# neeharperi/FutureDet

Measured on AMD Instinct MI355X. Metric: sweeps/sec end-to-end (300k pts, 10-sweep voxel), higher is better.
Workload: dtype f32

## Files before the change

### futuredet_amd/backbones.py

```python
import numpy as np
import torch
from torch import nn

from . import hip_ops, sparse as spconv
from .nn_utils import build_norm_layer
from .registry import BACKBONES
from .sparse import SparseConv3d, SubMConv3d


def conv3x3(in_planes, out_planes, stride=1, indice_key=None, bias=True):
    return spconv.SubMConv3d(in_planes, out_planes, kernel_size=3, stride=stride, padding=1, bias=bias,
                             indice_key=indice_key)


class SparseBasicBlock(spconv.SparseModule):
    expansion = 1

    def __init__(self, inplanes, planes, stride=1, norm_cfg=None, downsample=None, indice_key=None):
        super().__init__()
        if norm_cfg is None:
            norm_cfg = dict(type="BN1d", eps=1e-3, momentum=0.01)
        bias = norm_cfg is not None
        self.conv1 = conv3x3(inplanes, planes, stride, indice_key=indice_key, bias=bias)
        self.bn1 = build_norm_layer(norm_cfg, planes)[1]
        self.relu = nn.ReLU()
        self.conv2 = conv3x3(planes, planes, indice_key=indice_key, bias=bias)
        self.bn2 = build_norm_layer(norm_cfg, planes)[1]
        self.downsample = downsample
        self.stride = stride

    def forward(self, x):
        identity = x
        out = self.conv1(x)
        out.features = self.relu(self.bn1(out.features))
        out = self.conv2(out)
        out.features = self.bn2(out.features)
        if self.downsample is not None:
            identity = self.downsample(x)
        out.features = self.relu(out.features + identity.features)
        return out


@BACKBONES.register_module
class SpMiddleResNetFHD(nn.Module):
    def __init__(self, num_input_features=128, norm_cfg=None, name="SpMiddleResNetFHD", **kwargs):
        super().__init__()
        self.name = name
        if norm_cfg is None:
            norm_cfg = dict(type="BN1d", eps=1e-3, momentum=0.01)
        S = spconv.SparseSequential
        self.conv_input = S(SubMConv3d(num_input_features, 16, 3, bias=False, indice_key="res0"),
                            build_norm_layer(norm_cfg, 16)[1], nn.ReLU(inplace=True))
        self.conv1 = S(SparseBasicBlock(16, 16, norm_cfg=norm_cfg, indice_key="res0"),
                       SparseBasicBlock(16, 16, norm_cfg=norm_cfg, indice_key="res0"))
        self.conv2 = S(SparseConv3d(16, 32, 3, 2, padding=1, bias=False), build_norm_layer(norm_cfg, 32)[1],
                       nn.ReLU(inplace=True), SparseBasicBlock(32, 32, norm_cfg=norm_cfg, indice_key="res1"),
                       SparseBasicBlock(32, 32, norm_cfg=norm_cfg, indice_key="res1"))
        self.conv3 = S(SparseConv3d(32, 64, 3, 2, padding=1, bias=False), build_norm_layer(norm_cfg, 64)[1],
                       nn.ReLU(inplace=True), SparseBasicBlock(64, 64, norm_cfg=norm_cfg, indice_key="res2"),
                       SparseBasicBlock(64, 64, norm_cfg=norm_cfg, indice_key="res2"))
        self.conv4 = S(SparseConv3d(64, 128, 3, 2, padding=[0, 1, 1], bias=False), build_norm_layer(norm_cfg, 128)[1],
                       nn.ReLU(inplace=True), SparseBasicBlock(128, 128, norm_cfg=norm_cfg, indice_key="res3"),
                       SparseBasicBlock(128, 128, norm_cfg=norm_cfg, indice_key="res3"))
        self.extra_conv = S(SparseConv3d(128, 128, (3, 1, 1), (2, 1, 1), bias=False), build_norm_layer(norm_cfg, 128)[1],
                            nn.ReLU())
        self.compute_dtype = torch.float32
        self.dense_channels_last = True
        self.dense_dtype = None
        self.profile_hook = None

    def forward_generic(self, voxel_features, coors, batch_size, input_shape):
        sparse_shape = np.array(input_shape[::-1]) + [1, 0, 0]
        ret = spconv.SparseConvTensor(voxel_features, coors.int(), sparse_shape, batch_size)
        x = self.conv_input(ret)
        x_conv1 = self.conv1(x)
        x_conv2 = self.conv2(x_conv1)
        x_conv3 = self.conv3(x_conv2)
        x_conv4 = self.conv4(x_conv3)
        ret = self.extra_conv(x_conv4).dense()
        N, C, D, H, W = ret.shape
        ret = ret.view(N, C * D, H, W)
        return ret, {"conv1": x_conv1, "conv2": x_conv2, "conv3": x_conv3, "conv4": x_conv4}

    def _stages(self):
        return [(self.conv_input[0], self.conv_input[1], [self.conv1[0], self.conv1[1]], True),
                (self.conv2[0], self.conv2[1], [self.conv2[3], self.conv2[4]], False),
                (self.conv3[0], self.conv3[1], [self.conv3[3], self.conv3[4]], False),
                (self.conv4[0], self.conv4[1], [self.conv4[3], self.conv4[4]], False),
                (self.extra_conv[0], self.extra_conv[1], [], False)]

    def build_indexes(self, mark_fn, batch_size, input_shape, device, voxels=None, static=False, expected=None, row_caps=None):
        D, H, W = [int(v) for v in (np.array(input_shape[::-1]) + [1, 0, 0])]
        if voxels is not None:
            geoms = [self._stages()[lvl][0].geometry() for lvl in range(1, 5)]
            return hip_ops.build_pyramid(voxels[0], voxels[1], voxels[2], batch_size, (D, H, W), geoms, device, static=static,
                                         expected=expected, row_caps=row_caps)
        assert not static, "static indexes are built from the voxelizer's device output (voxels=...)"
        counts = torch.zeros((5,), dtype=torch.int32, device=device)
        idx = [hip_ops.SparseIndex(batch_size, D, H, W, device)]
        mark_fn(idx[0])
        idx[0].scan(counts[0:1])
        for lvl in range(1, 5):
            conv = self._stages()[lvl][0]
            ks, st, pd = conv.geometry()
            nxt = idx[-1].downsample(ks, st, pd)
            nxt.scan(counts[lvl:lvl + 1])
            idx.append(nxt)
        host = counts.cpu()
        for i, ix in enumerate(idx):
            ix.finalize(int(host[i]))
        return idx

    def run_fused(self, idx, feats0, dense_out=None, fork=False):
        dt = self.compute_dtype
        stages = self._stages()
        rb_cache = {}

        def rulebook(src, dst, conv):
            ks, st, pd = conv.geometry()
            key = (id(src), id(dst), tuple(ks), tuple(st), tuple(pd))
            if key not in rb_cache:
                rb_cache[key] = src.rulebook(dst, ks, st, pd)
            return rb_cache[key]

        def run(conv, bn, x, src, dst, relu, residual=None):
            wpk, bias, cin_p, cout_p = conv.packed_weight(dt, bn)
            assert x.shape[1] == cin_p, (x.shape, cin_p)
            nbr = rulebook(src, dst, conv)
            fn = lambda: hip_ops.spconv_apply(x, wpk, bias, nbr, dst.n, cout_p, residual=residual, relu=relu)
            if self.profile_hook is not None:
                s = 4 if dt == torch.float32 else 2
                K = nbr.shape[0]
                pairs = lambda: int((nbr[:, : dst.n] >= 0).sum().item())
                return self.profile_hook("spconv_%dx%d_K%d" % (cin_p, cout_p, K),
                                         dict(s=s, K=K, cin=cin_p, cout=cout_p, n_in=src.n, n_out=dst.n, pairs=pairs), fn)
            return fn()

        main, side = None, None
        if fork and feats0.is_cuda:
            main = torch.cuda.current_stream(feats0.device)
            pool = self.__dict__.setdefault("_side_streams", {})
            side = pool.get(main.cuda_stream)
            if side is None:
                side = pool[main.cuda_stream] = torch.cuda.Stream(device=feats0.device)
            side.wait_stream(main)
            with torch.cuda.stream(side):
                made = []
                for lvl, (conv, bn, blocks, is_subm_in) in enumerate(stages):
                    if lvl == 0:
                        continue
                    src_l, dst_l = (idx[lvl] if is_subm_in else idx[lvl - 1]), idx[lvl]
                    made.append(rulebook(src_l, dst_l, conv))
                    for blk in blocks:
                        nbr = rulebook(dst_l, dst_l, blk.conv1)
                        made.append(nbr)
                        cp = spconv.pad_channels(blk.conv1.out_channels)
                        if dt == torch.float32 and nbr.shape[0] == 27 and \
                                hip_ops._lib.load().fd_spconv_wants_balanced_ranges(cp, cp, 0):
                            r = hip_ops.ranges_for(nbr, cp, cp)
                            if r[0] is not None:
                                made.append(r[0])
                for t in made:
                    t.record_stream(main)
        x = feats0
        levels = {}
        for lvl, (conv, bn, blocks, is_subm_in) in enumerate(stages):
            src = idx[lvl] if is_subm_in else idx[lvl - 1]
            dst = idx[lvl]
            if lvl == 1 and side is not None:
                main.wait_stream(side)
            x = run(conv, bn, x, src, dst, relu=True)
            for blk in blocks:
                y = run(blk.conv1, blk.bn1, x, dst, dst, relu=True)
                x = run(blk.conv2, blk.bn2, y, dst, dst, relu=True, residual=x)
            levels[lvl] = (x, dst)
        bev = hip_ops.densify(x, idx[4], out_dtype=self.dense_dtype or dt, channels_last=self.dense_channels_last, out=dense_out)
        return bev, levels

    def forward(self, voxel_features, coors, batch_size, input_shape):
        if self.training:
            if self.compute_dtype != torch.float32 and torch.is_grad_enabled():
                raise NotImplementedError("SpMiddleResNetFHD: training runs the fp32 sparse convolution only; the %s path is inference-only "
                                          "(set compute_dtype = torch.float32 to train)" % self.compute_dtype)
            return self.forward_generic(voxel_features, coors, batch_size, input_shape)
        coors = coors.int().contiguous()
        dev = voxel_features.device
        idx = self.build_indexes(lambda i0: i0.mark(coors), batch_size, input_shape, dev)
        row_of = idx[0].lookup(coors)
        feats0 = hip_ops.rows_permute(voxel_features.float().contiguous(), row_of,
                                      spconv.pad_channels(voxel_features.shape[1]), self.compute_dtype, n_rows=idx[0].n)
        bev, levels = self.run_fused(idx, feats0)
        multi = {}
        for name, lvl, c in (("conv1", 0, 16), ("conv2", 1, 32), ("conv3", 2, 64), ("conv4", 3, 128)):
            f, ix = levels[lvl]
            multi[name] = spconv.SparseConvTensor(f[:, :c], None, ix.spatial_shape, batch_size, _index=ix)
        return bev, multi


@BACKBONES.register_module
class PointPillarsScatter(nn.Module):

    def __init__(self, num_input_features=64, norm_cfg=None, name="PointPillarsScatter", **kwargs):
        super().__init__()
        self.name = "PointPillarsScatter"
        self.nchannels = num_input_features
        self.dense_channels_last = True

    def forward(self, voxel_features, coords, batch_size, input_shape, n_dev=None):
        self.nx = int(input_shape[0])
        self.ny = int(input_shape[1])
        coords = coords.int().contiguous()
        if n_dev is None and torch.is_grad_enabled() and voxel_features.requires_grad:
            return _ScatterFn.apply(voxel_features, coords, batch_size, self.ny, self.nx, self.dense_channels_last)
        return hip_ops.pillar_scatter(voxel_features, coords, n_dev, batch_size, self.ny, self.nx,
                                      channels_last=self.dense_channels_last)


class _ScatterFn(torch.autograd.Function):

    @staticmethod
    def forward(ctx, feats, coords, batch_size, ny, nx, channels_last):
        ctx.coords = coords
        return hip_ops.pillar_scatter(feats, coords, None, batch_size, ny, nx, channels_last=channels_last)

    @staticmethod
    def backward(ctx, dcanvas):
        d = hip_ops.pillar_scatter_backward(dcanvas.float(), ctx.coords)
        ctx.coords = None
        return d, None, None, None, None, None
```

### futuredet_amd/csrc/fd_common.h

```cpp
#pragma once
#include <hip/hip_runtime.h>
#include <stdint.h>
#include <stdio.h>

#include <atomic>

#include "../../include/futuredet_hip.h"

namespace fd {

void set_error(const char *fmt, ...);
int spconv_f32_compact_dispatch(const float *in, const void *wp, const float *bias, const float *residual, int relu, const int *nbr,
                                int64_t nbr_stride, int K, int64_t n_in_bound, int n_out, const int *n_out_dev, int cin, int cout, float *out,
                                const int *ranges, int n_ranges, hipStream_t stream);

size_t spconv_bf16_win_weight_bytes(int K, int cin, int cout);
void spconv_bf16_win_pack(const float *w, int K, int cin, int cout, uint16_t (*tobf)(float), uint16_t *dst);
int spconv_bf16_win_dispatch(const void *in, const void *wp_win, const float *bias, const void *residual, int relu, const int *nbr, int64_t nbr_stride, int K,
                             int64_t n_in_bound, int n_out, const int *n_out_dev, int64_t n_expected, int cin, int cout, void *out, hipStream_t stream);
int spconv_bf16_ws_dispatch(const void *in, const void *wp, const float *bias, const void *residual, int relu, const int *nbr, int64_t nbr_stride, int K,
                            int64_t n_in_bound, int n_out, const int *n_out_dev, int64_t n_expected, int cin, int cout, void *out, hipStream_t stream);

int wino_pc_launch(const float *x, const void *wp, const float *bias, float *y, int B, int H, int W, int cin, int cout, int relu, int cout_total,
                   int co_off, int wide_items, hipStream_t stream);

int spconv_f32_res16_dispatch(const float *in, const void *wp, const float *bias, const float *residual, int relu, const int *nbr, int64_t nbr_stride, int K,
                              int64_t n_in_bound, int n_out, const int *n_out_dev, int64_t n_expected, int cin, int cout, float *out, hipStream_t stream);

int spconv_f32_c32_dispatch(const float *in, const void *wp, const float *bias, const float *residual, int relu, const int *nbr,
                            int64_t nbr_stride, int K, int64_t n_in_bound, int n_out, const int *n_out_dev, int cin, int cout, float *out,
                            const int *ranges, int n_ranges, hipStream_t stream);

__device__ __forceinline__ int device_count(int capacity, const int *count_dev) {
    if (!count_dev) return capacity;
    const int n = *count_dev;
    return n < capacity ? (n > 0 ? n : 0) : capacity;
}

inline int check_launch(const char *what) {
    hipError_t e = hipGetLastError();
    if (e != hipSuccess) {
        set_error("%s: %s", what, hipGetErrorString(e));
        return FD_ELAUNCH;
    }
    return FD_OK;
}

#define FD_REQUIRE(cond, ...)           \
    do {                                \
        if (!(cond)) {                  \
            fd::set_error(__VA_ARGS__); \
            return FD_EINVAL;           \
        }                               \
    } while (0)

inline hipStream_t as_stream(fd_stream_t s) { return reinterpret_cast<hipStream_t>(s); }

int fill_words(void *p, uint32_t value, size_t n_words, hipStream_t stream);
int fill_words3(void *p0, uint32_t v0, size_t n0, void *p1, uint32_t v1, size_t n1, void *p2, uint32_t v2, size_t n2, hipStream_t stream);

constexpr int kMaxDevices = 64;
int current_device();
int device_cu_count();
bool ensure_dynamic_lds(const void *kernel, size_t bytes, std::atomic<uint64_t> &done);
enum TuneKey { kTuneSpconvRG = 0, kTuneSpconvV1, kTuneSpconvBf16V1, kTuneV2Depth, kTuneV2TM, kTuneV2LdsPad, kTuneConvNT, kTuneV2RangesPerCU, kTuneV2Uniform, kTuneV2RowCost, kTuneSpconvC32, kTuneBf16GP, kTuneBf16RG, kTuneBf16Depth, kTuneBf16NW, kTuneStrict, kTuneBf16Win, kTuneF32ResRG, kTuneConvStrip, kTuneF32ResNW, kTuneCount };
int tuning(TuneKey key);

inline size_t align_up(size_t v, size_t a) { return (v + a - 1) / a * a; }

struct IndexGeom {
    int B, D, H, W, Ht, Wt;
    __host__ __device__ int64_t num_cols() const { return (int64_t)B * Ht * Wt * 64; }
};
__host__ __device__ inline IndexGeom make_geom(int B, int D, int H, int W) {
    IndexGeom g;
    g.B = B; g.D = D; g.H = H; g.W = W;
    g.Ht = (H + 7) >> 3; g.Wt = (W + 7) >> 3;
    return g;
}
__host__ __device__ inline int64_t col_of(const IndexGeom &g, int b, int y, int x) {
    return ((((int64_t)b * g.Ht + (y >> 3)) * g.Wt + (x >> 3)) << 6) + ((y & 7) << 3) + (x & 7);
}
__device__ inline void col_to_byx(const IndexGeom &g, int64_t col, int &b, int &y, int &x) {
    int in = (int)(col & 63);
    int64_t t = col >> 6;
    int tx = (int)(t % g.Wt);
    t /= g.Wt;
    int ty = (int)(t % g.Ht);
    b = (int)(t / g.Ht);
    y = ty * 8 + (in >> 3);
    x = tx * 8 + (in & 7);
}

__device__ inline unsigned xcd_swizzle(unsigned bid, unsigned nblocks) {
    const unsigned nx = 8;
    unsigned per = nblocks / nx, rem = nblocks % nx;
    unsigned xcd = bid % nx, loc = bid / nx;
    unsigned start = xcd * per + (xcd < rem ? xcd : rem);
    return start + loc;
}

}
```

### futuredet_amd/csrc/fd_error.hip

```cpp
#include <stdarg.h>
#include <stdlib.h>
#include <string.h>

#include "fd_common.h"

namespace fd {
static thread_local char g_err[512] = "";
void set_error(const char *fmt, ...) {
    va_list ap;
    va_start(ap, fmt);
    vsnprintf(g_err, sizeof(g_err), fmt, ap);
    va_end(ap);
}

int current_device() {
    int dev = 0;
    if (hipGetDevice(&dev) != hipSuccess) {
        (void)hipGetLastError();
        return 0;
    }
    return dev;
}

int device_cu_count() {
    static std::atomic<int> cache[kMaxDevices];
    const int dev = current_device();
    if (dev < 0 || dev >= kMaxDevices) return 256;
    int n = cache[dev].load(std::memory_order_relaxed);
    if (n <= 0) {
        if (hipDeviceGetAttribute(&n, hipDeviceAttributeMultiprocessorCount, dev) != hipSuccess || n <= 0) {
            (void)hipGetLastError();
            n = 256;
        }
        cache[dev].store(n, std::memory_order_relaxed);
    }
    return n;
}

bool ensure_dynamic_lds(const void *kernel, size_t bytes, std::atomic<uint64_t> &done) {
    const int dev = current_device();
    const uint64_t bit = (dev >= 0 && dev < kMaxDevices) ? (1ull << dev) : 0ull;
    if (bit && (done.load(std::memory_order_acquire) & bit)) return true;
    if (hipFuncSetAttribute(kernel, hipFuncAttributeMaxDynamicSharedMemorySize, (int)bytes) != hipSuccess) {
        (void)hipGetLastError();
        return false;
    }
    if (bit) done.fetch_or(bit, std::memory_order_release);
    return true;
}

namespace {
struct TuneTable {
    std::atomic<int> v[kTuneCount];
    TuneTable() {
        static const char *const env[kTuneCount] = {"FD_SPCONV_RG", "FD_SPCONV_V1", "FD_SPCONV_BF16_V1", "FD_V2_DEPTH", "FD_V2_TM",
                                                    "FD_V2_LDSPAD", "FD_CONV_NT", "FD_V2_RANGES_PER_CU", "FD_V2_UNIFORM", "FD_V2_ROWCOST", "FD_SPCONV_C32", "FD_BF16_GP", "FD_BF16_RG", "FD_BF16_DEPTH", "FD_BF16_NW", "FD_STRICT", "FD_BF16_WIN", "FD_F32_RES_RG", "FD_CONV_STRIP", "FD_F32_RES_NW"};
        for (int i = 0; i < kTuneCount; ++i) {
            const char *e = getenv(env[i]);
            v[i].store(e ? atoi(e) : 0, std::memory_order_relaxed);
        }
    }
};
TuneTable &tune_table() {
    static TuneTable t;
    return t;
}
const char *const kTuneNames[kTuneCount] = {"spconv_rg", "spconv_v1", "spconv_bf16_v1", "v2_depth", "v2_tm", "v2_ldspad", "conv_nt", "v2_ranges_per_cu", "v2_uniform", "v2_rowcost", "spconv_c32", "bf16_gp", "bf16_rg", "bf16_depth", "bf16_nw", "strict", "bf16_win", "f32_res_rg", "conv_strip", "f32_res_nw"};
}

int tuning(TuneKey key) { return tune_table().v[key].load(std::memory_order_relaxed); }
}

namespace {
struct FillJob {
    uint32_t *p[3];
    uint32_t v[3];
    size_t n[3];
    unsigned first_block[4];
};
__global__ void __launch_bounds__(256) fill_words_kernel(FillJob j) {
    const int r = blockIdx.x >= j.first_block[2] ? 2 : (blockIdx.x >= j.first_block[1] ? 1 : 0);
    uint32_t *__restrict__ p = j.p[r];
    const uint32_t v = j.v[r];
    const size_t n = j.n[r];
    const size_t nb = j.first_block[r + 1] - j.first_block[r], b = blockIdx.x - j.first_block[r];
    const size_t head = ((16 - ((uintptr_t)p & 15)) & 15) / 4 < n ? ((16 - ((uintptr_t)p & 15)) & 15) / 4 : n;
    const size_t n4 = (n - head) / 4;
    uint4 *p4 = reinterpret_cast<uint4 *>(p + head);
    const uint4 v4 = make_uint4(v, v, v, v);
    for (size_t i = b * 256 + threadIdx.x; i < n4; i += nb * 256) p4[i] = v4;
    if (b == 0) {
        if (threadIdx.x < head) p[threadIdx.x] = v;
        const size_t tail0 = head + n4 * 4;
        if (tail0 + threadIdx.x < n && threadIdx.x < 4) p[tail0 + threadIdx.x] = v;
    }
}
}

int fd::fill_words3(void *p0, uint32_t v0, size_t n0, void *p1, uint32_t v1, size_t n1, void *p2, uint32_t v2, size_t n2, hipStream_t stream) {
    FillJob j;
    void *ps[3] = {p0, p1, p2};
    const uint32_t vs[3] = {v0, v1, v2};
    const size_t ns[3] = {n0, n1, n2};
    unsigned total = 0;
    for (int r = 0; r < 3; ++r) {
        j.p[r] = (uint32_t *)ps[r];
        j.v[r] = vs[r];
        j.n[r] = ps[r] ? ns[r] : 0;
        j.first_block[r] = total;
        size_t blocks = j.n[r] ? (j.n[r] / 4 + 1023) / 1024 : 0;
        if (j.n[r] && blocks == 0) blocks = 1;
        if (blocks > 2048) blocks = 2048;
        total += (unsigned)blocks;
    }
    j.first_block[3] = total;
    if (!total) return 0;
    hipLaunchKernelGGL(fill_words_kernel, dim3(total), dim3(256), 0, stream, j);
    return 0;
}

int fd::fill_words(void *p, uint32_t value, size_t n_words, hipStream_t stream) {
    return fd::fill_words3(p, value, n_words, nullptr, 0u, 0, nullptr, 0u, 0, stream);
}

extern "C" const char *fd_last_error(void) { return fd::g_err; }
extern "C" int fd_abi_version(void) { return 8; }

extern "C" int fd_tuning_set(const char *name, int value) {
    FD_REQUIRE(name, "fd_tuning_set: null name");
    for (int i = 0; i < fd::kTuneCount; ++i)
        if (strcmp(name, fd::kTuneNames[i]) == 0) {
            fd::tune_table().v[i].store(value, std::memory_order_relaxed);
            return FD_OK;
        }
    fd::set_error("fd_tuning_set: unknown knob '%s'", name);
    return FD_EINVAL;
}
```

### futuredet_amd/csrc/fd_spconv.hip

```cpp
#include "fd_common.h"

namespace {

typedef float f32x4 __attribute__((ext_vector_type(4)));
typedef short s16x4 __attribute__((ext_vector_type(4)));
typedef __bf16 bf16x8 __attribute__((ext_vector_type(8)));

__device__ inline unsigned short f2bf(float v) {
    unsigned u = __float_as_uint(v);
    u += 0x7fffu + ((u >> 16) & 1u);
    return (unsigned short)(u >> 16);
}
__device__ inline float bf2f(unsigned short h) { return __uint_as_float(((unsigned)h) << 16); }

constexpr int kMaxTaps = 27;

template <int CIN, int COUT, int RG>
__global__ void __launch_bounds__(256) spconv_f32(const float *__restrict__ in, const float4 *__restrict__ wp,
                                                  const float *__restrict__ bias, const float *__restrict__ residual, int relu,
                                                  const int *__restrict__ nbr, int64_t nbr_stride, int K, int n_out,
                                                  const int *__restrict__ n_out_dev, float *__restrict__ out) {
    constexpr int ROWS_B = 64 * RG;
    constexpr int NB = COUT / 16, NC = CIN / 16;
    __shared__ int s_nbr[kMaxTaps * ROWS_B];
    const int tile = blockIdx.x;
    const int row0 = tile * ROWS_B;
    n_out = fd::device_count(n_out, n_out_dev);
    if (row0 >= n_out) return;
    for (int t = threadIdx.x; t < K * ROWS_B; t += 256) {
        int k = t / ROWS_B, r = t - k * ROWS_B;
        int64_t o = (int64_t)row0 + r;
        s_nbr[t] = (o < n_out) ? nbr[(int64_t)k * nbr_stride + o] : -1;
    }
    __syncthreads();
    const int lane = threadIdx.x & 63, wave = __builtin_amdgcn_readfirstlane(threadIdx.x >> 6);
    const int lrow = lane & 15, lq = lane >> 4;
    const int wrow = wave * 16 * RG;
    if (row0 + wrow >= n_out) return;

    f32x4 acc[RG][NB];
#pragma unroll
    for (int g = 0; g < RG; ++g)
#pragma unroll
        for (int nb = 0; nb < NB; ++nb) acc[g][nb] = (f32x4){0.f, 0.f, 0.f, 0.f};

    for (int k = 0; k < K; ++k) {
        int idx[RG];
        bool any[RG];
        bool any_all = false;
#pragma unroll
        for (int g = 0; g < RG; ++g) {
            idx[g] = s_nbr[k * ROWS_B + wrow + g * 16 + lrow];
            any[g] = __ballot(idx[g] >= 0) != 0ull;
            any_all = any_all || any[g];
        }
        if (!any_all) continue;
        const float4 *wk = wp + (int64_t)k * NC * NB * 64 + lane;
#pragma unroll
        for (int c = 0; c < NC; ++c) {
            float4 a[RG];
#pragma unroll
            for (int g = 0; g < RG; ++g) {
                a[g] = make_float4(0.f, 0.f, 0.f, 0.f);
                if (idx[g] >= 0) a[g] = *reinterpret_cast<const float4 *>(in + (int64_t)idx[g] * CIN + c * 16 + lq * 4);
            }
#pragma unroll
            for (int nb = 0; nb < NB; ++nb) {
                const float4 b = wk[(c * NB + nb) * 64];
#pragma unroll
                for (int g = 0; g < RG; ++g) {
                    if (any[g]) {
                        acc[g][nb] = __builtin_amdgcn_mfma_f32_16x16x4f32(a[g].x, b.x, acc[g][nb], 0, 0, 0);
                        acc[g][nb] = __builtin_amdgcn_mfma_f32_16x16x4f32(a[g].y, b.y, acc[g][nb], 0, 0, 0);
                        acc[g][nb] = __builtin_amdgcn_mfma_f32_16x16x4f32(a[g].z, b.z, acc[g][nb], 0, 0, 0);
                        acc[g][nb] = __builtin_amdgcn_mfma_f32_16x16x4f32(a[g].w, b.w, acc[g][nb], 0, 0, 0);
                    }
                }
            }
        }
    }
#pragma unroll
    for (int g = 0; g < RG; ++g) {
#pragma unroll
        for (int nb = 0; nb < NB; ++nb) {
            const int col = nb * 16 + lrow;
            const float bv = bias ? bias[col] : 0.0f;
#pragma unroll
            for (int r = 0; r < 4; ++r) {
                const int row = row0 + wrow + g * 16 + lq * 4 + r;
                if (row < n_out) {
                    float v = acc[g][nb][r] + bv;
                    if (residual) v += residual[(int64_t)row * COUT + col];
                    if (relu) v = fmaxf(v, 0.0f);
                    out[(int64_t)row * COUT + col] = v;
                }
            }
        }
    }
}

template <int CIN, int COUT, int RG>
__global__ void __launch_bounds__(256) spconv_bf16(const unsigned short *__restrict__ in, const void *__restrict__ wp_,
                                                   const float *__restrict__ bias, const unsigned short *__restrict__ residual,
                                                   int relu, const int *__restrict__ nbr, int64_t nbr_stride, int K, int n_out,
                                                   const int *__restrict__ n_out_dev, unsigned short *__restrict__ out) {
    constexpr int ROWS_B = 64 * RG;
    constexpr int NB = COUT / 16;
    constexpr bool WIDE = CIN >= 32;
    constexpr int NC = WIDE ? CIN / 32 : 1;
    __shared__ int s_nbr[kMaxTaps * ROWS_B];
    const int tile = blockIdx.x;
    const int row0 = tile * ROWS_B;
    n_out = fd::device_count(n_out, n_out_dev);
    if (row0 >= n_out) return;
    for (int t = threadIdx.x; t < K * ROWS_B; t += 256) {
        int k = t / ROWS_B, r = t - k * ROWS_B;
        int64_t o = (int64_t)row0 + r;
        s_nbr[t] = (o < n_out) ? nbr[(int64_t)k * nbr_stride + o] : -1;
    }
    __syncthreads();
    const int lane = threadIdx.x & 63, wave = __builtin_amdgcn_readfirstlane(threadIdx.x >> 6);
    const int lrow = lane & 15, lq = lane >> 4;
    const int wrow = wave * 16 * RG;
    if (row0 + wrow >= n_out) return;

    f32x4 acc[RG][NB];
#pragma unroll
    for (int g = 0; g < RG; ++g)
#pragma unroll
        for (int nb = 0; nb < NB; ++nb) acc[g][nb] = (f32x4){0.f, 0.f, 0.f, 0.f};

    for (int k = 0; k < K; ++k) {
        int idx[RG];
        bool any[RG];
        bool any_all = false;
#pragma unroll
        for (int g = 0; g < RG; ++g) {
            idx[g] = s_nbr[k * ROWS_B + wrow + g * 16 + lrow];
            any[g] = __ballot(idx[g] >= 0) != 0ull;
            any_all = any_all || any[g];
        }
        if (!any_all) continue;
        if constexpr (WIDE) {
            const bf16x8 *wk = reinterpret_cast<const bf16x8 *>(wp_) + (int64_t)k * NC * NB * 64 + lane;
#pragma unroll
            for (int c = 0; c < NC; ++c) {
                bf16x8 a[RG];
#pragma unroll
                for (int g = 0; g < RG; ++g) {
                    uint4 raw = make_uint4(0u, 0u, 0u, 0u);
                    if (idx[g] >= 0) raw = *reinterpret_cast<const uint4 *>(in + (int64_t)idx[g] * CIN + c * 32 + lq * 8);
                    a[g] = __builtin_bit_cast(bf16x8, raw);
                }
#pragma unroll
                for (int nb = 0; nb < NB; ++nb) {
                    const bf16x8 b = wk[(c * NB + nb) * 64];
#pragma unroll
                    for (int g = 0; g < RG; ++g)
                        if (any[g]) acc[g][nb] = __builtin_amdgcn_mfma_f32_16x16x32_bf16(a[g], b, acc[g][nb], 0, 0, 0);
                }
            }
        } else {
            const s16x4 *wk = reinterpret_cast<const s16x4 *>(wp_) + (int64_t)k * NB * 64 + lane;
            s16x4 a[RG];
#pragma unroll
            for (int g = 0; g < RG; ++g) {
                uint2 raw = make_uint2(0u, 0u);
                if (idx[g] >= 0) raw = *reinterpret_cast<const uint2 *>(in + (int64_t)idx[g] * CIN + lq * 4);
                a[g] = __builtin_bit_cast(s16x4, raw);
            }
#pragma unroll
            for (int nb = 0; nb < NB; ++nb) {
                const s16x4 b = wk[nb * 64];
#pragma unroll
                for (int g = 0; g < RG; ++g)
                    if (any[g]) acc[g][nb] = __builtin_amdgcn_mfma_f32_16x16x16bf16_1k(a[g], b, acc[g][nb], 0, 0, 0);
            }
        }
    }
#pragma unroll
    for (int g = 0; g < RG; ++g) {
#pragma unroll
        for (int nb = 0; nb < NB; ++nb) {
            const int col = nb * 16 + lrow;
            const float bv = bias ? bias[col] : 0.0f;
#pragma unroll
            for (int r = 0; r < 4; ++r) {
                const int row = row0 + wrow + g * 16 + lq * 4 + r;
                if (row < n_out) {
                    float v = acc[g][nb][r] + bv;
                    if (residual) v += bf2f(residual[(int64_t)row * COUT + col]);
                    if (relu) v = fmaxf(v, 0.0f);
                    out[(int64_t)row * COUT + col] = f2bf(v);
                }
            }
        }
    }
}

struct LaunchArgs {
    const void *in, *wp;
    const float *bias;
    const void *residual;
    int relu;
    const int *nbr;
    int64_t nbr_stride;
    int K, n_out;
    const int *n_out_dev;
    void *out;
    hipStream_t stream;
};

template <int CIN, int COUT, int RG>
void launch(const LaunchArgs &a, int dtype) {
    const int rows_b = 64 * RG;
    dim3 grid((unsigned)((a.n_out + rows_b - 1) / rows_b));
    if (dtype == 0)
        hipLaunchKernelGGL((spconv_f32<CIN, COUT, RG>), grid, dim3(256), 0, a.stream, (const float *)a.in, (const float4 *)a.wp, a.bias,
                           (const float *)a.residual, a.relu, a.nbr, a.nbr_stride, a.K, a.n_out, a.n_out_dev, (float *)a.out);
    else
        hipLaunchKernelGGL((spconv_bf16<CIN, COUT, RG>), grid, dim3(256), 0, a.stream, (const unsigned short *)a.in, a.wp, a.bias,
                           (const unsigned short *)a.residual, a.relu, a.nbr, a.nbr_stride, a.K, a.n_out, a.n_out_dev, (unsigned short *)a.out);
}

template <int CIN, int COUT>
void launch_rg(const LaunchArgs &a, int dtype, int rg) {
    if (rg >= 4) launch<CIN, COUT, 4>(a, dtype);
    else if (rg == 2) launch<CIN, COUT, 2>(a, dtype);
    else launch<CIN, COUT, 1>(a, dtype);
}

int pick_rg(int64_t n_out, int cin, int cout) {
    const int forced = fd::tuning(fd::kTuneSpconvRG);
    if (forced > 0) return forced;
    const int64_t waves2 = (n_out + 31) / 32;
    int rg = (cin * cout >= 128 * 128) ? 1 : 2;
    if (rg == 2 && waves2 < 256 * 4 * 2) rg = 1;
    return rg;
}

}

inline bool has_c32_layout(int cin, int cout, int dtype) { return dtype == 0 && cout == 32 && cin == 32; }
inline int64_t pair_layout_elems(int K, int cin, int cout, int dtype) { return (dtype == 1 && cin == 16) ? (int64_t)((K + 1) / 2) * 32 * cout : 0; }

extern "C" size_t fd_spconv_packed_weight_bytes(int K, int cin, int cout, int dtype) {
    if (K <= 0 || cin <= 0 || cout <= 0) return 0;
    return (size_t)K * cin * cout * (dtype == 0 ? 4 : 2) * (has_c32_layout(cin, cout, dtype) ? 2 : 1) + (size_t)pair_layout_elems(K, cin, cout, dtype) * 2 +
           (dtype == 1 ? fd::spconv_bf16_win_weight_bytes(K, cin, cout) : 0);
}

extern "C" int fd_spconv_pack_weight(const float *w, int K, int cin, int cout, int dtype, void *dst) {
    FD_REQUIRE(w && dst, "fd_spconv_pack_weight: null argument");
    FD_REQUIRE(K >= 1 && K <= kMaxTaps, "fd_spconv_pack_weight: K must be in [1,27]");
    FD_REQUIRE(cin % 16 == 0 && cout % 16 == 0 && cin >= 16 && cin <= 128 && cout >= 16 && cout <= 128,
               "fd_spconv_pack_weight: channels must be multiples of 16 in [16,128] (got %d -> %d)", cin, cout);
    FD_REQUIRE(dtype == 0 || dtype == 1, "fd_spconv_pack_weight: dtype must be 0 (f32) or 1 (bf16)");
    const int NB = cout / 16;
    auto W = [&](int k, int ci, int co) { return w[((int64_t)k * cin + ci) * cout + co]; };
    auto tobf = [](float v) -> uint16_t {
        union { float f; uint32_t u; } cvt;
        cvt.f = v;
        uint32_t u = cvt.u;
        u += 0x7fffu + ((u >> 16) & 1u);
        return (uint16_t)(u >> 16);
    };
    if (dtype == 0) {
        const int NC = cin / 16;
        float *d = (float *)dst;
        for (int k = 0; k < K; ++k)
            for (int c = 0; c < NC; ++c)
                for (int nb = 0; nb < NB; ++nb)
                    for (int lane = 0; lane < 64; ++lane)
                        for (int j = 0; j < 4; ++j)
                            d[((((int64_t)k * NC + c) * NB + nb) * 64 + lane) * 4 + j] =
                                W(k, 16 * c + 4 * (lane >> 4) + j, 16 * nb + (lane & 15));
        if (has_c32_layout(cin, cout, dtype)) {
            float *e = d + (int64_t)K * cin * cout;
            for (int k = 0; k < K; ++k)
                for (int c = 0; c < cin / 8; ++c)
                    for (int lane = 0; lane < 64; ++lane)
                        for (int j = 0; j < 4; ++j)
                            e[(((int64_t)k * (cin / 8) + c) * 64 + lane) * 4 + j] = W(k, 8 * c + 4 * (lane >> 5) + j, lane & 31);
        }
    } else if (cin >= 32) {
        FD_REQUIRE(cin % 32 == 0, "fd_spconv_pack_weight: bf16 needs cin 16 or a multiple of 32");
        const int NC = cin / 32;
        uint16_t *d = (uint16_t *)dst;
        for (int k = 0; k < K; ++k)
            for (int c = 0; c < NC; ++c)
                for (int nb = 0; nb < NB; ++nb)
                    for (int lane = 0; lane < 64; ++lane)
                        for (int j = 0; j < 8; ++j)
                            d[((((int64_t)k * NC + c) * NB + nb) * 64 + lane) * 8 + j] =
                                tobf(W(k, 32 * c + 8 * (lane >> 4) + j, 16 * nb + (lane & 15)));
        if (fd::spconv_bf16_win_weight_bytes(K, cin, cout)) fd::spconv_bf16_win_pack(w, K, cin, cout, +tobf, d + (int64_t)K * cin * cout);
    } else {
        uint16_t *d = (uint16_t *)dst;
        for (int k = 0; k < K; ++k)
            for (int nb = 0; nb < NB; ++nb)
                for (int lane = 0; lane < 64; ++lane)
                    for (int j = 0; j < 4; ++j)
                        d[(((int64_t)k * NB + nb) * 64 + lane) * 4 + j] = tobf(W(k, 4 * (lane >> 4) + j, 16 * nb + (lane & 15)));
        uint16_t *e = d + (int64_t)K * cin * cout;
        for (int u = 0; u < (K + 1) / 2; ++u)
            for (int nb = 0; nb < NB; ++nb)
                for (int lane = 0; lane < 64; ++lane)
                    for (int j = 0; j < 8; ++j) {
                        const int q = lane >> 4, k = 2 * u + (q >> 1);
                        e[(((int64_t)u * NB + nb) * 64 + lane) * 8 + j] = k < K ? tobf(W(k, 8 * (q & 1) + j, 16 * nb + (lane & 15))) : (uint16_t)0;
                    }
    }
    return FD_OK;
}

extern "C" int fd_spconv_apply(const void *in_feats, int64_t n_in, const void *wpacked, const float *bias, const void *residual, int relu,
                               const int32_t *nbr, int64_t nbr_stride, const int32_t *ranges, int n_ranges, int K, int64_t n_out,
                               const int32_t *n_out_dev, int64_t n_expected, int cin, int cout, int dtype, void *out_feats, fd_stream_t stream) {
    FD_REQUIRE(K >= 1 && K <= kMaxTaps, "fd_spconv_apply: K must be in [1,27]");
    FD_REQUIRE(dtype == 0 || dtype == 1, "fd_spconv_apply: dtype must be 0 (f32) or 1 (bf16)");
    FD_REQUIRE(n_out >= 0 && n_out <= nbr_stride && n_out < (1ll << 31), "fd_spconv_apply: n_out out of range");
    FD_REQUIRE(n_ranges >= 0 && (ranges == nullptr || n_ranges >= 1), "fd_spconv_apply: ranges needs n_ranges >= 1");
    if (n_expected <= 0 || n_expected > n_out) n_expected = n_out;
    if (n_out == 0) return FD_OK;
    FD_REQUIRE(in_feats && wpacked && nbr && out_feats, "fd_spconv_apply: null argument");
    if (dtype == 0 && !fd::tuning(fd::kTuneSpconvV1) && cin == 16 && fd::tuning(fd::kTuneF32ResRG) >= 0) {
        if (fd::spconv_f32_res16_dispatch((const float *)in_feats, wpacked, bias, (const float *)residual, relu, nbr, nbr_stride, K, n_in, (int)n_out,
                                          n_out_dev, n_expected, cin, cout, (float *)out_feats, fd::as_stream(stream)))
            return fd::check_launch("fd_spconv_apply(f32 resident)");
    }
    if (dtype == 0 && !fd::tuning(fd::kTuneSpconvV1) && has_c32_layout(cin, cout, dtype) && fd::tuning(fd::kTuneSpconvC32) >= 0) {
        const void *w32 = (const char *)wpacked + (size_t)K * cin * cout * 4;
        if (fd::spconv_f32_c32_dispatch((const float *)in_feats, w32, bias, (const float *)residual, relu, nbr, nbr_stride, K, n_in, (int)n_out,
                                        n_out_dev, cin, cout, (float *)out_feats, ranges, n_ranges, fd::as_stream(stream)))
            return fd::check_launch("fd_spconv_apply(c32)");
    }
    if (dtype == 0 && !fd::tuning(fd::kTuneSpconvV1)) {
        if (fd::spconv_f32_compact_dispatch((const float *)in_feats, wpacked, bias, (const float *)residual, relu, nbr, nbr_stride, K, n_in,
                                            (int)n_out, n_out_dev, cin, cout, (float *)out_feats, ranges, n_ranges, fd::as_stream(stream)))
            return fd::check_launch("fd_spconv_apply(compact)");
    }
    if (dtype == 1 && fd::tuning(fd::kTuneBf16GP) >= 0) {
        const void *w = cin == 16 ? (const void *)((const char *)wpacked + (size_t)K * cin * cout * 2) : wpacked;
        const bool subm_like = (K == 27 && n_in == n_out) || fd::tuning(fd::kTuneBf16Win) == 2;
        if (fd::tuning(fd::kTuneBf16Win) >= 0 && subm_like && fd::spconv_bf16_win_weight_bytes(K, cin, cout) &&
            fd::spconv_bf16_win_dispatch(in_feats, (const char *)wpacked + (size_t)K * cin * cout * 2, bias, residual, relu, nbr, nbr_stride, K, n_in, (int)n_out,
                                         n_out_dev, n_expected, cin, cout, out_feats, fd::as_stream(stream)))
            return fd::check_launch("fd_spconv_apply(bf16 window)");
        if (fd::spconv_bf16_ws_dispatch(in_feats, w, bias, residual, relu, nbr, nbr_stride, K, n_in, (int)n_out, n_out_dev, n_expected, cin, cout, out_feats,
                                        fd::as_stream(stream)))
            return fd::check_launch("fd_spconv_apply(bf16 ws)");
        if (fd::tuning(fd::kTuneStrict) && n_in * cin * 2 < (1ll << 31)) {
            fd::set_error("fd_spconv_apply: strict mode: the bf16 kernel (fd_spconv_bf16.hip) did not take %d -> %d, K = %d", cin, cout, K);
            return FD_EINVAL;
        }
    }
    LaunchArgs a{in_feats, wpacked, bias, residual, relu, nbr, nbr_stride, K, (int)n_out, n_out_dev, out_feats, fd::as_stream(stream)};
    const int rg = pick_rg(n_expected, cin, cout);
    const int key = cin * 1000 + cout;
    switch (key) {
        case 16016: launch_rg<16, 16>(a, dtype, rg); break;
        case 16032: launch_rg<16, 32>(a, dtype, rg); break;
        case 32032: launch_rg<32, 32>(a, dtype, rg); break;
        case 32064: launch_rg<32, 64>(a, dtype, rg); break;
        case 64064: launch_rg<64, 64>(a, dtype, rg); break;
        case 64128: launch_rg<64, 128>(a, dtype, rg); break;
        case 128128: launch_rg<128, 128>(a, dtype, rg); break;
        default:
            fd::set_error("fd_spconv_apply: unsupported channels %d -> %d", cin, cout);
            return FD_EINVAL;
    }
    return fd::check_launch("fd_spconv_apply");
}
```

### futuredet_amd/csrc/fd_spconv_c32.hip

```cpp
#include "fd_spconv_chunk.h"

namespace {

namespace sk = fd::skeleton;
typedef float f32x16 __attribute__((ext_vector_type(16)));
typedef unsigned u32x4 __attribute__((ext_vector_type(4)));
constexpr int TM = 128, COUT = 32, TS = 4, WR = 1;
constexpr sk::Layout L = sk::layout(TM, COUT, TS, 32);
static_assert(((sk::kMaxTaps + TS - 1) / TS) * (TM / WR / 32) <= L.item_slot, "item list slot");

template <int CIN, int DEPTH>
__global__ void __launch_bounds__(256) spconv_f32_c32(const float *__restrict__ in, const float4 *__restrict__ wp, const float *__restrict__ bias,
                                                      const float *__restrict__ residual, int relu, const int *__restrict__ nbr, int64_t nbr_stride,
                                                      int K, int n_out, const int *__restrict__ n_out_dev, float *__restrict__ out, unsigned in_bytes,
                                                      const int *__restrict__ ranges, int rows_per_range) {
    constexpr int NCH = CIN / 8;
    constexpr int kPad = sk::pad_entry(TM);
    extern __shared__ __attribute__((aligned(16))) unsigned char smem[];
    int *s_list = reinterpret_cast<int *>(smem + L.list);
    unsigned short *s_items = reinterpret_cast<unsigned short *>(smem + L.items);
    unsigned char *s_cnt = smem + L.cnt;
    int *s_pad = reinterpret_cast<int *>(smem + L.pad);
    float *s_acc = reinterpret_cast<float *>(smem + L.acc);

    const int tid = threadIdx.x, lane = tid & 63, wave = __builtin_amdgcn_readfirstlane(tid >> 6);
    int r_begin, r_end, n_chunks, chunk_rows;
    sk::resolve_range(n_out, n_out_dev, ranges, rows_per_range, r_begin, r_end);
    if (r_begin >= r_end) return;
    sk::cut_chunks<TM>(r_begin, r_end, n_chunks, chunk_rows);
    int pre[sk::kSliceRegs<TM>];
    sk::fetch_slice<TM>(pre, nbr, nbr_stride, K, r_begin);

    const int ln = lane & 31, lh = lane >> 5;
    const int ts = wave, wr = 0;
    unsigned char *acc_bytes = reinterpret_cast<unsigned char *>(s_acc + ts * L.acc_copy);
    const __amdgpu_buffer_rsrc_t rsrc = __builtin_amdgcn_make_buffer_rsrc(const_cast<float *>(in), 0, (int)in_bytes, 0x00020000);
    unsigned short *items = s_items + wave * L.item_slot;

    for (int chunk = 0; chunk < n_chunks; ++chunk) {
        int row0, n_rows;
        if (!sk::chunk_span(r_begin, r_end, chunk_rows, chunk, row0, n_rows)) break;
        sk::stage_chunk<TM, COUT, TS, 32>(pre, s_list, s_pad, s_acc, bias, residual, K, row0, n_rows);
        __syncthreads();
        sk::compact_taps<TM, WR>(s_list, s_cnt, K);
        __syncthreads();
        if (chunk + 1 < n_chunks) sk::fetch_slice<TM>(pre, nbr, nbr_stride, K, row0 + chunk_rows);
        const int n_items = sk::build_items<TS, 32>(s_cnt, items, K, ts, wr);

        int k_r[DEPTH], row_r[DEPTH];
        u32x4 a_r[DEPTH][NCH];
        auto stage_a0 = [&](int it) -> int { return sk::stage_a0(items, n_items, it); };
        auto stage_a1 = [&](int it, int code_v, int &kk, int &e) { sk::stage_a1<TM, WR, 32>(s_list, s_pad, n_items, wr, ln, it, code_v, kk, e); };
        auto gather_offset = [&](int e) -> unsigned { return sk::entry_row_bytes<CIN>(e) + (unsigned)(lh * 16); };
        auto gather_step = [&](unsigned voff, int c) { return __builtin_amdgcn_raw_buffer_load_b128(rsrc, voff + c * 32, 0, 0); };
        float4 b[NCH];
        auto load_b = [&](int k) {
            const float4 *wk = wp + (int64_t)k * NCH * 64 + lane;
#pragma unroll
            for (int c = 0; c < NCH; ++c) b[c] = wk[c * 64];
        };
        int k_s, e_s, code_s;
#pragma unroll
        for (int d = 0; d < DEPTH - 1; ++d) {
            stage_a1(d, stage_a0(d), k_s, e_s);
            const unsigned vo = gather_offset(e_s);
#pragma unroll
            for (int c = 0; c < NCH; ++c) a_r[d][c] = gather_step(vo, c);
            k_r[d] = k_s;
            row_r[d] = e_s;
        }
        k_r[DEPTH - 1] = -1;
        row_r[DEPTH - 1] = kPad;
        stage_a1(DEPTH - 1, stage_a0(DEPTH - 1), k_s, e_s);
        code_s = stage_a0(DEPTH);
        if (n_items > 0) load_b(k_r[0]);

        for (int i0 = 0; i0 < n_items; i0 += DEPTH) {
#pragma unroll
            for (int d = 0; d < DEPTH; ++d) {
                const unsigned arow = sk::entry_local_row(row_r[d]);
                unsigned aoff[4];
#pragma unroll
                for (int q = 0; q < 4; ++q) aoff[q] = sk::acc_slot_bytes<COUT>(arow, (unsigned)(2 * q + lh));
                f32x16 acc;
#pragma unroll
                for (int q = 0; q < 4; ++q) {
                    const float4 v = *reinterpret_cast<const float4 *>(acc_bytes + aoff[q]);
                    acc[4 * q + 0] = v.x; acc[4 * q + 1] = v.y; acc[4 * q + 2] = v.z; acc[4 * q + 3] = v.w;
                }
                const int dn = (d + DEPTH - 1) % DEPTH;
                {
                    const int it = i0 + d + DEPTH - 1;
                    const unsigned vo = gather_offset(e_s);
                    k_r[dn] = k_s;
                    row_r[dn] = e_s;
#pragma unroll
                    for (int c = 0; c < NCH; ++c) a_r[dn][c] = gather_step(vo, c);
                    stage_a1(it + 1, code_s, k_s, e_s);
                    code_s = stage_a0(it + 2);
                }
                const int knext = k_r[(d + 1) % DEPTH];
                const bool reload = knext >= 0 && knext != k_r[d];
                __builtin_amdgcn_sched_barrier(0);
#pragma unroll
                for (int c = 0; c < NCH; ++c) {
                    const float4 av = __builtin_bit_cast(float4, a_r[d][c]);
                    acc = __builtin_amdgcn_mfma_f32_32x32x2f32(b[c].x, av.x, acc, 0, 0, 0);
                    acc = __builtin_amdgcn_mfma_f32_32x32x2f32(b[c].y, av.y, acc, 0, 0, 0);
                    acc = __builtin_amdgcn_mfma_f32_32x32x2f32(b[c].z, av.z, acc, 0, 0, 0);
                    acc = __builtin_amdgcn_mfma_f32_32x32x2f32(b[c].w, av.w, acc, 0, 0, 0);
                    if (reload) b[c] = (wp + (int64_t)knext * NCH * 64 + lane)[c * 64];
                }
#pragma unroll
                for (int q = 0; q < 4; ++q)
                    *reinterpret_cast<float4 *>(acc_bytes + aoff[q]) = make_float4(acc[4 * q + 0], acc[4 * q + 1], acc[4 * q + 2], acc[4 * q + 3]);
                __builtin_amdgcn_sched_barrier(0);
            }
        }
        __syncthreads();
        sk::epilogue<TM, COUT, TS>(s_acc, bias, residual, relu, out, row0, n_rows);
        __syncthreads();
    }
}

template <int CIN, int DEPTH>
int launch_c32(const float *in, const void *wp, const float *bias, const float *residual, int relu, const int *nbr, int64_t nbr_stride, int K,
               int n_out, const int *n_out_dev, float *out, unsigned in_bytes, const int *ranges, int n_ranges, hipStream_t stream) {
    int rows_per = 0;
    if (!ranges) sk::equal_rows_split(n_out, TM, n_out_dev != nullptr, n_ranges, rows_per);
    static std::atomic<uint64_t> lds_set{0};
    if (!fd::ensure_dynamic_lds(reinterpret_cast<const void *>(spconv_f32_c32<CIN, DEPTH>), (size_t)L.bytes, lds_set)) return 0;
    hipLaunchKernelGGL((spconv_f32_c32<CIN, DEPTH>), dim3((unsigned)n_ranges), dim3(256), (size_t)L.bytes, stream, in, (const float4 *)wp, bias, residual, relu,
                       nbr, nbr_stride, K, n_out, n_out_dev, out, in_bytes, ranges, rows_per);
    return 1;
}

}

namespace fd {
int spconv_f32_c32_dispatch(const float *in, const void *wp, const float *bias, const float *residual, int relu, const int *nbr, int64_t nbr_stride,
                            int K, int64_t n_in_bound, int n_out, const int *n_out_dev, int cin, int cout, float *out, const int *ranges,
                            int n_ranges, hipStream_t stream) {
    if (cout != 32 || cin != 32) return 0;
    if (!sk::entries_fit(n_in_bound, cin)) return 0;
    const unsigned in_bytes = (unsigned)(n_in_bound * cin * 4);
    const int depth = fd::tuning(fd::kTuneV2Depth);
    if (depth == 2) return launch_c32<32, 2>(in, wp, bias, residual, relu, nbr, nbr_stride, K, n_out, n_out_dev, out, in_bytes, ranges, n_ranges, stream);
    if (depth == 4) return launch_c32<32, 4>(in, wp, bias, residual, relu, nbr, nbr_stride, K, n_out, n_out_dev, out, in_bytes, ranges, n_ranges, stream);
    return launch_c32<32, 3>(in, wp, bias, residual, relu, nbr, nbr_stride, K, n_out, n_out_dev, out, in_bytes, ranges, n_ranges, stream);
}
}
```

### futuredet_amd/csrc/fd_spconv_chunk.h

```cpp
#pragma once
#include "fd_common.h"

namespace fd {
namespace skeleton {

constexpr int kMaxTaps = 27;

constexpr int pad_entry(int tm) { return (int)(0xffffff00u | (unsigned)tm); }
__device__ __forceinline__ int pack_entry(int in_row, int local_row) { return (in_row << 8) | local_row; }
__device__ __forceinline__ unsigned entry_local_row(int e) { return (unsigned)e & 255u; }
template <int CIN>
__device__ __forceinline__ unsigned entry_row_bytes(int e) {
    static_assert(CIN == 16 || CIN == 32 || CIN == 64 || CIN == 128, "shift per CIN");
    const unsigned hi = (unsigned)e & 0xffffff00u;
    return CIN >= 64 ? hi << (CIN == 128 ? 1 : 0) : hi >> (CIN == 32 ? 1 : 2);
}
inline bool entries_fit(int64_t n_in_bound, int cin) { return n_in_bound < (1ll << 23) && n_in_bound * cin * 4 < (1ll << 31); }

struct Layout {
    int list;
    int items;
    int item_slot;
    int cnt;
    int pad;
    int acc;
    int acc_copy;
    int bytes;
};
constexpr int acc_copy_floats(int tm, int cout) { return (tm + 1) * cout; }
constexpr Layout layout(int tm, int cout, int ts, int item) {
    Layout l{};
    l.list = 0;
    l.items = l.list + (int)sizeof(int) * kMaxTaps * tm;
    l.item_slot = item == 16 ? kMaxTaps * (tm / 16) : 32;
    l.cnt = l.items + (int)sizeof(unsigned short) * 4 * l.item_slot;
    l.pad = l.cnt + 112;
    l.acc = l.pad + (int)sizeof(int) * item;
    l.acc_copy = acc_copy_floats(tm, cout);
    l.bytes = l.acc + (int)sizeof(float) * ts * l.acc_copy;
    return l;
}

template <int COUT>
__device__ __forceinline__ unsigned acc_swizzle(unsigned row) {
    static_assert(COUT == 16 || COUT == 32 || COUT == 64 || COUT == 128, "whole bank rows");
    constexpr int kSwzShift = COUT >= 64 ? 0 : COUT == 32 ? 1 : 2;
    constexpr unsigned kSwzMask = COUT >= 64 ? 15u : COUT == 32 ? 7u : 3u;
    return (row >> kSwzShift) & kSwzMask;
}
template <int COUT>
__device__ __forceinline__ int acc_slot(int row, int col) {
    return row * (COUT / 4) + (col ^ (int)acc_swizzle<COUT>((unsigned)row));
}
template <int COUT>
__device__ __forceinline__ unsigned acc_slot_bytes(unsigned row, unsigned col) {
    return row * (COUT * 4) + ((col ^ acc_swizzle<COUT>(row)) << 4);
}

__device__ __forceinline__ void resolve_range(int n_out, const int *n_out_dev, const int *ranges, int rows_per_range,
                                              int &r_begin, int &r_end) {
    if (n_out_dev) n_out = fd::device_count(n_out, n_out_dev);
    if (ranges) {
        r_begin = ranges[blockIdx.x];
        r_end = ranges[blockIdx.x + 1];
    } else {
        if (n_out_dev) rows_per_range = (((n_out + (int)gridDim.x - 1) / (int)gridDim.x) + 15) & ~15;
        const int64_t b = (int64_t)blockIdx.x * rows_per_range;
        r_begin = (int)(b < n_out ? b : n_out);
        r_end = (int)(b + rows_per_range < n_out ? b + rows_per_range : n_out);
    }
    if (r_end > n_out) r_end = n_out;
}
template <int TM>
__device__ __forceinline__ void cut_chunks(int r_begin, int r_end, int &n_chunks, int &chunk_rows) {
    n_chunks = (r_end - r_begin + TM - 1) / TM;
    chunk_rows = (((r_end - r_begin + n_chunks - 1) / n_chunks) + 15) & ~15;
}
__device__ __forceinline__ bool chunk_span(int r_begin, int r_end, int chunk_rows, int chunk, int &row0, int &n_rows) {
    row0 = r_begin + chunk * chunk_rows;
    n_rows = (r_end - row0) < chunk_rows ? (r_end - row0) : chunk_rows;
    return n_rows > 0;
}
inline void equal_rows_split(int n_out, int tm, bool device_count, int &n_ranges, int &rows_per) {
    if (n_ranges <= 0) n_ranges = (n_out + tm - 1) / tm;
    rows_per = (((n_out + n_ranges - 1) / n_ranges) + 15) & ~15;
    if (!device_count) n_ranges = (n_out + rows_per - 1) / rows_per;
}

template <int TM>
constexpr int kSliceRegs = (kMaxTaps * TM + 255) / 256;

template <int TM>
__device__ __forceinline__ void fetch_slice(int (&pre)[kSliceRegs<TM>], const int *nbr, int64_t nbr_stride, int K, int row0) {
    const int tid = threadIdx.x;
#pragma unroll
    for (int i = 0; i < kSliceRegs<TM>; ++i) {
        const int t = tid + i * 256;
        int k = t / TM;
        const int r = t - k * TM;
        k = k < K ? k : K - 1;
        int64_t o = (int64_t)row0 + r;
        o = o < nbr_stride ? o : nbr_stride - 1;
        pre[i] = nbr[(int64_t)k * nbr_stride + o];
    }
}

template <int COUT>
constexpr bool kInitAcc = COUT <= 64;

template <int TM, int COUT, int TS>
__device__ __forceinline__ void init_acc(float *s_acc, const float *bias, const float *residual, int row0, int n_rows) {
    const int tid = threadIdx.x;
    if constexpr (kInitAcc<COUT>) {
        constexpr int C4i = COUT / 4, NINIT = TM * C4i / 256;
        static_assert(TM * C4i % 256 == 0, "whole passes");
        float4 iv[NINIT];
#pragma unroll
        for (int i = 0; i < NINIT; ++i) {
            const int t = tid + i * 256, c4 = t % C4i;
            iv[i] = bias ? reinterpret_cast<const float4 *>(bias)[c4] : make_float4(0.f, 0.f, 0.f, 0.f);
        }
        if (residual) {
            float4 rv[NINIT];
#pragma unroll
            for (int i = 0; i < NINIT; ++i) {
                const int t = tid + i * 256, r = t / C4i, c4 = t - r * C4i;
                const int rr = r < n_rows ? r : n_rows - 1;
                rv[i] = reinterpret_cast<const float4 *>(residual + (int64_t)(row0 + rr) * COUT)[c4];
            }
#pragma unroll
            for (int i = 0; i < NINIT; ++i) { iv[i].x += rv[i].x; iv[i].y += rv[i].y; iv[i].z += rv[i].z; iv[i].w += rv[i].w; }
        }
#pragma unroll
        for (int i = 0; i < NINIT; ++i) {
            const int t = tid + i * 256, r = t / C4i, c4 = t - r * C4i;
            reinterpret_cast<float4 *>(s_acc)[acc_slot<COUT>(r, c4)] = r < n_rows ? iv[i] : make_float4(0.f, 0.f, 0.f, 0.f);
        }
        for (int t = TM * C4i + tid; t < TS * acc_copy_floats(TM, COUT) / 4; t += 256) reinterpret_cast<float4 *>(s_acc)[t] = make_float4(0.f, 0.f, 0.f, 0.f);
    } else {
        for (int t = tid; t < TS * acc_copy_floats(TM, COUT) / 4; t += 256) reinterpret_cast<float4 *>(s_acc)[t] = make_float4(0.f, 0.f, 0.f, 0.f);
    }
}

template <int TM, int COUT, int TS, int ITEM>
__device__ __forceinline__ void stage_chunk(const int (&pre)[kSliceRegs<TM>], int *s_list, int *s_pad, float *s_acc, const float *bias,
                                            const float *residual, int K, int row0, int n_rows) {
    const int tid = threadIdx.x;
    static_assert(256 % TM == 0, "a thread stages the same local row in every pass");
    const bool in_chunk = tid % TM < n_rows;
#pragma unroll
    for (int i = 0; i < kSliceRegs<TM>; ++i) {
        const int t = tid + i * 256;
        if (t < K * TM) s_list[t] = in_chunk ? pre[i] : -1;
    }
    init_acc<TM, COUT, TS>(s_acc, bias, residual, row0, n_rows);
    if (tid < ITEM) s_pad[tid] = pad_entry(TM);
}

template <int TM, int WR>
__device__ __forceinline__ void compact_taps(int *s_list, unsigned char *s_cnt, int K) {
    const int lane = threadIdx.x & 63, wave = __builtin_amdgcn_readfirstlane(threadIdx.x >> 6);
    constexpr int RW = TM / WR, NH = (RW + 63) / 64;
    for (int k = wave; k < K; k += 4) {
#pragma unroll
        for (int wr = 0; wr < WR; ++wr) {
            const int base = k * TM + wr * RW;
            int count = 0;
            int v[NH];
#pragma unroll
            for (int h = 0; h < NH; ++h) {
                const int r = h * 64 + lane;
                v[h] = (r < RW) ? s_list[base + r] : -1;
            }
#pragma unroll
            for (int h = 0; h < NH; ++h) {
                const int r = h * 64 + lane;
                if (r < RW) s_list[base + r] = pad_entry(TM);
            }
#pragma unroll
            for (int h = 0; h < NH; ++h) {
                const int r = h * 64 + lane;
                const unsigned long long m = __ballot(v[h] >= 0);
                const int pos = count + __popcll(m & ((1ull << lane) - 1ull));
                if (v[h] >= 0) s_list[base + pos] = pack_entry(v[h], wr * RW + r);
                count += __popcll(m);
            }
            if (lane == 0) s_cnt[k * 4 + wr] = (unsigned char)count;
        }
    }
}

template <int TS, int ITEM>
__device__ __forceinline__ int build_items(const unsigned char *s_cnt, unsigned short *items, int K, int ts, int wr) {
    const int lane = threadIdx.x & 63;
    const int ng = (lane < K && (lane % TS) == ts) ? ((int)s_cnt[lane * 4 + wr] + ITEM - 1) / ITEM : 0;
    int inc = ng;
#pragma unroll
    for (int off = 1; off < 64; off <<= 1) {
        const int u = __shfl_up(inc, off);
        if (lane >= off) inc += u;
    }
    const int n_items = __builtin_amdgcn_readfirstlane(__shfl(inc, 63));
    for (int g = 0; g < ng; ++g) items[inc - ng + g] = (unsigned short)((lane << 3) | g);
    __builtin_amdgcn_fence(__ATOMIC_RELEASE, "workgroup");
    __builtin_amdgcn_wave_barrier();
    __builtin_amdgcn_fence(__ATOMIC_ACQUIRE, "workgroup");
    return n_items;
}

__device__ __forceinline__ int stage_a0(const unsigned short *items, int n_items, int it) { return (int)items[it < n_items ? it : 0]; }
template <int TM, int WR, int ITEM>
__device__ __forceinline__ void stage_a1(const int *s_list, const int *s_pad, int n_items, int wr, int lp, int it, int code_v, int &kk, int &e) {
    const bool v = it < n_items;
    const int code = __builtin_amdgcn_readfirstlane(code_v);
    const int ks = v ? (code >> 3) : 0;
    kk = v ? ks : -1;
    const int *lst = v ? s_list + ks * TM + wr * (TM / WR) + (code & 7) * ITEM : s_pad;
    e = lst[lp];
}

template <int TM, int COUT, int TS>
__device__ __forceinline__ void epilogue(float *s_acc, const float *bias, const float *residual, int relu,
                                         float *out, int row0, int n_rows) {
    const int tid = threadIdx.x;
    constexpr int C4 = COUT / 4;
    for (int t = tid; t < n_rows * C4; t += 256) {
        const int r = t / C4, c4 = t - r * C4;
        const int row = row0 + r;
        const int slot = acc_slot<COUT>(r, c4);
        float4 v = reinterpret_cast<const float4 *>(s_acc)[slot];
#pragma unroll
        for (int q = 1; q < TS; ++q) {
            const float4 v2 = reinterpret_cast<const float4 *>(s_acc + q * acc_copy_floats(TM, COUT))[slot];
            v.x += v2.x; v.y += v2.y; v.z += v2.z; v.w += v2.w;
        }
        if constexpr (!kInitAcc<COUT>) {
            if (bias) {
                const float4 bv = reinterpret_cast<const float4 *>(bias)[c4];
                v.x += bv.x; v.y += bv.y; v.z += bv.z; v.w += bv.w;
            }
            if (residual) {
                const float4 rv = reinterpret_cast<const float4 *>(residual + (int64_t)row * COUT)[c4];
                v.x += rv.x; v.y += rv.y; v.z += rv.z; v.w += rv.w;
            }
        }
        if (relu) { v.x = fmaxf(v.x, 0.f); v.y = fmaxf(v.y, 0.f); v.z = fmaxf(v.z, 0.f); v.w = fmaxf(v.w, 0.f); }
        reinterpret_cast<float4 *>(out + (int64_t)row * COUT)[c4] = v;
    }
}

}
}
```

### futuredet_amd/csrc/fd_spconv_v2.hip

```cpp
#include "fd_spconv_chunk.h"

namespace {

namespace sk = fd::skeleton;
typedef float f32x4 __attribute__((ext_vector_type(4)));
typedef unsigned u32x4 __attribute__((ext_vector_type(4)));
typedef int i32x4 __attribute__((ext_vector_type(4)));

#ifdef FD_V2_TRACE
__device__ unsigned long long *g_trace;
#define FD_T(i)                                                                                  \
    do {                                                                                         \
        if (threadIdx.x == 0 && g_trace) g_trace[(size_t)blockIdx.x * 16 + (i)] = __builtin_readcyclecounter(); \
    } while (0)
#define FD_TV(i, v)                                                                    \
    do {                                                                               \
        if (threadIdx.x == 0 && g_trace) g_trace[(size_t)blockIdx.x * 16 + (i)] = (v); \
    } while (0)
#else
#define FD_T(i)
#define FD_TV(i, v)
#endif


constexpr int tap_splits(int cout) { return (cout == 32 || cout == 64) ? 2 : 1; }

template <int CIN, int COUT, int TM, int DEPTH>
__global__ void __launch_bounds__(256) spconv_f32_compact(const float *__restrict__ in, const float4 *__restrict__ wp,
                                                          const float *__restrict__ bias, const float *__restrict__ residual, int relu,
                                                          const int *__restrict__ nbr, int64_t nbr_stride, int K, int n_out,
                                                          const int *__restrict__ n_out_dev, float *__restrict__ out, unsigned in_bytes,
                                                          const int *__restrict__ ranges, int rows_per_range) {
    constexpr int NB = COUT / 16, NC = CIN / 16;
    constexpr int WC = NB == 8 ? 4 : (NB >= 2 ? 2 : 1);
    constexpr int NBW = NB / WC;
    constexpr int TS = tap_splits(COUT);
    constexpr int WR = 4 / (WC * TS);
    constexpr int NACC = NBW;
    static_assert((TM == 128 || TM == 64) && TM / WR >= 16, "local row uses 8 bits (0..TM, TM = scratch row)");
    constexpr int kPad = sk::pad_entry(TM);
    constexpr sk::Layout L = sk::layout(TM, COUT, TS, 16);
    extern __shared__ __attribute__((aligned(16))) unsigned char smem[];
    int *s_list = reinterpret_cast<int *>(smem + L.list);
    unsigned short *s_items = reinterpret_cast<unsigned short *>(smem + L.items);
    unsigned char *s_cnt = smem + L.cnt;
    int *s_pad = reinterpret_cast<int *>(smem + L.pad);
    float *s_acc = reinterpret_cast<float *>(smem + L.acc);

    const int tid = threadIdx.x, lane = tid & 63, wave = __builtin_amdgcn_readfirstlane(tid >> 6);
    int r_begin, r_end, n_chunks, chunk_rows;
    sk::resolve_range(n_out, n_out_dev, ranges, rows_per_range, r_begin, r_end);
    if (r_begin >= r_end) return;
    FD_T(0);
    sk::cut_chunks<TM>(r_begin, r_end, n_chunks, chunk_rows);
    int pre[sk::kSliceRegs<TM>];
    sk::fetch_slice<TM>(pre, nbr, nbr_stride, K, r_begin);

    const int lrow = lane & 15, lq = lane >> 4;
    const int wc = wave % WC, wr = TS == 1 ? wave / WC : 0, ts = TS == 1 ? 0 : wave / WC;
    const int cb = wc * NBW * 16;
    unsigned char *acc_bytes = reinterpret_cast<unsigned char *>(s_acc + ts * L.acc_copy);
    const unsigned slot0 = (unsigned)(cb >> 2) + (unsigned)lq;
    const __amdgpu_buffer_rsrc_t rsrc = __builtin_amdgcn_make_buffer_rsrc(const_cast<float *>(in), 0, (int)in_bytes, 0x00020000);
    unsigned short *items = s_items + wave * L.item_slot;

    for (int chunk = 0; chunk < n_chunks; ++chunk) {
    int row0, n_rows;
    if (!sk::chunk_span(r_begin, r_end, chunk_rows, chunk, row0, n_rows)) break;
    sk::stage_chunk<TM, COUT, TS, 16>(pre, s_list, s_pad, s_acc, bias, residual, K, row0, n_rows);
    __syncthreads();
    if (chunk == 0) FD_T(1);
    sk::compact_taps<TM, WR>(s_list, s_cnt, K);
    __syncthreads();
    if (chunk == 0) FD_T(2);
    if (chunk + 1 < n_chunks) sk::fetch_slice<TM>(pre, nbr, nbr_stride, K, row0 + chunk_rows);
    const int n_items = sk::build_items<TS, 16>(s_cnt, items, K, ts, wr);

    int k_r[DEPTH];
    int row_r[DEPTH];
    u32x4 a_r[DEPTH][NC];
    auto stage_a0 = [&](int it) -> int { return sk::stage_a0(items, n_items, it); };
    auto stage_a1 = [&](int it, int code_v, int &kk, int &e) { sk::stage_a1<TM, WR, 16>(s_list, s_pad, n_items, wr, lrow, it, code_v, kk, e); };
    auto gather_offset = [&](int e) -> unsigned { return sk::entry_row_bytes<CIN>(e) + (unsigned)(lq * 16); };
    auto gather_chunk = [&](unsigned voff, int c) { return __builtin_amdgcn_raw_buffer_load_b128(rsrc, voff + c * 64, 0, 0); };
    auto load_b = [&](int k, float4(&dst)[NC][NBW]) {
        const float4 *wk = wp + ((int64_t)k * NC * NB + wc * NBW) * 64 + lane;
#pragma unroll
        for (int c = 0; c < NC; ++c)
#pragma unroll
            for (int nw = 0; nw < NBW; ++nw) dst[c][nw] = wk[(c * NB + nw) * 64];
    };
    float4 b[NC][NBW];
    static_assert(DEPTH >= 2, "the slot freed by the previous item is refilled during the current item's MFMAs");
    int k_s, e_s, code_s;
#pragma unroll
    for (int d = 0; d < DEPTH - 1; ++d) {
        stage_a1(d, stage_a0(d), k_s, e_s);
        const unsigned vo = gather_offset(e_s);
#pragma unroll
        for (int c = 0; c < NC; ++c) a_r[d][c] = gather_chunk(vo, c);
        k_r[d] = k_s;
        row_r[d] = e_s;
    }
    k_r[DEPTH - 1] = -1;
    row_r[DEPTH - 1] = kPad;
    stage_a1(DEPTH - 1, stage_a0(DEPTH - 1), k_s, e_s);
    code_s = stage_a0(DEPTH);
    if (n_items > 0) load_b(k_r[0], b);
    if (chunk == 0) { FD_T(3); FD_TV(8, (unsigned long long)n_items); FD_TV(9, (unsigned long long)n_chunks); FD_TV(10, (unsigned long long)n_rows);
                      FD_TV(11, (unsigned long long)__builtin_amdgcn_s_getreg(4 | (31 << 11))); FD_TV(12, (unsigned long long)__builtin_amdgcn_s_getreg(20 | (31 << 11))); }
    FD_TV(13, (unsigned long long)(g_trace ? g_trace[(size_t)blockIdx.x * 16 + 13] : 0) + (unsigned long long)n_items);

    auto mfma_chunk = [&](const u32x4 &a4, const float4(&bc)[NBW], f32x4(&acc)[NACC]) {
        const float4 av = __builtin_bit_cast(float4, a4);
#pragma unroll
        for (int nw = 0; nw < NBW; ++nw) acc[nw] = __builtin_amdgcn_mfma_f32_16x16x4f32(bc[nw].x, av.x, acc[nw], 0, 0, 0);
#pragma unroll
        for (int nw = 0; nw < NBW; ++nw) acc[nw] = __builtin_amdgcn_mfma_f32_16x16x4f32(bc[nw].y, av.y, acc[nw], 0, 0, 0);
#pragma unroll
        for (int nw = 0; nw < NBW; ++nw) acc[nw] = __builtin_amdgcn_mfma_f32_16x16x4f32(bc[nw].z, av.z, acc[nw], 0, 0, 0);
#pragma unroll
        for (int nw = 0; nw < NBW; ++nw) acc[nw] = __builtin_amdgcn_mfma_f32_16x16x4f32(bc[nw].w, av.w, acc[nw], 0, 0, 0);
    };

    for (int i0 = 0; i0 < n_items; i0 += DEPTH) {
#pragma unroll
        for (int d = 0; d < DEPTH; ++d) {
            const unsigned arow = sk::entry_local_row(row_r[d]);
            unsigned aoff[NBW];
#pragma unroll
            for (int nw = 0; nw < NBW; ++nw) aoff[nw] = sk::acc_slot_bytes<COUT>(arow, slot0 + 4u * nw);
            f32x4 acc[NACC];
#pragma unroll
            for (int nw = 0; nw < NBW; ++nw) acc[nw] = *reinterpret_cast<const f32x4 *>(acc_bytes + aoff[nw]);
            const int dn = (d + DEPTH - 1) % DEPTH;
            unsigned vo;
            {
                const int it = i0 + d + DEPTH - 1;
                vo = gather_offset(e_s);
                k_r[dn] = k_s;
                row_r[dn] = e_s;
                stage_a1(it + 1, code_s, k_s, e_s);
                code_s = stage_a0(it + 2);
            }
            const int knext = k_r[(d + 1) % DEPTH];
            const bool reload = knext >= 0 && knext != k_r[d];
            constexpr bool kSpread = NC * 4 * NBW >= 16;
            if constexpr (!kSpread) {
#pragma unroll
                for (int c = 0; c < NC; ++c) a_r[dn][c] = gather_chunk(vo, c);
            }
            __builtin_amdgcn_sched_barrier(0);
            if (reload) {
                const float4 *wk = wp + ((int64_t)knext * NC * NB + wc * NBW) * 64 + lane;
#pragma unroll
                for (int c = 0; c < NC; ++c) {
                    mfma_chunk(a_r[d][c], b[c], acc);
                    if constexpr (kSpread) a_r[dn][c] = gather_chunk(vo, c);
#pragma unroll
                    for (int nw = 0; nw < NBW; ++nw) b[c][nw] = wk[(c * NB + nw) * 64];
                    __builtin_amdgcn_sched_group_barrier(0x008, 4 * NBW, 0);
                    __builtin_amdgcn_sched_group_barrier(0x020, (kSpread ? 1 : 0) + NBW, 0);
                }
            } else {
#pragma unroll
                for (int c = 0; c < NC; ++c) {
                    mfma_chunk(a_r[d][c], b[c], acc);
                    if constexpr (kSpread) {
                        a_r[dn][c] = gather_chunk(vo, c);
                        __builtin_amdgcn_sched_group_barrier(0x008, 4 * NBW, 0);
                        __builtin_amdgcn_sched_group_barrier(0x020, 1, 0);
                    }
                }
            }
#pragma unroll
            for (int nw = 0; nw < NBW; ++nw) *reinterpret_cast<f32x4 *>(acc_bytes + aoff[nw]) = acc[nw];
            __builtin_amdgcn_sched_barrier(0);
        }
    }
    if (chunk == 0) FD_T(4);
    __syncthreads();
    if (chunk == 0) FD_T(5);
    sk::epilogue<TM, COUT, TS>(s_acc, bias, residual, relu, out, row0, n_rows);
    __syncthreads();
    if (chunk == 0) FD_T(6);
    }
    FD_T(7);
}

inline size_t lds_request(int cin, int cout, int tm) {
    const size_t lds = (size_t)sk::layout(tm, cout, tap_splits(cout), 16).bytes;
    const size_t pad = (size_t)fd::tuning(fd::kTuneV2LdsPad);
    if (pad) return lds + pad;
    return (cin == 64 && cout == 64 && tm == 128 && lds < 56 * 1024) ? (size_t)56 * 1024 : lds;
}

template <int CIN, int COUT, int TM, int DEPTH>
int launch_compact(const float *in, const void *wp, const float *bias, const float *residual, int relu, const int *nbr,
                   int64_t nbr_stride, int K, int n_out, const int *n_out_dev, float *out, unsigned in_bytes, const int *ranges, int n_ranges,
                   hipStream_t stream) {
    const size_t lds_req = lds_request(CIN, COUT, TM);
    static std::atomic<uint64_t> lds_set{0};
    auto kern = spconv_f32_compact<CIN, COUT, TM, DEPTH>;
    if (fd::tuning(fd::kTuneV2LdsPad)) {
        if (hipFuncSetAttribute(reinterpret_cast<const void *>(kern), hipFuncAttributeMaxDynamicSharedMemorySize, (int)lds_req) != hipSuccess) {
            (void)hipGetLastError();
            return 0;
        }
    } else if (!fd::ensure_dynamic_lds(reinterpret_cast<const void *>(kern), lds_req, lds_set)) {
        return 0;
    }
    int rows_per = 0;
    if (!ranges) sk::equal_rows_split(n_out, TM, n_out_dev != nullptr, n_ranges, rows_per);
    hipLaunchKernelGGL(kern, dim3((unsigned)n_ranges), dim3(256), lds_req, stream, in, (const float4 *)wp, bias, residual, relu, nbr, nbr_stride, K,
                       n_out, n_out_dev, out, in_bytes, ranges, rows_per);
    return 1;
}

constexpr int kWorkRows = 8;
constexpr int kRowCost = 24;
__global__ void __launch_bounds__(256) block_work_kernel(const int *__restrict__ nbr, int64_t nbr_stride, int K, int n_out,
                                                         const int *__restrict__ n_out_dev, unsigned row_cost, unsigned *__restrict__ work) {
    n_out = fd::device_count(n_out, n_out_dev);
    const int n_blocks = (n_out + kWorkRows - 1) / kWorkRows;
    const int lane = threadIdx.x & 63;
    const int64_t wave = (int64_t)blockIdx.x * 4 + (threadIdx.x >> 6);
    const int64_t o = wave * 64 + lane;
    if (wave * 8 >= n_blocks) return;
    unsigned w = row_cost;
    for (int k = 0; k < K; ++k) {
        const bool v = o < n_out && nbr[(int64_t)k * nbr_stride + o] >= 0;
        const unsigned long long m = __ballot(v);
        const unsigned byte = (unsigned)(m >> (8 * (lane & 7))) & 0xffu;
        w += (unsigned)__popc(byte) * 2u + (byte ? 1u : 0u);
    }
    if (lane < 8 && wave * 8 + lane < n_blocks) work[wave * 8 + lane] = w;
}

__global__ void __launch_bounds__(1024) range_split_kernel(const unsigned *__restrict__ work, int n_out, const int *__restrict__ n_out_dev,
                                                           int n_ranges, int *__restrict__ ranges) {
    n_out = fd::device_count(n_out, n_out_dev);
    const int n_blocks = (n_out + kWorkRows - 1) / kWorkRows;
    __shared__ unsigned long long s_seg[16];
    __shared__ unsigned long long s_total;
    const int tid = threadIdx.x, lane = tid & 63, wave = tid >> 6;
    if (n_blocks == 0) {
        for (int j = tid; j <= n_ranges; j += 1024) ranges[j] = 0;
        return;
    }
    const int seg = (((n_blocks + 15) / 16) + 63) & ~63;
    const int b_lo = wave * seg, b_hi = min(n_blocks, b_lo + seg);
    constexpr int kU = 16;
    unsigned long long sum = 0;
    for (int c0 = b_lo; c0 < b_hi; c0 += 64 * kU) {
        unsigned wv[kU];
#pragma unroll
        for (int u = 0; u < kU; ++u) {
            const int bb = c0 + 64 * u + lane;
            wv[u] = work[bb < b_hi ? bb : b_hi - 1];
        }
#pragma unroll
        for (int u = 0; u < kU; ++u) sum += (c0 + 64 * u + lane < b_hi) ? wv[u] : 0u;
    }
#pragma unroll
    for (int o = 32; o > 0; o >>= 1) sum += __shfl_xor(sum, o);
    if (lane == 0) s_seg[wave] = sum;
    __syncthreads();
    if (tid == 0) {
        unsigned long long run = 0;
        for (int w = 0; w < 16; ++w) { const unsigned long long v = s_seg[w]; s_seg[w] = run; run += v; }
        s_total = run;
    }
    __syncthreads();
    const unsigned long long total = s_total > 0 ? s_total : 1ull;
    const double scale = (double)n_ranges / (2.0 * (double)total);
    auto range_of = [&](unsigned long long ex, unsigned w) -> int {
        const int r = (int)((double)(2ull * ex + w) * scale);
        return r < n_ranges ? r : n_ranges - 1;
    };
    unsigned long long run = s_seg[wave];
    int prev = -1;
    if (b_lo > 0 && b_lo < n_blocks) {
        const unsigned wp = work[b_lo - 1];
        prev = range_of(run - wp, wp);
    }
    constexpr int kB = 8;
    __shared__ unsigned s_buf[16][64 * (kB + 1)];
    unsigned *buf = s_buf[wave];
    for (int c0 = b_lo; c0 < b_hi; c0 += 64 * kB) {
#pragma unroll
        for (int u = 0; u < kB; ++u) {
            const int e = 64 * u + lane, bb = c0 + e;
            buf[(e / kB) * (kB + 1) + e % kB] = bb < b_hi ? work[bb] : 0u;
        }
        __builtin_amdgcn_fence(__ATOMIC_RELEASE, "workgroup");
        __builtin_amdgcn_wave_barrier();
        __builtin_amdgcn_fence(__ATOMIC_ACQUIRE, "workgroup");
        unsigned w[kB];
        unsigned tot = 0;
#pragma unroll
        for (int i = 0; i < kB; ++i) {
            w[i] = buf[lane * (kB + 1) + i];
            tot += w[i];
        }
        unsigned inc = tot;
#pragma unroll
        for (int o = 1; o < 64; o <<= 1) {
            const unsigned u = __shfl_up(inc, o);
            if (lane >= o) inc += u;
        }
        unsigned long long ex = run + (inc - tot);
        const int first = c0 + lane * kB;
        int last_rg = prev;
        {
            unsigned long long e2 = ex;
#pragma unroll
            for (int i = 0; i < kB; ++i) {
                if (first + i < b_hi) last_rg = range_of(e2, w[i]);
                e2 += w[i];
            }
        }
        int before = __shfl_up(last_rg, 1);
        if (lane == 0) before = prev;
        if (first >= b_hi) last_rg = before;
#pragma unroll
        for (int i = 0; i < kB; ++i) {
            const int bb = first + i;
            if (bb < b_hi) {
                const int rg = range_of(ex, w[i]);
                for (int j = before + 1; j <= rg; ++j) ranges[j] = bb * kWorkRows;
                before = rg;
                if (bb == n_blocks - 1)
                    for (int j = rg + 1; j <= n_ranges; ++j) ranges[j] = n_out;
            }
            ex += w[i];
        }
        const int n_valid = min(64 * kB, b_hi - c0);
        prev = __shfl(last_rg, (n_valid - 1) / kB);
        run += __shfl(inc, 63);
        __builtin_amdgcn_wave_barrier();
    }
}

}

#ifdef FD_V2_TRACE
extern "C" int fd_debug_set_trace(void *p) { return hipMemcpyToSymbol(HIP_SYMBOL(g_trace), &p, sizeof(p)) == hipSuccess ? 0 : -1; }
#endif

extern "C" int fd_spconv_num_ranges(int64_t n_out, int cin, int cout, int dtype) {
    if (n_out <= 0 || dtype != 0) return 0;
    const int n_cu = fd::device_cu_count();
    const int64_t tiles = (n_out + 127) / 128;
    const int mult = fd::tuning(fd::kTuneV2RangesPerCU);
    int64_t per_cu;
    if (mult) per_cu = mult;
    else if (cout >= 64) per_cu = (int64_t)((160 * 1024) / lds_request(cin, cout, 128));
    else per_cu = (tiles + n_cu - 1) / n_cu;
    if (per_cu < 1) per_cu = 1;
    return (int)(per_cu * n_cu);
}

extern "C" int fd_spconv_wants_balanced_ranges(int cin, int cout, int dtype) { return dtype == 0 && cout >= 64 && !fd::tuning(fd::kTuneV2Uniform); }

extern "C" size_t fd_spconv_ranges_workspace_bytes(int64_t n_out) {
    return fd::align_up(sizeof(unsigned) * (size_t)((n_out + kWorkRows - 1) / kWorkRows + 8), 256);
}

extern "C" int fd_spconv_ranges(const int32_t *nbr, int64_t nbr_stride, int K, int64_t n_out, const int32_t *n_out_dev, int n_ranges,
                                int32_t *ranges, void *workspace, size_t workspace_bytes, fd_stream_t stream_) {
    FD_REQUIRE(nbr && ranges && workspace, "fd_spconv_ranges: null argument");
    FD_REQUIRE(n_ranges >= 1 && n_out >= 0 && n_out <= nbr_stride && n_out < (1ll << 31), "fd_spconv_ranges: bad sizes");
    FD_REQUIRE(workspace_bytes >= fd_spconv_ranges_workspace_bytes(n_out), "fd_spconv_ranges: workspace too small");
    hipStream_t stream = fd::as_stream(stream_);
    const int n_blocks = (int)((n_out + kWorkRows - 1) / kWorkRows);
    unsigned *work = (unsigned *)workspace;
    if (n_blocks > 0)
        hipLaunchKernelGGL(block_work_kernel, dim3((unsigned)((n_blocks + 31) / 32)), dim3(256), 0, stream, nbr, nbr_stride, K, (int)n_out, n_out_dev,
                           (unsigned)(fd::tuning(fd::kTuneV2RowCost) ? fd::tuning(fd::kTuneV2RowCost) : kRowCost), work);
    hipLaunchKernelGGL(range_split_kernel, dim3(1), dim3(1024), 0, stream, work, (int)n_out, n_out_dev, n_ranges, ranges);
    return fd::check_launch("fd_spconv_ranges");
}

namespace fd {
int spconv_f32_compact_dispatch(const float *in, const void *wp, const float *bias, const float *residual, int relu, const int *nbr,
                                int64_t nbr_stride, int K, int64_t n_in_bound, int n_out, const int *n_out_dev, int cin, int cout, float *out,
                                const int *ranges, int n_ranges, hipStream_t stream) {
    if (!sk::entries_fit(n_in_bound, cin)) return 0;
    const unsigned in_bytes = (unsigned)(n_in_bound * cin * 4);
    const int dsel = fd::tuning(fd::kTuneV2Depth), tsel = fd::tuning(fd::kTuneV2TM);
#define FD_LAUNCH(CI, CO, T, D) \
    launch_compact<CI, CO, T, D>(in, wp, bias, residual, relu, nbr, nbr_stride, K, n_out, n_out_dev, out, in_bytes, ranges, n_ranges, stream)
#define FD_CASE(CI, CO, DDEF, TDEF)                                  \
    if (cin == CI && cout == CO) {                                   \
        const int dd = dsel ? dsel : DDEF, tt = tsel ? tsel : TDEF;  \
        if (tt == 64) {                                              \
            if (dd <= 2) return FD_LAUNCH(CI, CO, 64, 2);            \
            if (dd == 3) return FD_LAUNCH(CI, CO, 64, 3);            \
            return FD_LAUNCH(CI, CO, 64, 4);                         \
        }                                                            \
        if (dd <= 2) return FD_LAUNCH(CI, CO, 128, 2);               \
        if (dd == 3) return FD_LAUNCH(CI, CO, 128, 3);               \
        return FD_LAUNCH(CI, CO, 128, 4);                            \
    }
    FD_CASE(16, 16, 4, 128)
    FD_CASE(16, 32, 4, 128)
    FD_CASE(32, 32, 4, 128)
    FD_CASE(32, 64, 4, 128)
    FD_CASE(64, 64, 3, 128)
    FD_CASE(64, 128, 3, 128)
    FD_CASE(128, 128, 2, 128)
    FD_CASE(32, 16, 4, 128)
    FD_CASE(64, 32, 4, 128)
    FD_CASE(128, 64, 2, 128)
#undef FD_CASE
#undef FD_LAUNCH
    return 0;
}
}
```

### futuredet_amd/hip_ops.py

```python
import ctypes
import threading

import numpy as np
import torch

from . import lib as _lib
from .lib import DecodeCfg, FutureDetHipError, MapView, check


_raw_stream = getattr(torch._C, "_cuda_getCurrentRawStream", None)


def _stream():
    if _raw_stream is not None:
        return ctypes.c_void_p(_raw_stream(torch.cuda.current_device()))
    return ctypes.c_void_p(torch.cuda.current_stream().cuda_stream)


def _dev(t, name, dtype=None):
    if not isinstance(t, torch.Tensor) or not t.is_cuda:
        raise FutureDetHipError("%s must be a tensor on the HIP device (got %s); this path has no CPU implementation"
                                % (name, "cpu tensor" if isinstance(t, torch.Tensor) else type(t)))
    if dtype is not None and t.dtype != dtype:
        raise FutureDetHipError("%s must be %s, got %s" % (name, dtype, t.dtype))
    if not t.is_contiguous():
        raise FutureDetHipError("%s must be contiguous" % name)
    return t


def _p(t):
    return ctypes.c_void_p(t.data_ptr()) if t is not None else None


class _Workspace(object):

    def __init__(self):
        self._bufs = {}
        self._scope = threading.local()

    def scope(self, token):
        ws = self

        class _Scope(object):
            def __enter__(self_):
                self_.prev = getattr(ws._scope, "token", None)
                ws._scope.token = token

            def __exit__(self_, *exc):
                ws._scope.token = self_.prev

        return _Scope()

    def release(self, token):
        for key in [k for k in self._bufs if k[2] == ("scope", token)]:
            del self._bufs[key]

    def get(self, tag, nbytes, device):
        token = getattr(self._scope, "token", None)
        key = (tag, device.index, ("scope", token) if token is not None else _stream().value)
        buf = self._bufs.get(key)
        if buf is None or buf.numel() < nbytes:
            buf = torch.empty(max(int(nbytes), 256), dtype=torch.uint8, device=device)
            self._bufs[key] = buf
        return buf


workspace = _Workspace()
_DT = {torch.float32: 0, torch.bfloat16: 1}


def set_tuning(name, value):
    check(_lib.load().fd_tuning_set(name.encode(), int(value)), "fd_tuning_set")


def voxelize(points, voxel_size, coors_range, max_points, max_voxels, batch_idx=0, want_voxels=True, want_mean=False,
             mean_stride=None, coor_cols=3, out=None, n_points_dev=None):
    L = _lib.load()
    points = _dev(points, "points", torch.float32)
    n, ndim = points.shape
    dev = points.device
    rng = (ctypes.c_float * 6)(*[float(np.float32(v)) for v in coors_range])
    vs = (ctypes.c_float * 3)(*[float(np.float32(v)) for v in voxel_size])
    out = dict(out or {})
    if want_voxels and "voxels" not in out:
        out["voxels"] = torch.empty((max_voxels, max_points, ndim), dtype=torch.float32, device=dev)
    if want_mean and "mean" not in out:
        out["mean"] = torch.empty((max_voxels, mean_stride or ndim), dtype=torch.float32, device=dev)
    if "coors" not in out:
        out["coors"] = torch.empty((max_voxels, coor_cols), dtype=torch.int32, device=dev)
    if "num_points" not in out:
        out["num_points"] = torch.empty((max_voxels,), dtype=torch.int32, device=dev)
    if "num_voxels" not in out:
        out["num_voxels"] = torch.zeros((1,), dtype=torch.int32, device=dev)
    mean = out.get("mean") if want_mean else None
    voxels = out.get("voxels") if want_voxels else None
    ws_bytes = L.fd_voxelize_workspace_bytes(n, max_voxels)
    ws = workspace.get("voxelize", ws_bytes, dev)
    check(L.fd_voxelize(_p(points), n, _p(n_points_dev), ndim, rng, vs, int(max_points), int(max_voxels), int(batch_idx), _p(voxels), _p(mean),
                        int(mean.shape[1]) if mean is not None else 0, _p(out["coors"]), int(out["coors"].shape[1]),
                        _p(out["num_points"]), _p(out["num_voxels"]), _p(ws), ws.numel(), _stream()), "fd_voxelize")
    return out


class SparseIndex(object):

    def __init__(self, B, D, H, W, device, words=None, prefix=None):
        L = _lib.load()
        self.B, self.D, self.H, self.W = int(B), int(D), int(H), int(W)
        self.ncols = L.fd_index_num_cols(self.B, self.H, self.W)
        self.words = torch.zeros((self.ncols,), dtype=torch.int64, device=device) if words is None else words
        self.prefix = torch.empty((self.ncols,), dtype=torch.int32, device=device) if prefix is None else prefix
        self.n_dev = None
        self.n = None
        self.coords = None
        self.device = device
        self.static = False
        self.n_expected = 0

    @property
    def spatial_shape(self):
        return [self.D, self.H, self.W]

    def mark(self, coords, n_dev=None, n_max=None):
        L = _lib.load()
        coords = _dev(coords, "coords", torch.int32)
        n_max = coords.shape[0] if n_max is None else n_max
        check(L.fd_index_mark(_p(coords), _p(n_dev), n_max, self.B, self.D, self.H, self.W, _p(self.words), _stream()),
              "fd_index_mark")

    def scan(self, n_dev):
        L = _lib.load()
        ws = workspace.get("index_scan", L.fd_index_workspace_bytes(self.ncols), self.device)
        self.n_dev = n_dev
        check(L.fd_index_scan(_p(self.words), self.ncols, _p(self.prefix), _p(n_dev), _p(ws), ws.numel(), _stream()),
              "fd_index_scan")

    def downsample(self, ksize, stride, pad):
        L = _lib.load()
        od = [(i + 2 * p - (k - 1) - 1) // s + 1 for i, k, s, p in zip(self.spatial_shape, ksize, stride, pad)]
        out = SparseIndex(self.B, od[0], od[1], od[2], self.device)
        check(L.fd_index_downsample(_p(self.words), self.B, self.D, self.H, self.W, (ctypes.c_int * 3)(*ksize),
                                    (ctypes.c_int * 3)(*stride), (ctypes.c_int * 3)(*pad), _p(out.words), _stream()),
              "fd_index_downsample")
        return out

    def finalize(self, n):
        L = _lib.load()
        self.n = int(n)
        self.coords = torch.empty((max(self.n, 1), 4), dtype=torch.int32, device=self.device)[: self.n]
        if self.n:
            check(L.fd_index_coords(_p(self.words), _p(self.prefix), self.B, self.D, self.H, self.W, _p(self.coords),
                                    _stream()), "fd_index_coords")

    def lookup(self, coords, n_dev=None):
        L = _lib.load()
        coords = _dev(coords, "coords", torch.int32)
        row_of = torch.empty((coords.shape[0],), dtype=torch.int32, device=self.device)
        check(L.fd_index_lookup(_p(self.words), _p(self.prefix), self.B, self.D, self.H, self.W, _p(coords), _p(n_dev),
                                coords.shape[0], _p(row_of), _stream()), "fd_index_lookup")
        return row_of

    def rulebook(self, out_index, ksize, stride, pad):
        L = _lib.load()
        assert out_index.n is not None
        K = int(ksize[0] * ksize[1] * ksize[2])
        nstride = max(64, (out_index.n + 63) // 64 * 64)
        nbr = torch.empty((K, nstride), dtype=torch.int32, device=self.device)
        static = getattr(out_index, "static", False)
        if out_index.n == 0:
            nbr.fill_(-1)
            return nbr
        check(L.fd_rulebook(_p(self.words), _p(self.prefix), self.B, self.D, self.H, self.W, _p(out_index.coords), out_index.n,
                            _p(out_index.n_dev), nstride, 0 if static else 1, (ctypes.c_int * 3)(*ksize), (ctypes.c_int * 3)(*stride),
                            (ctypes.c_int * 3)(*pad), _p(nbr), _stream()), "fd_rulebook")
        nbr.n_out = out_index.n
        nbr.n_dev = out_index.n_dev if static else None
        nbr.n_expected = out_index.n_expected if static else 0
        return nbr


class _PyramidPlan(object):

    def __init__(self, B, shape0, geoms, device):
        L = _lib.load()
        self.B, self.geoms, self.device = int(B), geoms, device
        self.shapes = [tuple(int(v) for v in shape0)]
        for ks, st, pd in geoms:
            self.shapes.append(tuple((i + 2 * p - (k - 1) - 1) // s + 1 for i, k, s, p in zip(self.shapes[-1], ks, st, pd)))
        self.ncols = [L.fd_index_num_cols(self.B, sh[1], sh[2]) for sh in self.shapes]
        self.ws_bytes = L.fd_index_workspace_bytes(sum(self.ncols) + 2048 * len(self.ncols))

    def row_caps(self, cap0):
        caps = [min(int(cap0), self.B * int(np.prod(self.shapes[0])))]
        for (ks, st, pd), sh in zip(self.geoms, self.shapes[1:]):
            fan = int(np.prod([-(-k // s) for k, s in zip(ks, st)]))
            caps.append(min(caps[-1] * fan, self.B * int(np.prod(sh))))
        return caps


_pyramid_plans = {}


def build_pyramid(coors, nvox, n_max, B, shape0, geoms, device, static=False, expected=None, row_caps=None):
    L = _lib.load()
    key = (int(B), tuple(int(v) for v in shape0), tuple((tuple(k), tuple(s), tuple(p)) for k, s, p in geoms), str(device))
    plan = _pyramid_plans.get(key)
    if plan is None:
        plan = _pyramid_plans[key] = _PyramidPlan(B, shape0, geoms, device)
    shapes, ncols = plan.shapes, plan.ncols
    words_all = torch.empty((sum(ncols),), dtype=torch.int64, device=device)
    prefix_all = torch.empty((sum(ncols),), dtype=torch.int32, device=device)
    counts = torch.empty((len(shapes),), dtype=torch.int32, device=device)
    idx, off = [], 0
    levels = (_lib.IndexLevel * len(shapes))()
    wp, pp = words_all.data_ptr(), prefix_all.data_ptr()
    for l, (sh, nc) in enumerate(zip(shapes, ncols)):
        ix = SparseIndex.__new__(SparseIndex)
        ix.B, ix.D, ix.H, ix.W, ix.ncols, ix.device = plan.B, sh[0], sh[1], sh[2], nc, device
        ix.words, ix.prefix = words_all[off:off + nc], prefix_all[off:off + nc]
        ix.n_dev, ix.n, ix.coords = counts[l:l + 1], None, None
        ix.level_counts = counts
        ix.static, ix.n_expected = False, 0
        lv = levels[l]
        lv.D, lv.H, lv.W = sh
        if l:
            ks, st, pd = geoms[l - 1]
            lv.ksize[:], lv.stride[:], lv.pad[:] = list(ks), list(st), list(pd)
        lv.words, lv.prefix, lv.coords = wp + 8 * off, pp + 4 * off, None
        idx.append(ix)
        off += nc
    ws = workspace.get("index_scan", plan.ws_bytes, device)

    def size_coords(host):
        total = sum(host)
        coords_all = torch.empty((max(total, 1), 4), dtype=torch.int32, device=device)
        o = 0
        for l, ix in enumerate(idx):
            ix.n = int(host[l])
            ix.coords = coords_all[o:o + ix.n]
            levels[l].coords = (coords_all.data_ptr() + 16 * o) if ix.n else None
            levels[l].coords_rows = ix.n
            o += ix.n

    if static:
        host = plan.row_caps(int(B) * int(n_max))
        if row_caps is not None:
            host = [min(int(a), int(b)) for a, b in zip(host, row_caps)]
        for l, ix in enumerate(idx):
            ix.static = True
            ix.n_expected = int(expected[l]) if expected is not None else 0
        size_coords(host)
        fused = all(int(h) > 0 for h in host)
        check(L.fd_index_pyramid(_p(coors), _p(nvox), int(n_max), plan.B, len(shapes), levels, _p(counts), _p(ws), ws.numel(), _stream()),
              "fd_index_pyramid")
        if not fused:
            check(L.fd_index_pyramid_coords(plan.B, len(shapes), levels, _stream()), "fd_index_pyramid_coords")
        return idx
    check(L.fd_index_pyramid(_p(coors), _p(nvox), int(n_max), plan.B, len(shapes), levels, _p(counts), _p(ws), ws.numel(), _stream()),
          "fd_index_pyramid")
    size_coords(counts.tolist())
    check(L.fd_index_pyramid_coords(plan.B, len(shapes), levels, _stream()), "fd_index_pyramid_coords")
    return idx


def ranges_for(nbr, cin, cout):
    cached = getattr(nbr, "ranges", None)
    if cached is not None:
        return cached
    L = _lib.load()
    n_out = getattr(nbr, "n_out", None)
    if not n_out:
        return None, 0
    K, nstride = nbr.shape
    n = int(L.fd_spconv_num_ranges(getattr(nbr, "n_expected", 0) or n_out, cin, cout, 0))
    if n <= 0:
        return None, 0
    ranges = torch.empty((n + 1,), dtype=torch.int32, device=nbr.device)
    ws = workspace.get("spconv_ranges", L.fd_spconv_ranges_workspace_bytes(n_out), nbr.device)
    check(L.fd_spconv_ranges(_p(nbr), nstride, K, n_out, _p(getattr(nbr, "n_dev", None)), n, _p(ranges), _p(ws), ws.numel(), _stream()),
          "fd_spconv_ranges")
    nbr.ranges = (ranges, n)
    return nbr.ranges


def rows_permute(src, row_of, c_dst, dtype=torch.float32, n_rows=None, n_dev=None):
    L = _lib.load()
    src = _dev(src, "src", torch.float32)
    row_of = _dev(row_of, "row_of", torch.int32)
    n_rows = src.shape[0] if n_rows is None else n_rows
    dst = torch.zeros((max(n_rows, 1), c_dst), dtype=dtype, device=src.device)[:n_rows]
    if src.shape[0]:
        check(L.fd_rows_permute(_p(src), src.shape[1], _p(row_of), _p(n_dev), src.shape[0], _p(dst), c_dst,
                                _DT[dtype], _stream()), "fd_rows_permute")
    return dst


def rows_place(index, coords, src, c_dst, dtype=torch.float32, n_dev=None, out=None):
    L = _lib.load()
    coords = _dev(coords, "coords", torch.int32)
    src = _dev(src, "src", torch.float32)
    if out is None:
        out = torch.zeros((max(index.n, 1), c_dst), dtype=dtype, device=src.device)[: index.n]
    _dev(out, "out", dtype)
    if coords.dim() != 2 or coords.shape[1] != 4:
        raise FutureDetHipError("rows_place: coords must be [n, 4] (b, z, y, x), got %s" % (tuple(coords.shape),))
    if src.dim() != 2 or src.shape[0] < coords.shape[0]:
        raise FutureDetHipError("rows_place: src must be [n, c_src] with a row per coordinate")
    if out.dim() != 2 or out.shape[1] != c_dst or index.n is None or out.shape[0] < index.n:
        raise FutureDetHipError("rows_place: out must be [rows >= index.n, %d] (finalised index), got %s" % (c_dst, tuple(out.shape)))
    check(L.fd_rows_place(_p(index.words), _p(index.prefix), index.B, index.D, index.H, index.W, _p(coords), _p(n_dev),
                          coords.shape[0], _p(src), src.shape[1], _p(out), c_dst, _DT[dtype], _stream()), "fd_rows_place")
    return out


def pack_spconv_weight(w_kio, dtype=torch.float32):
    L = _lib.load()
    dev = w_kio.device
    w = w_kio.detach().to("cpu", torch.float32).contiguous()
    K, cin, cout = w.shape
    nbytes = L.fd_spconv_packed_weight_bytes(K, cin, cout, _DT[dtype])
    host = torch.empty((nbytes,), dtype=torch.uint8)
    check(L.fd_spconv_pack_weight(ctypes.c_void_p(w.data_ptr()), K, cin, cout, _DT[dtype], ctypes.c_void_p(host.data_ptr())),
          "fd_spconv_pack_weight")
    return host.to(dev)


PACK_PLAIN, PACK_TRANSPOSED, PACK_FLIPPED_TRANSPOSED = 0, 1, 2


def pack_spconv_weight_device(w_kio, mode=PACK_PLAIN):
    L = _lib.load()
    w = _dev(w_kio.detach(), "w_kio", torch.float32)
    K, cin, cout = w.shape
    ci, co = (cout, cin) if mode else (cin, cout)
    out = torch.empty((L.fd_spconv_packed_weight_bytes(K, ci, co, 0),), dtype=torch.uint8, device=w.device)
    check(L.fd_spconv_pack_weight_device(_p(w), K, cin, cout, int(mode), _p(out), _stream()), "fd_spconv_pack_weight_device")
    return out


def spconv_wgrad(feats, dy, nbr, n_out):
    L = _lib.load()
    feats = _dev(feats, "feats", torch.float32)
    dy = _dev(dy, "dy", torch.float32)
    K, nstride = nbr.shape
    cin, cout = feats.shape[1], dy.shape[1]
    assert dy.shape[0] >= n_out
    dw = torch.empty((K, cin, cout), dtype=torch.float32, device=feats.device)
    ws = workspace.get("spconv_wgrad", L.fd_spconv_wgrad_workspace_bytes(K, n_out, cin, cout), feats.device)
    check(L.fd_spconv_wgrad(_p(feats), feats.shape[0], _p(dy), _p(_dev(nbr, "nbr", torch.int32)), nstride, K, n_out,
                            _p(getattr(nbr, "n_dev", None)), cin, cout, _p(dw), _p(ws), ws.numel(), _stream()), "fd_spconv_wgrad")
    return dw


def assign_targets(boxes, counts, classes, trajectory, cfg, out):
    L = _lib.load()
    boxes = _dev(boxes, "boxes", torch.float32)
    B = boxes.shape[0]
    assert tuple(boxes.shape) == (B, cfg.T, cfg.n_max, 12), (tuple(boxes.shape), cfg.T, cfg.n_max)
    assert tuple(counts.shape) == (B, cfg.T) and tuple(classes.shape) == (B, cfg.T, cfg.n_max)
    assert (trajectory is None) == (cfg.n_sets == 1)
    if trajectory is not None:
        assert tuple(trajectory.shape) == (B, cfg.T, cfg.n_max)
        trajectory = _dev(trajectory, "trajectory", torch.int32)
    U = cfg.n_tasks + (2 if cfg.n_sets == 3 else 0)
    ws = workspace.get("targets", L.fd_targets_workspace_bytes(B, cfg.T, U, cfg.max_objs), boxes.device)
    check(L.fd_assign_targets(_p(boxes), _p(_dev(counts, "counts", torch.int32)), _p(_dev(classes, "classes", torch.int32)), _p(trajectory), B,
                              ctypes.byref(cfg), _p(_dev(out["hm"], "hm", torch.float32)), _p(_dev(out["ind"], "ind", torch.int64)),
                              _p(_dev(out["mask"], "mask", torch.uint8)), _p(_dev(out["cat"], "cat", torch.int64)),
                              _p(_dev(out["anno_box"], "anno_box", torch.float32)), _p(_dev(out["gt_boxes_and_cls"], "gt_boxes_and_cls", torch.float32)),
                              _p(_dev(out["status"], "status", torch.int32)), _p(ws), ws.numel(), _stream()), "fd_assign_targets")
    return out


def rulebook_transpose(nbr, n_out, n_in):
    L = _lib.load()
    K, nstride = nbr.shape
    istride = max(64, (n_in + 63) // 64 * 64)
    inv = torch.empty((K, istride), dtype=torch.int32, device=nbr.device)
    check(L.fd_rulebook_transpose(_p(_dev(nbr, "nbr", torch.int32)), nstride, K, n_out, _p(getattr(nbr, "n_dev", None)), n_in, _p(inv),
                                  istride, _stream()), "fd_rulebook_transpose")
    return inv


def dense_gather(grad, index, c):
    L = _lib.load()
    if not (isinstance(grad, torch.Tensor) and grad.is_cuda and grad.dtype == torch.float32):
        raise FutureDetHipError("dense_gather: grad must be a float32 tensor on the HIP device")
    n = int(index.n)
    feats = torch.empty((max(n, 1), c), dtype=torch.float32, device=grad.device)[:n]
    sb, sc, sy, sx = grad.stride()
    check(L.fd_dense_gather(_p(grad), sb, sc, sy, sx, index.D, _p(index.coords), n, _p(index.n_dev if index.static else None), c,
                            _p(feats), _stream()), "fd_dense_gather")
    return feats


def spconv_apply(feats, wpacked, bias, nbr, n_out, cout, residual=None, relu=False, out=None, balanced=None):
    L = _lib.load()
    feats = _dev(feats, "feats")
    dt = _DT[feats.dtype]
    cin = feats.shape[1]
    out_dtype, out_cols = feats.dtype, cout
    K, nstride = nbr.shape
    if out is None:
        out = torch.empty((max(n_out, 1), out_cols), dtype=out_dtype, device=feats.device)[:n_out]
    if residual is not None:
        _dev(residual, "residual", out_dtype)
    ranges, n_ranges = None, 0
    n_dev, n_expected = getattr(nbr, "n_dev", None), getattr(nbr, "n_expected", 0)
    if dt == 0 and n_out > 0:
        if balanced is None:
            balanced = K == 27 and cin == cout and bool(L.fd_spconv_wants_balanced_ranges(cin, cout, 0))
        if balanced == "tiles":
            n_ranges = 0
        elif balanced:
            ranges, n_ranges = ranges_for(nbr, cin, cout)
        else:
            n_ranges = int(L.fd_spconv_num_ranges(n_expected or n_out, cin, cout, 0))
    check(L.fd_spconv_apply(_p(feats), feats.shape[0], _p(_dev(wpacked, "wpacked")), _p(bias), _p(residual), int(bool(relu)),
                            _p(_dev(nbr, "nbr", torch.int32)), nstride, _p(ranges), n_ranges, K, n_out, _p(n_dev), int(n_expected or 0),
                            cin, cout, dt, _p(out), _stream()),
          "fd_spconv_apply")
    return out


def densify(feats, index, out_dtype=None, channels_last=False, out=None):
    L = _lib.load()
    feats = _dev(feats, "feats")
    C = feats.shape[1]
    shape = (index.B, C * index.D, index.H, index.W)
    if out is None:
        out_dtype = out_dtype or feats.dtype
        out = torch.empty(shape, dtype=out_dtype, device=feats.device,
                          memory_format=torch.channels_last if channels_last else torch.contiguous_format)
    else:
        assert tuple(out.shape) == shape and out.is_cuda
        out_dtype = out.dtype
    sb, sc, sy, sx = out.stride()
    check(L.fd_densify(_p(feats), C, _DT[feats.dtype], _p(index.words), _p(index.prefix), index.B, index.D, index.H,
                       index.W, _p(out), _DT[out_dtype], sb, sc, sy, sx, int(feats.shape[0]), _stream()), "fd_densify")
    return out


def pack_conv2d_weight(w_oihw):
    L = _lib.load()
    dev = w_oihw.device
    w = w_oihw.detach().to("cpu", torch.float32).contiguous()
    cout, cin, ks, _ = w.shape
    nbytes = L.fd_conv2d_packed_weight_bytes(cout, cin, ks)
    if nbytes == 0:
        raise FutureDetHipError("fd_conv2d: unsupported weight shape %s" % (tuple(w.shape),))
    host = torch.empty((nbytes,), dtype=torch.uint8)
    check(L.fd_conv2d_pack_weight(ctypes.c_void_p(w.data_ptr()), cout, cin, ks, ctypes.c_void_p(host.data_ptr())),
          "fd_conv2d_pack_weight")
    return host.to(dev)


def conv2d_nhwc_bf16(x, wpk, bias, cout, ks, stride=1, relu=True, out=None, co_off=0, osy=1, osx=1, ooy=0, oox=0):
    L = _lib.load()
    x = _dev(x, "x", torch.bfloat16)
    B, H, W, cin = x.shape
    pad = 1 if ks == 3 else 0
    Ho, Wo = (H + 2 * pad - ks) // stride + 1, (W + 2 * pad - ks) // stride + 1
    if out is None:
        out = torch.empty((B, Ho * osy, Wo * osx, cout), dtype=torch.bfloat16, device=x.device)
    _dev(out, "out", torch.bfloat16)
    check(L.fd_conv2d_nhwc_bf16(_p(x), B, H, W, cin, _p(wpk), _p(bias), cout, ks, stride, pad, int(bool(relu)), _p(out),
                                out.shape[3], co_off, osy, osx, ooy, oox, _stream()), "fd_conv2d_nhwc_bf16")
    return out


def pack_conv2d_weight_f32(w_oihw):
    L = _lib.load()
    dev = w_oihw.device
    w = w_oihw.detach().to("cpu", torch.float32).contiguous()
    cout, cin, ks, _ = w.shape
    nbytes = L.fd_conv2d_f32_packed_weight_bytes(cout, cin, ks)
    if nbytes == 0:
        raise FutureDetHipError("fd_conv2d_f32: unsupported weight shape %s" % (tuple(w.shape),))
    host = torch.empty((nbytes,), dtype=torch.uint8)
    check(L.fd_conv2d_f32_pack_weight(ctypes.c_void_p(w.data_ptr()), cout, cin, ks, ctypes.c_void_p(host.data_ptr())),
          "fd_conv2d_f32_pack_weight")
    return host.to(dev)


def conv2d_nhwc_f32(x, wpk, bias, cout, ks, stride=1, relu=True, out=None, co_off=0, osy=1, osx=1, ooy=0, oox=0, tile=0):
    L = _lib.load()
    x = _dev(x, "x", torch.float32)
    B, H, W, cin = x.shape
    pad = 1 if ks == 3 else 0
    Ho, Wo = (H + 2 * pad - ks) // stride + 1, (W + 2 * pad - ks) // stride + 1
    if out is None:
        out = torch.empty((B, Ho * osy, Wo * osx, cout), dtype=torch.float32, device=x.device)
    _dev(out, "out", torch.float32)
    check(L.fd_conv2d_nhwc_f32(_p(x), B, H, W, cin, _p(wpk), _p(bias), cout, ks, stride, pad, int(bool(relu)), _p(out),
                               out.shape[3], co_off, osy, osx, ooy, oox, int(tile), _stream()), "fd_conv2d_nhwc_f32")
    return out


def conv2d_f32_num_tiles():
    return int(_lib.load().fd_conv2d_f32_num_tiles())


def conv2d_shuffle_nhwc_f32(x, wpk, bias, cout_sub, k, relu=True, out=None, co_off=0, tile=0):
    L = _lib.load()
    x = _dev(x, "x", torch.float32)
    B, H, W, cin = x.shape
    if out is None:
        out = torch.empty((B, H * k, W * k, cout_sub), dtype=torch.float32, device=x.device)
    _dev(out, "out", torch.float32)
    check(L.fd_conv2d_shuffle_nhwc_f32(_p(x), B, H, W, cin, _p(wpk), _p(bias), int(cout_sub), int(k), int(bool(relu)), _p(out), out.shape[3],
                                       co_off, int(tile), _stream()), "fd_conv2d_shuffle_nhwc_f32")
    return out


def conv2d_grouped_nhwc_f32(x, wpk, bias, counts, cin_g, relu=False, out=None, co_off=0, tile=0):
    L = _lib.load()
    x = _dev(x, "x", torch.float32)
    B, H, W, cin = x.shape
    groups = len(counts)
    assert cin == groups * cin_g
    if out is None:
        out = torch.empty((B, H, W, int(sum(counts))), dtype=torch.float32, device=x.device)
    _dev(out, "out", torch.float32)
    check(L.fd_conv2d_grouped_nhwc_f32(_p(x), B, H, W, groups, int(cin_g), _p(wpk), _p(bias), (ctypes.c_int * groups)(*[int(c) for c in counts]),
                                       int(bool(relu)), _p(out), out.shape[3], co_off, int(tile), _stream()), "fd_conv2d_grouped_nhwc_f32")
    return out


def pack_conv2d_weight_wino(w_oihw):
    L = _lib.load()
    dev = w_oihw.device
    w = w_oihw.detach().to("cpu", torch.float32).contiguous()
    cout, cin, ks, _ = w.shape
    nbytes = L.fd_conv2d_wino_f32_packed_weight_bytes(cout, cin) if ks == 3 else 0
    if nbytes == 0:
        raise FutureDetHipError("fd_conv2d_wino_f32: unsupported weight shape %s" % (tuple(w.shape),))
    host = torch.empty((nbytes,), dtype=torch.uint8)
    check(L.fd_conv2d_wino_f32_pack_weight(ctypes.c_void_p(w.data_ptr()), cout, cin, ctypes.c_void_p(host.data_ptr())),
          "fd_conv2d_wino_f32_pack_weight")
    return host.to(dev)


def conv2d_wino_nhwc_f32(x, wpk, bias, cout, relu=True, out=None, co_off=0, tile=0):
    L = _lib.load()
    x = _dev(x, "x", torch.float32)
    B, H, W, cin = x.shape
    if out is None:
        out = torch.empty((B, H, W, cout), dtype=torch.float32, device=x.device)
    _dev(out, "out", torch.float32)
    check(L.fd_conv2d_wino_nhwc_f32(_p(x), B, H, W, cin, _p(wpk), _p(bias), cout, int(bool(relu)), _p(out), out.shape[3], co_off, int(tile),
                                    _stream()), "fd_conv2d_wino_nhwc_f32")
    return out


def conv2d_wino_f32_num_tiles():
    return int(_lib.load().fd_conv2d_wino_f32_num_tiles())


CIRCLE_PRE_MAX = 4096


def pack_deform_adapt(w_cls, w_reg, off_w_cls, off_b_cls, off_w_reg, off_b_reg, bf16):
    L = _lib.load()
    dev = w_cls.device
    wc = w_cls.detach().to("cpu", torch.float32).contiguous()
    wr = w_reg.detach().to("cpu", torch.float32).contiguous()
    if tuple(wc.shape) != (64, 64, 3, 3) or tuple(wr.shape) != (64, 64, 3, 3):
        raise FutureDetHipError("fd_deform_adapt: conv_adaption weights must be [64, 64, 3, 3], got %s / %s" % (tuple(wc.shape), tuple(wr.shape)))
    host = torch.empty((L.fd_deform_adapt_packed_weight_bytes(int(bool(bf16))),), dtype=torch.uint8)
    check(L.fd_deform_adapt_pack_weight(ctypes.c_void_p(wc.data_ptr()), ctypes.c_void_p(wr.data_ptr()), int(bool(bf16)),
                                        ctypes.c_void_p(host.data_ptr())), "fd_deform_adapt_pack_weight")
    ow = torch.stack([off_w_cls.detach().float().reshape(72, 64), off_w_reg.detach().float().reshape(72, 64)]).contiguous()
    ob = torch.stack([off_b_cls.detach().float().reshape(72), off_b_reg.detach().float().reshape(72)]).contiguous()
    return host.to(dev), ow.to(dev), ob.to(dev)


def deform_adapt_nhwc(x, wpk, off_w=None, off_b=None, offsets=None, out=None):
    L = _lib.load()
    if x.dtype not in (torch.float32, torch.bfloat16):
        raise FutureDetHipError("x must be float32 or bfloat16, got %s" % (x.dtype,))
    x = _dev(x, "x")
    B, H, W, C = x.shape
    bf16 = int(x.dtype == torch.bfloat16)
    if offsets is not None:
        _dev(offsets, "offsets", torch.float32)
        if tuple(offsets.shape) != (B, H, W, 144):
            raise FutureDetHipError("offsets must be [B, H, W, 144], got %s" % (tuple(offsets.shape),))
    else:
        if off_w is None or off_b is None:
            raise FutureDetHipError("deform_adapt_nhwc: off_w and off_b are required without offsets")
        _dev(off_w, "off_w", torch.float32)
        _dev(off_b, "off_b", torch.float32)
        if off_w.numel() != 2 * 72 * C or off_b.numel() != 2 * 72:
            raise FutureDetHipError("off_w must be [2, 72, %d] and off_b [2, 72]" % C)
    if wpk.numel() != L.fd_deform_adapt_packed_weight_bytes(bf16):
        raise FutureDetHipError("deform_adapt_nhwc: packed weights are not of this dtype")
    _dev(wpk, "wpk")
    if out is None:
        out = torch.empty((B, H, W, 2 * C), dtype=x.dtype, device=x.device)
    _dev(out, "out", x.dtype)
    if tuple(out.shape) != (B, H, W, 2 * C):
        raise FutureDetHipError("out must be [B, H, W, %d], got %s" % (2 * C, tuple(out.shape)))
    check(L.fd_deform_adapt_nhwc(_p(x), B, H, W, C, bf16, _p(off_w), _p(off_b), _p(offsets), _p(wpk), _p(out), _stream()),
          "fd_deform_adapt_nhwc")
    return out


def _adapt_weight(w, name):
    w = _dev(w.detach(), name, torch.float32)
    if tuple(w.shape) != (64, 64, 3, 3):
        raise FutureDetHipError("fd_deform_adapt: %s must be [64, 64, 3, 3], got %s" % (name, tuple(w.shape)))
    return w


def pack_deform_adapt_device(w_cls, w_reg):
    L = _lib.load()
    wc, wr = _adapt_weight(w_cls, "w_cls"), _adapt_weight(w_reg, "w_reg")
    out = torch.empty((L.fd_deform_adapt_packed_weight_bytes(0),), dtype=torch.uint8, device=wc.device)
    check(L.fd_deform_adapt_pack_weight_device(_p(wc), _p(wr), _p(out), _stream()), "fd_deform_adapt_pack_weight_device")
    return out


def deform_adapt_backward(x, offsets, w_cls, w_reg, y, dy, need=(True, True, True)):
    L = _lib.load()
    x = _dev(x, "x", torch.float32)
    B, H, W, C = x.shape
    for t, name, ch in ((offsets, "offsets", 144), (y, "y", 2 * C), (dy, "dy", 2 * C)):
        _dev(t, name, torch.float32)
        if tuple(t.shape) != (B, H, W, ch):
            raise FutureDetHipError("%s must be [B, H, W, %d], got %s" % (name, ch, tuple(t.shape)))
    wc, wr = _adapt_weight(w_cls, "w_cls"), _adapt_weight(w_reg, "w_reg")
    dx = torch.empty_like(x) if need[0] else None
    doff = torch.empty_like(offsets) if need[1] else None
    dw = torch.empty((2, 64, 64, 3, 3), dtype=torch.float32, device=x.device) if need[2] else None
    ws = workspace.get("deform_adapt_backward", L.fd_deform_adapt_backward_workspace_bytes(B, H, W), x.device)
    check(L.fd_deform_adapt_backward(_p(x), _p(offsets), _p(wc), _p(wr), _p(y), _p(dy), B, H, W, C, _p(dx), _p(doff), _p(dw), _p(ws), ws.numel(),
                                     _stream()), "fd_deform_adapt_backward")
    return dx, doff, dw


def make_decode_cfg(H, W, test_cfg, hm_channels=1, group_radius=None):
    c = DecodeCfg()
    c.hm_channels = int(hm_channels)
    c.H, c.W = int(H), int(W)
    c.out_size_factor = float(test_cfg["out_size_factor"])
    c.voxel_x, c.voxel_y = float(test_cfg["voxel_size"][0]), float(test_cfg["voxel_size"][1])
    c.pc_x, c.pc_y = float(test_cfg["pc_range"][0]), float(test_cfg["pc_range"][1])
    c.score_threshold = float(test_cfg["score_threshold"])
    for i, v in enumerate(test_cfg["post_center_limit_range"]):
        c.center_range[i] = float(v)
    nms = test_cfg["nms"]
    c.nms_iou_threshold = float(nms["nms_iou_threshold"])
    c.nms_pre_max = int(nms["nms_pre_max_size"])
    c.nms_post_max = int(nms["nms_post_max_size"])
    if group_radius is not None:
        if not 1 <= len(group_radius) <= 16:
            raise ValueError("circular NMS: 1..16 decode groups, got %d radii" % len(group_radius))
        c.nms_kind, c.n_radius = 1, len(group_radius)
        c.nms_pre_max = CIRCLE_PRE_MAX
        for i, r in enumerate(group_radius):
            c.circle_radius[i] = float(r)
    return c


def centerpoint_decode(hm, reg, height, dim, rot, cfg):
    L = _lib.load()
    G = hm.shape[0]
    ts = [_dev(t, n, torch.float32) for t, n in ((hm, "hm"), (reg, "reg"), (height, "height"), (dim, "dim"), (rot, "rot"))]
    dev = hm.device
    post = cfg.nms_post_max
    boxes = torch.empty((G, post, 7), dtype=torch.float32, device=dev)
    scores = torch.empty((G, post), dtype=torch.float32, device=dev)
    cell = torch.empty((G, post), dtype=torch.int32, device=dev)
    count = torch.empty((G,), dtype=torch.int32, device=dev)
    ws = workspace.get("decode", L.fd_decode_workspace_bytes(G, ctypes.byref(cfg)), dev)
    args = []
    for t in ts:
        args += [_p(t), t.stride(0)]
    check(L.fd_centerpoint_decode(*args, G, ctypes.byref(cfg), _p(boxes), _p(scores), _p(cell), _p(count), _p(ws),
                                  ws.numel(), _stream()), "fd_centerpoint_decode")
    return boxes, scores, cell, count


def nhwc_channel_view(buf, c0):
    assert buf.is_cuda and buf.is_contiguous() and buf.dim() == 4 and buf.dtype in (torch.float32, torch.bfloat16)
    G, H, W, C = buf.shape
    return MapView(buf.data_ptr() + int(c0) * buf.element_size(), H * W * C, 1, C, 0 if buf.dtype == torch.float32 else 1)


def centerpoint_decode_views(views, G, cfg, device):
    L = _lib.load()
    post = cfg.nms_post_max
    boxes = torch.empty((G, post, 7), dtype=torch.float32, device=device)
    scores = torch.empty((G, post), dtype=torch.float32, device=device)
    cell = torch.empty((G, post), dtype=torch.int32, device=device)
    count = torch.empty((G,), dtype=torch.int32, device=device)
    ws = workspace.get("decode", L.fd_decode_workspace_bytes(G, ctypes.byref(cfg)), device)
    check(L.fd_centerpoint_decode_maps(*[ctypes.byref(v) for v in views], G, ctypes.byref(cfg), _p(boxes), _p(scores), _p(cell), _p(count), _p(ws),
                                       ws.numel(), _stream()), "fd_centerpoint_decode_maps")
    return boxes, scores, cell, count


def centerpoint_decode_packed(views, vel_view, G, B, cfg, device, step_group, step_vel_channel, step_label):
    L = _lib.load()
    post, S = cfg.nms_post_max, len(step_group)
    boxes = torch.empty((G, post, 7), dtype=torch.float32, device=device)
    scores = torch.empty((G, post), dtype=torch.float32, device=device)
    cell = torch.empty((G, post), dtype=torch.int32, device=device)
    count = torch.empty((G,), dtype=torch.int32, device=device)
    packed = torch.empty((B, S, post, 11), dtype=torch.float32, device=device)
    counts = torch.empty((B, S), dtype=torch.int32, device=device)
    ws = workspace.get("decode", L.fd_decode_workspace_bytes(G, ctypes.byref(cfg)), device)
    arr = lambda v: (ctypes.c_int32 * S)(*[int(x) for x in v])
    check(L.fd_centerpoint_decode_packed(*[ctypes.byref(v) for v in views], ctypes.byref(vel_view), int(G), int(B), ctypes.byref(cfg), S, arr(step_group),
                                         arr(step_vel_channel), arr(step_label), _p(boxes), _p(scores), _p(cell), _p(count), _p(packed), _p(counts), _p(ws),
                                         ws.numel(), _stream()), "fd_centerpoint_decode_packed")
    return packed, counts


def assemble_detections(boxes7, scores, cell, count, vel_view, B, post, step_group, step_vel_channel, step_label):
    L = _lib.load()
    S = len(step_group)
    dev = boxes7.device
    packed = torch.empty((B, S, post, 11), dtype=torch.float32, device=dev)
    counts = torch.empty((B, S), dtype=torch.int32, device=dev)
    arr = lambda v: (ctypes.c_int32 * S)(*[int(x) for x in v])
    check(L.fd_assemble_detections(_p(boxes7), _p(scores), _p(cell), _p(count), ctypes.byref(vel_view), int(B), int(post), S, arr(step_group),
                                   arr(step_vel_channel), arr(step_label), _p(packed), _p(counts), _stream()), "fd_assemble_detections")
    return packed, counts


def rotated_nms(boxes7, thresh):
    L = _lib.load()
    boxes7 = _dev(boxes7, "boxes", torch.float32)
    n = boxes7.shape[0]
    keep = torch.zeros((max(n, 1),), dtype=torch.int64, device=boxes7.device)
    count = torch.zeros((1,), dtype=torch.int32, device=boxes7.device)
    ws = workspace.get("nms", L.fd_nms_workspace_bytes(n), boxes7.device)
    check(L.fd_rotated_nms(_p(boxes7), n, ctypes.c_float(thresh), _p(keep), _p(count), _p(ws), ws.numel(), _stream()),
          "fd_rotated_nms")
    return keep, count


def boxes_iou_bev(a, b):
    L = _lib.load()
    a = _dev(a, "boxes_a", torch.float32)
    b = _dev(b, "boxes_b", torch.float32)
    out = torch.zeros((a.shape[0], b.shape[0]), dtype=torch.float32, device=a.device)
    check(L.fd_boxes_iou_bev(_p(a), a.shape[0], _p(b), b.shape[0], _p(out), _stream()), "fd_boxes_iou_bev")
    return out


SWEEP_DESC = np.dtype([("m", np.float64, (16,)), ("row_begin", np.int64), ("row_end", np.int64), ("time", np.float32),
                       ("flags", np.int32)])
SWEEP_HAS_TRANSFORM, SWEEP_REMOVE_CLOSE = 1, 2


def sweep_descriptors(rows, transforms, time_lags, remove_close):
    S = len(rows) - 1
    d = np.zeros((S,), SWEEP_DESC)
    for s in range(S):
        d["row_begin"][s], d["row_end"][s] = int(rows[s]), int(rows[s + 1])
        flags = 0
        if transforms[s] is not None:
            d["m"][s] = np.asarray(transforms[s], np.float64).reshape(16)
            flags |= SWEEP_HAS_TRANSFORM
        if remove_close[s]:
            flags |= SWEEP_REMOVE_CLOSE
        d["flags"][s] = flags
        d["time"][s] = np.float32(np.float64(time_lags[s]))
    return d


def assemble_sweeps(raw, desc, keep_cols=4, min_distance=1.0, out=None, count=None, n_sweeps=None):
    L = _lib.load()
    raw = _dev(raw, "raw", torch.float32)
    R, raw_cols = raw.shape
    dev = raw.device
    if isinstance(desc, torch.Tensor):
        desc_dev = _dev(desc, "desc", torch.uint8)
        n_desc = int(n_sweeps) if n_sweeps is not None else desc_dev.numel() // SWEEP_DESC.itemsize
        assert desc_dev.numel() >= n_desc * SWEEP_DESC.itemsize
    else:
        desc = np.ascontiguousarray(desc)
        assert desc.dtype == SWEEP_DESC
        desc_dev = torch.from_numpy(desc.view(np.uint8).reshape(-1).copy()).to(dev, non_blocking=True)
        n_desc = len(desc)
    if out is None:
        out = torch.empty((R, keep_cols + 1), dtype=torch.float32, device=dev)
    else:
        out = _dev(out, "out", torch.float32)
        assert out.shape[0] >= R and out.shape[1] == keep_cols + 1
    if count is None:
        count = torch.empty((1,), dtype=torch.int32, device=dev)
    ws_bytes = L.fd_sweep_assemble_workspace_bytes(R)
    ws = workspace.get("sweeps", ws_bytes, dev)
    check(L.fd_sweep_assemble(_p(raw), raw_cols, int(keep_cols), R, _p(desc_dev), n_desc, float(min_distance), _p(out),
                              _p(count), _p(ws), ws.numel(), _stream()), "fd_sweep_assemble")
    return out, count


def pillar_encode(voxels, num_points, coors4, n_dev, geom, layers, with_distance=False, out_dtype=torch.float32):
    L = _lib.load()
    voxels = _dev(voxels, "voxels", torch.float32)
    M, P, ndim = voxels.shape
    (w1, s1, b1) = layers[0]
    (w2, s2, b2) = layers[1] if len(layers) > 1 else (None, None, None)
    assert len(layers) in (1, 2)
    U = (w2 if w2 is not None else w1).shape[0]
    out = torch.zeros((M, U), dtype=out_dtype, device=voxels.device)
    check(L.fd_pillar_encode(_p(voxels), _p(num_points), _p(coors4), _p(n_dev), M, P, ndim, int(bool(with_distance)),
                             float(geom[0]), float(geom[1]), float(geom[2]), float(geom[3]), _p(w1), _p(s1), _p(b1), w1.shape[0],
                             _p(w2), _p(s2), _p(b2), (w2.shape[0] if w2 is not None else 0), _DT[out_dtype], _p(out), U, _stream()),
          "fd_pillar_encode")
    return out


def pillar_train_workspace_bytes(m, max_points):
    return int(_lib.load().fd_pillar_train_workspace_bytes(int(m), int(max_points)))


def _pillar_train_args(voxels, num_points, coors4, geom, w1, g1, b1, w2, g2, b2, with_distance):
    voxels = _dev(voxels, "voxels", torch.float32)
    M, P, ndim = voxels.shape
    for t, name in ((w1, "w1"), (g1, "gamma1"), (b1, "beta1"), (w2, "w2"), (g2, "gamma2"), (b2, "beta2")):
        _dev(t, name, torch.float32)
    return [_p(voxels), _p(_dev(num_points, "num_points", torch.int32)), _p(_dev(coors4, "coors4", torch.int32)), M, P, ndim,
            int(bool(with_distance)), float(geom[0]), float(geom[1]), float(geom[2]), float(geom[3])]


def pillar_train_forward(voxels, num_points, coors4, geom, w1, g1, b1, eps1, w2, g2, b2, eps2, with_distance=False, out=None,
                         workspace=None):
    L = _lib.load()
    args = _pillar_train_args(voxels, num_points, coors4, geom, w1, g1, b1, w2, g2, b2, with_distance)
    M, P = args[3], args[4]
    dev = voxels.device
    nbytes = L.fd_pillar_train_workspace_bytes(M, P)
    if workspace is None:
        workspace = torch.empty((max(int(nbytes), 256),), dtype=torch.uint8, device=dev)
    if out is None:
        out = torch.empty((M, w2.shape[0]), dtype=torch.float32, device=dev)
    stats = torch.empty((2 * w1.shape[0] + 2 * w2.shape[0],), dtype=torch.float32, device=dev)
    u1, u2 = w1.shape[0], w2.shape[0]
    mean1, var1, mean2, var2 = stats[:u1], stats[u1:2 * u1], stats[2 * u1:2 * u1 + u2], stats[2 * u1 + u2:]
    check(L.fd_pillar_train_forward(*args, _p(w1), _p(g1), _p(b1), u1, float(eps1), _p(w2), _p(g2), _p(b2), u2, float(eps2),
                                    _p(_dev(out, "out", torch.float32)), _p(mean1), _p(var1), _p(mean2), _p(var2), _p(workspace),
                                    workspace.numel(), _stream()), "fd_pillar_train_forward")
    return out, mean1, var1, mean2, var2, workspace


def pillar_train_backward(dout, voxels, num_points, coors4, geom, w1, g1, b1, w2, g2, b2, workspace, with_distance=False):
    L = _lib.load()
    args = _pillar_train_args(voxels, num_points, coors4, geom, w1, g1, b1, w2, g2, b2, with_distance)
    dout = _dev(dout, "dout", torch.float32)
    assert tuple(dout.shape) == (args[3], w2.shape[0]), (tuple(dout.shape), args[3])
    dw1, dw2 = torch.empty_like(w1), torch.empty_like(w2)
    dg1, db1, dg2, db2 = torch.empty_like(g1), torch.empty_like(b1), torch.empty_like(g2), torch.empty_like(b2)
    check(L.fd_pillar_train_backward(*args, _p(w1), _p(g1), _p(b1), w1.shape[0], _p(w2), _p(g2), _p(b2), w2.shape[0], _p(dout),
                                     _p(dw1), _p(dg1), _p(db1), _p(dw2), _p(dg2), _p(db2), _p(workspace), workspace.numel(), _stream()),
          "fd_pillar_train_backward")
    return dw1, dg1, db1, dw2, dg2, db2


def pillar_scatter_backward(dcanvas, coors4):
    L = _lib.load()
    if not (isinstance(dcanvas, torch.Tensor) and dcanvas.is_cuda and dcanvas.dtype == torch.float32):
        raise FutureDetHipError("pillar_scatter_backward: dcanvas must be a float32 tensor on the HIP device")
    coors4 = _dev(coors4, "coors4", torch.int32)
    n, c = coors4.shape[0], dcanvas.shape[1]
    feats = torch.empty((max(n, 1), c), dtype=torch.float32, device=dcanvas.device)[:n]
    sb, sc, sy, sx = dcanvas.stride()
    check(L.fd_dense_gather(_p(dcanvas), sb, sc, sy, sx, 1, _p(coors4), n, None, c, _p(feats), _stream()), "fd_dense_gather")
    return feats


def pillar_scatter(feats, coors4, n_dev, batch_size, ny, nx, out_dtype=None, channels_last=False, out=None, zero_first=True):
    L = _lib.load()
    feats = _dev(feats, "feats")
    M, C = feats.shape
    if out is None:
        out = torch.empty((batch_size, C, ny, nx), dtype=out_dtype or feats.dtype, device=feats.device,
                          memory_format=torch.channels_last if channels_last else torch.contiguous_format)
    sb, sc, sy, sx = out.stride()
    check(L.fd_pillar_scatter(_p(feats), C, feats.stride(0), _DT[feats.dtype], _p(coors4), _p(n_dev), M, batch_size, ny, nx,
                              _p(out), _DT[out.dtype], sb, sc, sy, sx, int(bool(zero_first)), _stream()), "fd_pillar_scatter")
    return out


def forecast_chains(centers, velocity, counts, time, reject_thresh):
    L = _lib.load()
    centers = _dev(centers, "centers", torch.float64)
    velocity = _dev(velocity, "velocity", torch.float64)
    T, n, _ = centers.shape
    dev = centers.device
    i32 = dict(dtype=torch.int32, device=dev)
    out = dict(fwd_idx=torch.zeros((n, T), **i32), fwd_ok=torch.zeros((n,), **i32), bwd_idx=torch.zeros((n, T), **i32),
               bwd_ok=torch.zeros((n,), **i32), match_idx=torch.zeros((T, n), **i32),
               cv_centers=torch.zeros((n, T, 3), dtype=torch.float64, device=dev), status=torch.zeros((1,), **i32))
    check(L.fd_forecast_chains(_p(centers), _p(velocity), _p(counts), _p(time), T, n, float(reject_thresh), _p(out["fwd_idx"]),
                               _p(out["fwd_ok"]), _p(out["bwd_idx"]), _p(out["bwd_ok"]), _p(out["match_idx"]), _p(out["cv_centers"]),
                               _p(out["status"]), _stream()), "fd_forecast_chains")
    return out


def det_to_global_boxes(box3d, cs_record=None, pose_record=None):
    L = _lib.load()
    box3d = _dev(box3d, "box3d", torch.float32)
    n = box3d.shape[0]
    assert box3d.shape[1] == 9, "box3d_lidar rows are (x,y,z,w,l,h,vx,vy,yaw)"
    dev = box3d.device
    center = torch.empty((n, 3), dtype=torch.float64, device=dev)
    quat = torch.empty((n, 4), dtype=torch.float64, device=dev)
    vel = torch.empty((n, 3), dtype=torch.float64, device=dev)
    size = torch.empty((n, 3), dtype=torch.float32, device=dev)

    def rec(r):
        if r is None:
            return None, None
        q, t = (ctypes.c_double * 4)(*[float(v) for v in r[0]]), (ctypes.c_double * 3)(*[float(v) for v in r[1]])
        return q, t

    cq, ct = rec(cs_record)
    pq, pt = rec(pose_record)
    check(L.fd_det_to_global_boxes(_p(box3d), n, cq, ct, pq, pt, _p(center), _p(quat), _p(vel), _p(size), _stream()), "fd_det_to_global_boxes")
    return center, quat, vel, size


def nearest_rows(library, queries):
    L = _lib.load()
    library, queries = _dev(library, "library", torch.float64), _dev(queries, "queries", torch.float64)
    assert library.shape[1] == queries.shape[1]
    idx = torch.zeros((max(queries.shape[0], 1),), dtype=torch.int32, device=queries.device)[: queries.shape[0]]
    check(L.fd_nearest_rows(_p(library), library.shape[0], _p(queries), queries.shape[0], library.shape[1], _p(idx), _stream()), "fd_nearest_rows")
    return idx


def forecast_groups(centers, match_thresh):
    L = _lib.load()
    centers = _dev(centers, "centers", torch.float64)
    n = centers.shape[0]
    ids = torch.zeros((max(n, 1),), dtype=torch.int32, device=centers.device)[:n]
    check(L.fd_forecast_groups(_p(centers), n, float(match_thresh), _p(ids), _stream()), "fd_forecast_groups")
    return ids


class ForecastOutputs(object):

    FIELDS = (("center", (-1, -2, 3), torch.float64), ("quat", (-1, -2, 4), torch.float64), ("velocity", (-1, -2, 3), torch.float64),
              ("size", (-1, -2, 3), torch.float32), ("fwd_idx", (-3, -1), torch.int32), ("fwd_ok", (-3,), torch.int32),
              ("bwd_idx", (-3, -1), torch.int32), ("bwd_ok", (-3,), torch.int32), ("match_idx", (-1, -3), torch.int32),
              ("cv_centers", (-3, -1, 3), torch.float64), ("status", (), torch.int32), ("traj_kind", (-4,), torch.int32),
              ("traj_src", (-4,), torch.int32), ("traj_first", (-4,), torch.int32), ("traj_group", (-4,), torch.int32), ("n_traj", (), torch.int32))

    def __init__(self, B, T, post, device):
        self.B, self.T, self.post = int(B), int(T), int(post)
        sub = {-1: self.T, -2: self.post, -3: self.post, -4: 3 * self.post}
        layout, off = [], 0
        for name, shape, dt in self.FIELDS:
            shape = (self.B,) + tuple(sub.get(d, d) for d in shape)
            nbytes = int(np.prod(shape)) * torch.empty((), dtype=dt).element_size()
            layout.append((name, shape, dt, off, nbytes))
            off = (off + nbytes + 15) & ~15
        self.layout = layout
        self.blob = torch.zeros((off,), dtype=torch.uint8, device=device)
        for name, shape, dt, o, nbytes in layout:
            setattr(self, name, self.blob[o:o + nbytes].view(dt).view(shape))
        self.c_struct = _lib.ForecastBuffers(**{name: getattr(self, name).data_ptr() for name, _, _ in self.FIELDS})

    def views_of(self, blob_host):
        a = blob_host.numpy() if isinstance(blob_host, torch.Tensor) else np.asarray(blob_host)
        npdt = {torch.float64: np.float64, torch.float32: np.float32, torch.int32: np.int32}
        return {name: a[o:o + nbytes].view(npdt[dt]).reshape(shape) for name, shape, dt, o, nbytes in self.layout}

    def host(self):
        return self.views_of(self.blob.cpu())


def forecast_from_detections(packed, counts, time, records=None, reject_thresh=2.0, match_thresh=0.25, out=None):
    L = _lib.load()
    packed = _dev(packed, "packed", torch.float32)
    counts = _dev(counts, "counts", torch.int32)
    time = _dev(time, "time", torch.float64)
    B, T, post, F = packed.shape
    assert tuple(counts.shape) == (B, T) and tuple(time.shape) == (B, T - 1)
    if records is not None:
        records = _dev(records, "records", torch.float64)
        assert tuple(records.shape) == (B, 14)
    if out is None:
        out = ForecastOutputs(B, T, post, packed.device)
    assert (out.B, out.T, out.post) == (B, T, post)
    check(L.fd_forecast_from_detections(_p(packed), _p(counts), B, T, post, F, _p(records), _p(time), float(reject_thresh), float(match_thresh),
                                        ctypes.byref(out.c_struct), _stream()), "fd_forecast_from_detections")
    return out
```

### futuredet_amd/lib.py

```python
import ctypes
import os

_HERE = os.path.dirname(os.path.abspath(__file__))
LIB_PATH = os.environ.get("FD_LIB_PATH") or os.path.join(_HERE, "libfuturedet_hip.so")
_lib = None

c_void_p = ctypes.c_void_p
c_int = ctypes.c_int
c_i64 = ctypes.c_int64
c_size_t = ctypes.c_size_t
c_float = ctypes.c_float


class MapView(ctypes.Structure):
    _fields_ = [("data", ctypes.c_void_p), ("group_stride", ctypes.c_int64), ("channel_stride", ctypes.c_int64), ("cell_stride", ctypes.c_int64),
                ("dtype", ctypes.c_int)]


ABI_VERSION = 8


class DecodeCfg(ctypes.Structure):
    _fields_ = [("H", c_int), ("W", c_int), ("out_size_factor", c_float), ("voxel_x", c_float), ("voxel_y", c_float),
                ("pc_x", c_float), ("pc_y", c_float), ("score_threshold", c_float), ("center_range", c_float * 6),
                ("nms_iou_threshold", c_float), ("nms_pre_max", c_int), ("nms_post_max", c_int), ("hm_channels", c_int),
                ("nms_kind", c_int), ("n_radius", c_int), ("circle_radius", c_float * 16)]


class IndexLevel(ctypes.Structure):
    _fields_ = [("D", ctypes.c_int32), ("H", ctypes.c_int32), ("W", ctypes.c_int32), ("ksize", ctypes.c_int32 * 3),
                ("stride", ctypes.c_int32 * 3), ("pad", ctypes.c_int32 * 3), ("words", c_void_p), ("prefix", c_void_p),
                ("coords", c_void_p), ("coords_rows", ctypes.c_int64)]


class ForecastBuffers(ctypes.Structure):
    _fields_ = [(n, c_void_p) for n in ("center", "quat", "velocity", "size", "fwd_idx", "fwd_ok", "bwd_idx", "bwd_ok", "match_idx", "cv_centers",
                                        "status", "traj_kind", "traj_src", "traj_first", "traj_group", "n_traj")]


class TargetsCfg(ctypes.Structure):
    _fields_ = [("H", c_int), ("W", c_int), ("T", c_int), ("n_max", c_int), ("max_objs", c_int), ("n_sets", c_int), ("n_tasks", c_int),
                ("task_classes", c_int * 16), ("radius_mult", c_int), ("min_radius", c_int), ("out_size_factor", c_float), ("voxel_x", c_float),
                ("voxel_y", c_float), ("pc_x", c_float), ("pc_y", c_float), ("gaussian_overlap", ctypes.c_double)]


SIGNATURES = {
    "fd_abi_version": (c_int, []),
    "fd_last_error": (ctypes.c_char_p, []),
    "fd_tuning_set": (c_int, [ctypes.c_char_p, c_int]),
    "fd_voxelize_workspace_bytes": (c_size_t, [c_i64, c_i64]),
    "fd_voxelize": (c_int, [c_void_p, c_i64, c_void_p, c_int, c_void_p, c_void_p, c_int, c_i64, c_int, c_void_p, c_void_p, c_int,
                            c_void_p, c_int, c_void_p, c_void_p, c_void_p, c_size_t, c_void_p]),
    "fd_index_num_cols": (c_i64, [c_int, c_int, c_int]),
    "fd_index_workspace_bytes": (c_size_t, [c_i64]),
    "fd_index_mark": (c_int, [c_void_p, c_void_p, c_i64, c_int, c_int, c_int, c_int, c_void_p, c_void_p]),
    "fd_index_downsample": (c_int, [c_void_p, c_int, c_int, c_int, c_int, c_void_p, c_void_p, c_void_p, c_void_p, c_void_p]),
    "fd_index_scan": (c_int, [c_void_p, c_i64, c_void_p, c_void_p, c_void_p, c_size_t, c_void_p]),
    "fd_index_coords": (c_int, [c_void_p, c_void_p, c_int, c_int, c_int, c_int, c_void_p, c_void_p]),
    "fd_index_lookup": (c_int, [c_void_p, c_void_p, c_int, c_int, c_int, c_int, c_void_p, c_void_p, c_i64, c_void_p, c_void_p]),
    "fd_rows_permute": (c_int, [c_void_p, c_int, c_void_p, c_void_p, c_i64, c_void_p, c_int, c_int, c_void_p]),
    "fd_rulebook": (c_int, [c_void_p, c_void_p, c_int, c_int, c_int, c_int, c_void_p, c_i64, c_void_p, c_i64, c_int, c_void_p, c_void_p,
                            c_void_p, c_void_p, c_void_p]),
    "fd_spconv_packed_weight_bytes": (c_size_t, [c_int, c_int, c_int, c_int]),
    "fd_spconv_pack_weight": (c_int, [c_void_p, c_int, c_int, c_int, c_int, c_void_p]),
    "fd_spconv_apply": (c_int, [c_void_p, c_i64, c_void_p, c_void_p, c_void_p, c_int, c_void_p, c_i64, c_void_p, c_int, c_int, c_i64,
                                c_void_p, c_i64, c_int, c_int, c_int, c_void_p, c_void_p]),
    "fd_spconv_num_ranges": (c_int, [c_i64, c_int, c_int, c_int]),
    "fd_spconv_wants_balanced_ranges": (c_int, [c_int, c_int, c_int]),
    "fd_spconv_ranges_workspace_bytes": (c_size_t, [c_i64]),
    "fd_spconv_ranges": (c_int, [c_void_p, c_i64, c_int, c_i64, c_void_p, c_int, c_void_p, c_void_p, c_size_t, c_void_p]),
    "fd_densify": (c_int, [c_void_p, c_int, c_int, c_void_p, c_void_p, c_int, c_int, c_int, c_int, c_void_p, c_int, c_i64,
                           c_i64, c_i64, c_i64, c_i64, c_void_p]),
    "fd_conv2d_packed_weight_bytes": (c_size_t, [c_int, c_int, c_int]),
    "fd_conv2d_pack_weight": (c_int, [c_void_p, c_int, c_int, c_int, c_void_p]),
    "fd_conv2d_nhwc_bf16": (c_int, [c_void_p, c_int, c_int, c_int, c_int, c_void_p, c_void_p, c_int, c_int, c_int, c_int, c_int,
                                    c_void_p, c_int, c_int, c_int, c_int, c_int, c_int, c_void_p]),
    "fd_conv2d_f32_packed_weight_bytes": (c_size_t, [c_int, c_int, c_int]),
    "fd_conv2d_f32_pack_weight": (c_int, [c_void_p, c_int, c_int, c_int, c_void_p]),
    "fd_conv2d_f32_num_tiles": (c_int, []),
    "fd_conv2d_nhwc_f32": (c_int, [c_void_p, c_int, c_int, c_int, c_int, c_void_p, c_void_p, c_int, c_int, c_int, c_int, c_int,
                                   c_void_p, c_int, c_int, c_int, c_int, c_int, c_int, c_int, c_void_p]),
    "fd_conv2d_shuffle_nhwc_f32": (c_int, [c_void_p, c_int, c_int, c_int, c_int, c_void_p, c_void_p, c_int, c_int, c_int, c_void_p, c_int, c_int, c_int,
                                           c_void_p]),
    "fd_conv2d_grouped_nhwc_f32": (c_int, [c_void_p, c_int, c_int, c_int, c_int, c_int, c_void_p, c_void_p, c_void_p, c_int, c_void_p, c_int, c_int,
                                           c_int, c_void_p]),
    "fd_conv2d_wino_f32_num_tiles": (c_int, []),
    "fd_conv2d_wino_f32_packed_weight_bytes": (c_size_t, [c_int, c_int]),
    "fd_conv2d_wino_f32_pack_weight": (c_int, [c_void_p, c_int, c_int, c_void_p]),
    "fd_conv2d_wino_nhwc_f32": (c_int, [c_void_p, c_int, c_int, c_int, c_int, c_void_p, c_void_p, c_int, c_int, c_void_p, c_int, c_int, c_int,
                                        c_void_p]),
    "fd_decode_workspace_bytes": (c_size_t, [c_int, ctypes.POINTER(DecodeCfg)]),
    "fd_centerpoint_decode": (c_int, [c_void_p, c_i64, c_void_p, c_i64, c_void_p, c_i64, c_void_p, c_i64, c_void_p, c_i64,
                                      c_int, ctypes.POINTER(DecodeCfg), c_void_p, c_void_p, c_void_p, c_void_p, c_void_p,
                                      c_size_t, c_void_p]),
    "fd_centerpoint_decode_maps": (c_int, [ctypes.POINTER(MapView)] * 5 + [c_int, ctypes.POINTER(DecodeCfg), c_void_p, c_void_p, c_void_p, c_void_p,
                                           c_void_p, c_size_t, c_void_p]),
    "fd_centerpoint_decode_packed": (c_int, [ctypes.POINTER(MapView)] * 6 + [c_int, c_int, ctypes.POINTER(DecodeCfg), c_int, c_void_p, c_void_p, c_void_p,
                                             c_void_p, c_void_p, c_void_p, c_void_p, c_void_p, c_void_p, c_void_p, c_size_t, c_void_p]),
    "fd_assemble_detections": (c_int, [c_void_p, c_void_p, c_void_p, c_void_p, ctypes.POINTER(MapView), c_int, c_int, c_int, c_void_p, c_void_p,
                                       c_void_p, c_void_p, c_void_p, c_void_p]),
    "fd_nms_workspace_bytes": (c_size_t, [c_int]),
    "fd_rotated_nms": (c_int, [c_void_p, c_int, c_float, c_void_p, c_void_p, c_void_p, c_size_t, c_void_p]),
    "fd_boxes_iou_bev": (c_int, [c_void_p, c_int, c_void_p, c_int, c_void_p, c_void_p]),
    "fd_pillar_encode": (c_int, [c_void_p, c_void_p, c_void_p, c_void_p, c_i64, c_int, c_int, c_int, c_float, c_float, c_float,
                                 c_float, c_void_p, c_void_p, c_void_p, c_int, c_void_p, c_void_p, c_void_p, c_int, c_int,
                                 c_void_p, c_int, c_void_p]),
    "fd_pillar_scatter": (c_int, [c_void_p, c_int, c_int, c_int, c_void_p, c_void_p, c_i64, c_int, c_int, c_int, c_void_p, c_int,
                                  c_i64, c_i64, c_i64, c_i64, c_int, c_void_p]),
    "fd_forecast_chains": (c_int, [c_void_p, c_void_p, c_void_p, c_void_p, c_int, c_int, ctypes.c_double, c_void_p, c_void_p,
                                   c_void_p, c_void_p, c_void_p, c_void_p, c_void_p, c_void_p]),
    "fd_det_to_global_boxes": (c_int, [c_void_p, c_int, c_void_p, c_void_p, c_void_p, c_void_p, c_void_p, c_void_p, c_void_p, c_void_p, c_void_p]),
    "fd_forecast_groups": (c_int, [c_void_p, c_int, ctypes.c_double, c_void_p, c_void_p]),
    "fd_forecast_from_detections": (c_int, [c_void_p, c_void_p, c_int, c_int, c_int, c_int, c_void_p, c_void_p, ctypes.c_double, ctypes.c_double,
                                            ctypes.POINTER(ForecastBuffers), c_void_p]),
    "fd_nearest_rows": (c_int, [c_void_p, c_int, c_void_p, c_int, c_int, c_void_p, c_void_p]),
    "fd_index_pyramid": (c_int, [c_void_p, c_void_p, c_i64, c_int, c_int, ctypes.POINTER(IndexLevel), c_void_p, c_void_p, c_size_t,
                                 c_void_p]),
    "fd_index_pyramid_coords": (c_int, [c_int, c_int, ctypes.POINTER(IndexLevel), c_void_p]),
    "fd_rows_place": (c_int, [c_void_p, c_void_p, c_int, c_int, c_int, c_int, c_void_p, c_void_p, c_i64, c_void_p, c_int, c_void_p,
                              c_int, c_int, c_void_p]),
    "fd_sweep_assemble_workspace_bytes": (c_size_t, [c_i64]),
    "fd_sweep_assemble": (c_int, [c_void_p, c_int, c_int, c_i64, c_void_p, c_int, c_float, c_void_p, c_void_p, c_void_p,
                                  c_size_t, c_void_p]),
    "fd_deform_adapt_packed_weight_bytes": (c_size_t, [c_int]),
    "fd_deform_adapt_pack_weight": (c_int, [c_void_p, c_void_p, c_int, c_void_p]),
    "fd_deform_adapt_nhwc": (c_int, [c_void_p, c_int, c_int, c_int, c_int, c_int, c_void_p, c_void_p, c_void_p, c_void_p, c_void_p, c_void_p]),
    "fd_deform_adapt_backward_workspace_bytes": (c_size_t, [c_int, c_int, c_int]),
    "fd_deform_adapt_backward": (c_int, [c_void_p, c_void_p, c_void_p, c_void_p, c_void_p, c_void_p, c_int, c_int, c_int, c_int, c_void_p, c_void_p,
                                         c_void_p, c_void_p, c_size_t, c_void_p]),
    "fd_deform_adapt_pack_weight_device": (c_int, [c_void_p, c_void_p, c_void_p, c_void_p]),
    "fd_spconv_wgrad_workspace_bytes": (c_size_t, [c_int, c_i64, c_int, c_int]),
    "fd_spconv_wgrad": (c_int, [c_void_p, c_i64, c_void_p, c_void_p, c_i64, c_int, c_i64, c_void_p, c_int, c_int, c_void_p, c_void_p, c_size_t,
                                c_void_p]),
    "fd_rulebook_transpose": (c_int, [c_void_p, c_i64, c_int, c_i64, c_void_p, c_i64, c_void_p, c_i64, c_void_p]),
    "fd_spconv_pack_weight_device": (c_int, [c_void_p, c_int, c_int, c_int, c_int, c_void_p, c_void_p]),
    "fd_dense_gather": (c_int, [c_void_p, c_i64, c_i64, c_i64, c_i64, c_int, c_void_p, c_i64, c_void_p, c_int, c_void_p, c_void_p]),
    "fd_pillar_train_workspace_bytes": (c_size_t, [c_i64, c_int]),
    "fd_pillar_train_forward": (c_int, [c_void_p, c_void_p, c_void_p, c_i64, c_int, c_int, c_int, c_float, c_float, c_float, c_float,
                                        c_void_p, c_void_p, c_void_p, c_int, c_float, c_void_p, c_void_p, c_void_p, c_int, c_float,
                                        c_void_p, c_void_p, c_void_p, c_void_p, c_void_p, c_void_p, c_size_t, c_void_p]),
    "fd_pillar_train_backward": (c_int, [c_void_p, c_void_p, c_void_p, c_i64, c_int, c_int, c_int, c_float, c_float, c_float, c_float,
                                         c_void_p, c_void_p, c_void_p, c_int, c_void_p, c_void_p, c_void_p, c_int, c_void_p,
                                         c_void_p, c_void_p, c_void_p, c_void_p, c_void_p, c_void_p, c_void_p, c_size_t, c_void_p]),
    "fd_targets_workspace_bytes": (c_size_t, [c_int, c_int, c_int, c_int]),
    "fd_assign_targets": (c_int, [c_void_p, c_void_p, c_void_p, c_void_p, c_int, ctypes.POINTER(TargetsCfg), c_void_p, c_void_p, c_void_p, c_void_p,
                                  c_void_p, c_void_p, c_void_p, c_void_p, c_size_t, c_void_p]),
}


class FutureDetHipError(RuntimeError):
    pass


def load():
    global _lib
    if _lib is None:
        if not os.path.isfile(LIB_PATH):
            raise FutureDetHipError(
                "libfuturedet_hip.so is not built (%s). Run `python -c 'import __graft_entry__ as g; g.build()'` "
                "or `python futuredet_amd/build.py`; there is no CPU fallback for this path." % LIB_PATH)
        L = ctypes.CDLL(LIB_PATH)
        for name, (res, args) in SIGNATURES.items():
            fn = getattr(L, name)
            fn.restype = res
            fn.argtypes = args
        if L.fd_abi_version() != ABI_VERSION:
            raise FutureDetHipError("%s reports ABI %d, these bindings are written for %d: rebuild it (python futuredet_amd/build.py --force)"
                                    % (LIB_PATH, L.fd_abi_version(), ABI_VERSION))
        _lib = L
    return _lib


def check(status, what):
    if status != 0:
        msg = load().fd_last_error()
        raise FutureDetHipError("%s failed (%d): %s" % (what, status, msg.decode() if msg else "?"))
```

### include/futuredet_hip.h

```cpp
#ifndef FUTUREDET_HIP_H
#define FUTUREDET_HIP_H

#include <stddef.h>
#include <stdint.h>

#ifdef __cplusplus
extern "C" {
#endif

#define FD_OK 0
#define FD_EINVAL (-1)
#define FD_EWORKSPACE (-2)
#define FD_ELAUNCH (-3)

typedef void *fd_stream_t;

int fd_abi_version(void);
const char *fd_last_error(void);
int fd_tuning_set(const char *name, int value);

size_t fd_voxelize_workspace_bytes(int64_t n_points, int64_t max_voxels);
int fd_voxelize(const float *points, int64_t n_points, const int32_t *n_points_dev, int ndim, const float *range6_host,
                const float *voxel_size3_host, int max_points, int64_t max_voxels, int batch_idx,
                float *out_voxels, float *out_mean, int mean_stride, int32_t *out_coors, int coor_cols,
                int32_t *out_num_points, int32_t *out_num_voxels, void *workspace, size_t workspace_bytes,
                fd_stream_t stream);

int64_t fd_index_num_cols(int B, int H, int W);
size_t fd_index_workspace_bytes(int64_t num_cols);
int fd_index_mark(const int32_t *coords , const int32_t *n_dev ,
                  int64_t n_max, int B, int D, int H, int W, uint64_t *words, fd_stream_t stream);
int fd_index_downsample(const uint64_t *in_words, int B, int D, int H, int W, const int *ksize3,
                        const int *stride3, const int *pad3, uint64_t *out_words, fd_stream_t stream);
int fd_index_scan(const uint64_t *words, int64_t num_cols, int32_t *prefix, int32_t *n_active_dev,
                  void *workspace, size_t workspace_bytes, fd_stream_t stream);
int fd_index_coords(const uint64_t *words, const int32_t *prefix, int B, int D, int H, int W,
                    int32_t *coords , fd_stream_t stream);
int fd_index_lookup(const uint64_t *words, const int32_t *prefix, int B, int D, int H, int W,
                    const int32_t *coords_in, const int32_t *n_dev, int64_t n_max, int32_t *row_of,
                    fd_stream_t stream);
int fd_rows_permute(const float *src, int c_src, const int32_t *row_of, const int32_t *n_dev, int64_t n_max,
                    void *dst, int c_dst, int dst_bf16, fd_stream_t stream);
int fd_rulebook(const uint64_t *in_words, const int32_t *in_prefix, int B, int Din, int Hin, int Win,
                const int32_t *out_coords, int64_t out_rows, const int32_t *n_out_dev, int64_t nbr_stride, int fill_tail, const int *ksize3,
                const int *stride3, const int *pad3, int32_t *nbr, fd_stream_t stream);

size_t fd_spconv_packed_weight_bytes(int K, int cin, int cout, int dtype);
int fd_spconv_pack_weight(const float *w_kio_host, int K, int cin, int cout, int dtype, void *wpacked_host);
int fd_spconv_apply(const void *in_feats, int64_t n_in, const void *wpacked, const float *bias, const void *residual,
                    int relu, const int32_t *nbr, int64_t nbr_stride, const int32_t *ranges ,
                    int n_ranges, int K, int64_t n_out, const int32_t *n_out_dev ,
                    int64_t n_expected ,
                    int cin, int cout, int dtype, void *out_feats, fd_stream_t stream);
int fd_spconv_num_ranges(int64_t n_out, int cin, int cout, int dtype);
int fd_spconv_wants_balanced_ranges(int cin, int cout, int dtype);
size_t fd_spconv_ranges_workspace_bytes(int64_t n_out);
int fd_spconv_ranges(const int32_t *nbr, int64_t nbr_stride, int K, int64_t n_out, const int32_t *n_out_dev, int n_ranges,
                     int32_t *ranges , void *workspace, size_t workspace_bytes, fd_stream_t stream);

int fd_densify(const void *feats, int c, int dtype, const uint64_t *words, const int32_t *prefix, int B, int D,
               int H, int W, void *out, int out_dtype, int64_t stride_b, int64_t stride_c, int64_t stride_y,
               int64_t stride_x, int64_t n_rows ,
               fd_stream_t stream);

size_t fd_conv2d_packed_weight_bytes(int cout, int cin, int ks);
int fd_conv2d_pack_weight(const float *w_oihw_host, int cout, int cin, int ks, void *wpacked_host);
int fd_conv2d_nhwc_bf16(const void *x, int B, int H, int W, int cin, const void *wpacked, const float *bias, int cout,
                        int ks, int stride, int pad, int relu, void *y, int cout_total, int co_off, int osy, int osx,
                        int ooy, int oox, fd_stream_t stream);
size_t fd_conv2d_f32_packed_weight_bytes(int cout, int cin, int ks);
int fd_conv2d_f32_pack_weight(const float *w_oihw_host, int cout, int cin, int ks, void *wpacked_host);
int fd_conv2d_f32_num_tiles(void);
int fd_conv2d_nhwc_f32(const float *x, int B, int H, int W, int cin, const void *wpacked, const float *bias, int cout, int ks,
                       int stride, int pad, int relu, float *y, int cout_total, int co_off, int osy, int osx, int ooy, int oox,
                       int tile , fd_stream_t stream);
int fd_conv2d_shuffle_nhwc_f32(const float *x, int B, int H, int W, int cin, const void *wpacked, const float *bias, int cout_sub, int k,
                               int relu, float *y, int cout_total, int co_off, int tile, fd_stream_t stream);
int fd_conv2d_grouped_nhwc_f32(const float *x, int B, int H, int W, int groups, int cin_g, const void *wpacked, const float *bias,
                               const int *counts_host, int relu, float *y, int cout_total, int co_off, int tile, fd_stream_t stream);
int fd_conv2d_wino_f32_num_tiles(void);
size_t fd_conv2d_wino_f32_packed_weight_bytes(int cout, int cin);
int fd_conv2d_wino_f32_pack_weight(const float *w_oihw_host, int cout, int cin, void *wpacked_host);
int fd_conv2d_wino_nhwc_f32(const float *x, int B, int H, int W, int cin, const void *wpacked, const float *bias, int cout, int relu,
                            float *y, int cout_total, int co_off, int tile , fd_stream_t stream);

typedef struct fd_decode_cfg {
    int H, W;
    float out_size_factor, voxel_x, voxel_y, pc_x, pc_y;
    float score_threshold;
    float center_range[6];
    float nms_iou_threshold;
    int nms_pre_max, nms_post_max;
    int hm_channels;
    int nms_kind;
    int n_radius;
    float circle_radius[16];
} fd_decode_cfg;

typedef struct fd_map_view {
    const void *data;
    int64_t group_stride, channel_stride, cell_stride;
    int dtype;
} fd_map_view;

size_t fd_decode_workspace_bytes(int G, const fd_decode_cfg *cfg);
int fd_centerpoint_decode_maps(const fd_map_view *hm, const fd_map_view *reg, const fd_map_view *height, const fd_map_view *dim,
                               const fd_map_view *rot, int G, const fd_decode_cfg *cfg_host, float *out_boxes7, float *out_scores,
                               int32_t *out_cell, int32_t *out_count, void *workspace, size_t workspace_bytes, fd_stream_t stream);
int fd_assemble_detections(const float *boxes7, const float *scores, const int32_t *cell, const int32_t *count, const fd_map_view *vel,
                           int B, int post_max, int S, const int32_t *step_group, const int32_t *step_vel_channel,
                           const int32_t *step_label, float *packed, int32_t *counts_out, fd_stream_t stream);
int fd_centerpoint_decode_packed(const fd_map_view *hm, const fd_map_view *reg, const fd_map_view *height, const fd_map_view *dim,
                                 const fd_map_view *rot, const fd_map_view *vel, int G, int B, const fd_decode_cfg *cfg_host, int S,
                                 const int32_t *step_group, const int32_t *step_vel_channel, const int32_t *step_label, float *out_boxes7,
                                 float *out_scores, int32_t *out_cell, int32_t *out_count, float *packed, int32_t *counts_out, void *workspace,
                                 size_t workspace_bytes, fd_stream_t stream);
int fd_centerpoint_decode(const float *hm, int64_t hm_gstride, const float *reg, int64_t reg_gstride,
                          const float *height, int64_t height_gstride, const float *dim, int64_t dim_gstride,
                          const float *rot, int64_t rot_gstride, int G, const fd_decode_cfg *cfg_host,
                          float *out_boxes7, float *out_scores, int32_t *out_cell, int32_t *out_count,
                          void *workspace, size_t workspace_bytes, fd_stream_t stream);

size_t fd_nms_workspace_bytes(int n);
int fd_rotated_nms(const float *boxes7, int n, float thresh, int64_t *keep, int32_t *out_count,
                   void *workspace, size_t workspace_bytes, fd_stream_t stream);
int fd_boxes_iou_bev(const float *a7, int na, const float *b7, int nb, float *out, fd_stream_t stream);

#define FD_SWEEP_HAS_TRANSFORM 1
#define FD_SWEEP_REMOVE_CLOSE 2
typedef struct fd_sweep_desc {
    double m[16];
    int64_t row_begin, row_end;
    float time;
    int32_t flags;
} fd_sweep_desc;
size_t fd_sweep_assemble_workspace_bytes(int64_t n_rows);
int fd_sweep_assemble(const float *raw, int raw_cols, int keep_cols, int64_t n_rows, const fd_sweep_desc *sweeps_dev,
                      int n_sweeps, float min_distance, float *out_points, int32_t *out_count, void *workspace,
                      size_t workspace_bytes, fd_stream_t stream);

int fd_pillar_encode(const float *voxels, const int32_t *num_points, const int32_t *coors4, const int32_t *n_dev,
                     int64_t m_max, int max_points, int ndim, int with_distance, float vx, float vy, float x_offset,
                     float y_offset, const float *w1, const float *scale1, const float *shift1, int units1,
                     const float *w2, const float *scale2, const float *shift2, int units2, int out_dtype, void *out,
                     int out_stride, fd_stream_t stream);

int fd_pillar_scatter(const void *feats, int c, int feat_stride, int dtype, const int32_t *coors4, const int32_t *n_dev,
                      int64_t m_max, int B, int H, int W, void *out, int out_dtype, int64_t stride_b, int64_t stride_c,
                      int64_t stride_y, int64_t stride_x, int zero_first, fd_stream_t stream);


int fd_forecast_chains(const double *centers, const double *velocity, const int32_t *counts, const double *time_dev, int T,
                       int n_max, double reject_thresh, int32_t *fwd_idx, int32_t *fwd_ok, int32_t *bwd_idx, int32_t *bwd_ok,
                       int32_t *match_idx, double *cv_centers, int32_t *status, fd_stream_t stream);

int fd_det_to_global_boxes(const float *box3d9, int n, const double *cs_rotation4_host, const double *cs_translation3_host,
                           const double *pose_rotation4_host, const double *pose_translation3_host, double *center,
                           double *quat, double *velocity, float *size, fd_stream_t stream);
int fd_forecast_groups(const double *centers3, int n, double match_thresh, int32_t *ids, fd_stream_t stream);

typedef struct fd_forecast_buffers {
    double *center, *quat, *velocity;
    float *size;
    int32_t *fwd_idx, *fwd_ok, *bwd_idx, *bwd_ok, *match_idx;
    double *cv_centers;
    int32_t *status;
    int32_t *traj_kind, *traj_src, *traj_first, *traj_group, *n_traj;
} fd_forecast_buffers;
int fd_forecast_from_detections(const float *packed, const int32_t *counts, int B, int T, int post, int row_floats,
                                const double *records_dev, const double *time_dev, double reject_thresh, double match_thresh,
                                const fd_forecast_buffers *out, fd_stream_t stream);

int fd_nearest_rows(const double *library, int n_library, const double *queries, int n_queries, int dim, int32_t *idx, fd_stream_t stream);

typedef struct fd_index_level {
    int32_t D, H, W;
    int32_t ksize[3], stride[3], pad[3];
    uint64_t *words;
    int32_t *prefix;
    int32_t *coords;
    int64_t coords_rows;
} fd_index_level;
int fd_index_pyramid(const int32_t *coords, const int32_t *n_dev, int64_t n_max_per_sample, int B, int n_levels,
                     const fd_index_level *levels_host, int32_t *counts_dev, void *workspace, size_t workspace_bytes,
                     fd_stream_t stream);
int fd_index_pyramid_coords(int B, int n_levels, const fd_index_level *levels_host, fd_stream_t stream);

int fd_rows_place(const uint64_t *words, const int32_t *prefix, int B, int D, int H, int W, const int32_t *coords_in,
                  const int32_t *n_dev, int64_t n_max, const float *src, int c_src, void *dst, int c_dst, int dst_bf16,
                  fd_stream_t stream);

size_t fd_deform_adapt_packed_weight_bytes(int bf16);
int fd_deform_adapt_pack_weight(const float *w_cls_oihw_host, const float *w_reg_oihw_host, int bf16, void *wpacked_host);
int fd_deform_adapt_nhwc(const void *x, int B, int H, int W, int C, int bf16, const float *off_w, const float *off_b, const float *offsets,
                         const void *wpacked, void *y, fd_stream_t stream);

size_t fd_deform_adapt_backward_workspace_bytes(int B, int H, int W);
int fd_deform_adapt_backward(const float *x, const float *offsets, const float *w_cls_oihw, const float *w_reg_oihw, const float *y, const float *dy,
                             int B, int H, int W, int C, float *dx, float *doffsets, float *dw, void *workspace, size_t workspace_bytes,
                             fd_stream_t stream);
int fd_deform_adapt_pack_weight_device(const float *w_cls_oihw, const float *w_reg_oihw, void *wpacked, fd_stream_t stream);

size_t fd_spconv_wgrad_workspace_bytes(int K, int64_t n_out, int cin, int cout);
int fd_spconv_wgrad(const float *in_feats, int64_t n_in, const float *dy, const int32_t *nbr, int64_t nbr_stride, int K, int64_t n_out,
                    const int32_t *n_out_dev, int cin, int cout, float *dw, void *workspace, size_t workspace_bytes, fd_stream_t stream);
int fd_rulebook_transpose(const int32_t *nbr, int64_t nbr_stride, int K, int64_t n_out, const int32_t *n_out_dev, int64_t n_in, int32_t *inv,
                          int64_t inv_stride, fd_stream_t stream);
int fd_spconv_pack_weight_device(const float *w_kio, int K, int cin, int cout, int mode, void *wpacked, fd_stream_t stream);
int fd_dense_gather(const float *dense, int64_t stride_b, int64_t stride_c, int64_t stride_y, int64_t stride_x, int D, const int32_t *coords,
                    int64_t n_rows, const int32_t *n_dev, int c, float *feats, fd_stream_t stream);

#define FD_TARGETS_MAX_TASKS 16
typedef struct fd_targets_cfg {
    int H, W;
    int T, n_max, max_objs;
    int n_sets;
    int n_tasks;
    int task_classes[FD_TARGETS_MAX_TASKS];
    int radius_mult;
    int min_radius;
    float out_size_factor, voxel_x, voxel_y, pc_x, pc_y;
    double gaussian_overlap;
} fd_targets_cfg;
size_t fd_targets_workspace_bytes(int B, int T, int maps_per_step, int max_objs);
int fd_assign_targets(const float *boxes, const int32_t *counts, const int32_t *classes, const int32_t *trajectory, int B,
                      const fd_targets_cfg *cfg, float *hm, int64_t *ind, uint8_t *mask, int64_t *cat, float *anno_box,
                      float *gt_boxes_and_cls, int32_t *status, void *workspace, size_t workspace_bytes, fd_stream_t stream);

size_t fd_pillar_train_workspace_bytes(int64_t m, int max_points);
int fd_pillar_train_forward(const float *voxels, const int32_t *num_points, const int32_t *coors4, int64_t m, int max_points, int ndim,
                            int with_distance, float vx, float vy, float x_offset, float y_offset, const float *w1, const float *gamma1,
                            const float *beta1, int units1, float eps1, const float *w2, const float *gamma2, const float *beta2, int units2,
                            float eps2, float *out, float *mean1, float *var1, float *mean2, float *var2, void *workspace,
                            size_t workspace_bytes, fd_stream_t stream);
int fd_pillar_train_backward(const float *voxels, const int32_t *num_points, const int32_t *coors4, int64_t m, int max_points, int ndim,
                             int with_distance, float vx, float vy, float x_offset, float y_offset, const float *w1, const float *gamma1,
                             const float *beta1, int units1, const float *w2, const float *gamma2, const float *beta2, int units2,
                             const float *dout, float *dw1, float *dgamma1, float *dbeta1, float *dw2, float *dgamma2, float *dbeta2,
                             void *workspace, size_t workspace_bytes, fd_stream_t stream);

#ifdef __cplusplus
}
#endif
#endif
```

Measured before the change: 281.1.

## Prebuild per-rulebook chunk images to skip tap compaction in f32 subm convs

Adds a chunk image builder that precomputes the compacted per-chunk tap lists and counts for each 27-tap submanifold rulebook. The f32 c32 and compact kernels get an IMAGE variant that loads this record instead of staging the raw neighbor slice and running compact_taps with an extra barrier. Images are built once per rulebook, on the side stream when forking, and reused by the two convs in each residual block. The cost is an extra build kernel per rulebook plus extra device memory, and it adds more kernel variants.

```diff
diff --git a/futuredet_amd/backbones.py b/futuredet_amd/backbones.py
--- a/futuredet_amd/backbones.py
+++ b/futuredet_amd/backbones.py
@@ -127,6 +127,8 @@
             wpk, bias, cin_p, cout_p = conv.packed_weight(dt, bn)
             assert x.shape[1] == cin_p, (x.shape, cin_p)
             nbr = rulebook(src, dst, conv)
+            if src is dst and dt == torch.float32 and cin_p == cout_p:
+                hip_ops.image_for(nbr, cin_p, cout_p)
             fn = lambda: hip_ops.spconv_apply(x, wpk, bias, nbr, dst.n, cout_p, residual=residual, relu=relu)
             if self.profile_hook is not None:
                 s = 4 if dt == torch.float32 else 2
@@ -160,6 +162,10 @@
                             r = hip_ops.ranges_for(nbr, cp, cp)
                             if r[0] is not None:
                                 made.append(r[0])
+                        if dt == torch.float32:
+                            img = hip_ops.image_for(nbr, cp, cp)
+                            if img is not None:
+                                made.append(img[0])
                 for t in made:
                     t.record_stream(main)
         x = feats0
diff --git a/futuredet_amd/csrc/fd_common.h b/futuredet_amd/csrc/fd_common.h
--- a/futuredet_amd/csrc/fd_common.h
+++ b/futuredet_amd/csrc/fd_common.h
@@ -12,7 +12,8 @@
 void set_error(const char *fmt, ...);
 int spconv_f32_compact_dispatch(const float *in, const void *wp, const float *bias, const float *residual, int relu, const int *nbr,
                                 int64_t nbr_stride, int K, int64_t n_in_bound, int n_out, const int *n_out_dev, int cin, int cout, float *out,
-                                const int *ranges, int n_ranges, hipStream_t stream);
+                                const int *ranges, int n_ranges, const void *image, hipStream_t stream);
+size_t spconv_image_min_bytes(int64_t n_out, int n_ranges);
 
 size_t spconv_bf16_win_weight_bytes(int K, int cin, int cout);
 void spconv_bf16_win_pack(const float *w, int K, int cin, int cout, uint16_t (*tobf)(float), uint16_t *dst);
@@ -29,7 +30,7 @@
 
 int spconv_f32_c32_dispatch(const float *in, const void *wp, const float *bias, const float *residual, int relu, const int *nbr,
                             int64_t nbr_stride, int K, int64_t n_in_bound, int n_out, const int *n_out_dev, int cin, int cout, float *out,
-                            const int *ranges, int n_ranges, hipStream_t stream);
+                            const int *ranges, int n_ranges, const void *image, hipStream_t stream);
 
 __device__ __forceinline__ int device_count(int capacity, const int *count_dev) {
     if (!count_dev) return capacity;
@@ -63,7 +64,7 @@
 int current_device();
 int device_cu_count();
 bool ensure_dynamic_lds(const void *kernel, size_t bytes, std::atomic<uint64_t> &done);
-enum TuneKey { kTuneSpconvRG = 0, kTuneSpconvV1, kTuneSpconvBf16V1, kTuneV2Depth, kTuneV2TM, kTuneV2LdsPad, kTuneConvNT, kTuneV2RangesPerCU, kTuneV2Uniform, kTuneV2RowCost, kTuneSpconvC32, kTuneBf16GP, kTuneBf16RG, kTuneBf16Depth, kTuneBf16NW, kTuneStrict, kTuneBf16Win, kTuneF32ResRG, kTuneConvStrip, kTuneF32ResNW, kTuneCount };
+enum TuneKey { kTuneSpconvRG = 0, kTuneSpconvV1, kTuneSpconvBf16V1, kTuneV2Depth, kTuneV2TM, kTuneV2LdsPad, kTuneConvNT, kTuneV2RangesPerCU, kTuneV2Uniform, kTuneV2RowCost, kTuneSpconvC32, kTuneBf16GP, kTuneBf16RG, kTuneBf16Depth, kTuneBf16NW, kTuneStrict, kTuneBf16Win, kTuneF32ResRG, kTuneConvStrip, kTuneF32ResNW, kTuneSpconvImage, kTuneCount };
 int tuning(TuneKey key);
 
 inline size_t align_up(size_t v, size_t a) { return (v + a - 1) / a * a; }
diff --git a/futuredet_amd/csrc/fd_error.hip b/futuredet_amd/csrc/fd_error.hip
--- a/futuredet_amd/csrc/fd_error.hip
+++ b/futuredet_amd/csrc/fd_error.hip
@@ -54,7 +54,7 @@
     std::atomic<int> v[kTuneCount];
     TuneTable() {
         static const char *const env[kTuneCount] = {"FD_SPCONV_RG", "FD_SPCONV_V1", "FD_SPCONV_BF16_V1", "FD_V2_DEPTH", "FD_V2_TM",
-                                                    "FD_V2_LDSPAD", "FD_CONV_NT", "FD_V2_RANGES_PER_CU", "FD_V2_UNIFORM", "FD_V2_ROWCOST", "FD_SPCONV_C32", "FD_BF16_GP", "FD_BF16_RG", "FD_BF16_DEPTH", "FD_BF16_NW", "FD_STRICT", "FD_BF16_WIN", "FD_F32_RES_RG", "FD_CONV_STRIP", "FD_F32_RES_NW"};
+                                                    "FD_V2_LDSPAD", "FD_CONV_NT", "FD_V2_RANGES_PER_CU", "FD_V2_UNIFORM", "FD_V2_ROWCOST", "FD_SPCONV_C32", "FD_BF16_GP", "FD_BF16_RG", "FD_BF16_DEPTH", "FD_BF16_NW", "FD_STRICT", "FD_BF16_WIN", "FD_F32_RES_RG", "FD_CONV_STRIP", "FD_F32_RES_NW", "FD_SPCONV_IMAGE"};
         for (int i = 0; i < kTuneCount; ++i) {
             const char *e = getenv(env[i]);
             v[i].store(e ? atoi(e) : 0, std::memory_order_relaxed);
@@ -65,7 +65,7 @@
     static TuneTable t;
     return t;
 }
-const char *const kTuneNames[kTuneCount] = {"spconv_rg", "spconv_v1", "spconv_bf16_v1", "v2_depth", "v2_tm", "v2_ldspad", "conv_nt", "v2_ranges_per_cu", "v2_uniform", "v2_rowcost", "spconv_c32", "bf16_gp", "bf16_rg", "bf16_depth", "bf16_nw", "strict", "bf16_win", "f32_res_rg", "conv_strip", "f32_res_nw"};
+const char *const kTuneNames[kTuneCount] = {"spconv_rg", "spconv_v1", "spconv_bf16_v1", "v2_depth", "v2_tm", "v2_ldspad", "conv_nt", "v2_ranges_per_cu", "v2_uniform", "v2_rowcost", "spconv_c32", "bf16_gp", "bf16_rg", "bf16_depth", "bf16_nw", "strict", "bf16_win", "f32_res_rg", "conv_strip", "f32_res_nw", "spconv_image"};
 }
 
 int tuning(TuneKey key) { return tune_table().v[key].load(std::memory_order_relaxed); }
diff --git a/futuredet_amd/csrc/fd_spconv.hip b/futuredet_amd/csrc/fd_spconv.hip
--- a/futuredet_amd/csrc/fd_spconv.hip
+++ b/futuredet_amd/csrc/fd_spconv.hip
@@ -314,9 +314,10 @@
     return FD_OK;
 }
 
-extern "C" int fd_spconv_apply(const void *in_feats, int64_t n_in, const void *wpacked, const float *bias, const void *residual, int relu,
-                               const int32_t *nbr, int64_t nbr_stride, const int32_t *ranges, int n_ranges, int K, int64_t n_out,
-                               const int32_t *n_out_dev, int64_t n_expected, int cin, int cout, int dtype, void *out_feats, fd_stream_t stream) {
+static int spconv_apply_impl(const void *in_feats, int64_t n_in, const void *wpacked, const float *bias, const void *residual, int relu,
+                             const int32_t *nbr, int64_t nbr_stride, const int32_t *ranges, int n_ranges, int K, int64_t n_out,
+                             const int32_t *n_out_dev, int64_t n_expected, int cin, int cout, int dtype, void *out_feats, const void *image,
+                             fd_stream_t stream) {
     FD_REQUIRE(K >= 1 && K <= kMaxTaps, "fd_spconv_apply: K must be in [1,27]");
     FD_REQUIRE(dtype == 0 || dtype == 1, "fd_spconv_apply: dtype must be 0 (f32) or 1 (bf16)");
     FD_REQUIRE(n_out >= 0 && n_out <= nbr_stride && n_out < (1ll << 31), "fd_spconv_apply: n_out out of range");
@@ -332,12 +333,12 @@
     if (dtype == 0 && !fd::tuning(fd::kTuneSpconvV1) && has_c32_layout(cin, cout, dtype) && fd::tuning(fd::kTuneSpconvC32) >= 0) {
         const void *w32 = (const char *)wpacked + (size_t)K * cin * cout * 4;
         if (fd::spconv_f32_c32_dispatch((const float *)in_feats, w32, bias, (const float *)residual, relu, nbr, nbr_stride, K, n_in, (int)n_out,
-                                        n_out_dev, cin, cout, (float *)out_feats, ranges, n_ranges, fd::as_stream(stream)))
+                                        n_out_dev, cin, cout, (float *)out_feats, ranges, n_ranges, image, fd::as_stream(stream)))
             return fd::check_launch("fd_spconv_apply(c32)");
     }
     if (dtype == 0 && !fd::tuning(fd::kTuneSpconvV1)) {
         if (fd::spconv_f32_compact_dispatch((const float *)in_feats, wpacked, bias, (const float *)residual, relu, nbr, nbr_stride, K, n_in,
-                                            (int)n_out, n_out_dev, cin, cout, (float *)out_feats, ranges, n_ranges, fd::as_stream(stream)))
+                                            (int)n_out, n_out_dev, cin, cout, (float *)out_feats, ranges, n_ranges, image, fd::as_stream(stream)))
             return fd::check_launch("fd_spconv_apply(compact)");
     }
     if (dtype == 1 && fd::tuning(fd::kTuneBf16GP) >= 0) {
@@ -372,3 +373,24 @@
     }
     return fd::check_launch("fd_spconv_apply");
 }
+
+extern "C" int fd_spconv_apply(const void *in_feats, int64_t n_in, const void *wpacked, const float *bias, const void *residual, int relu,
+                               const int32_t *nbr, int64_t nbr_stride, const int32_t *ranges, int n_ranges, int K, int64_t n_out,
+                               const int32_t *n_out_dev, int64_t n_expected, int cin, int cout, int dtype, void *out_feats, fd_stream_t stream) {
+    return spconv_apply_impl(in_feats, n_in, wpacked, bias, residual, relu, nbr, nbr_stride, ranges, n_ranges, K, n_out, n_out_dev, n_expected, cin, cout,
+                             dtype, out_feats, nullptr, stream);
+}
+
+extern "C" int fd_spconv_apply_image(const void *in_feats, int64_t n_in, const void *wpacked, const float *bias, const void *residual, int relu,
+                                     const int32_t *nbr, int64_t nbr_stride, const int32_t *ranges, int n_ranges, int K, int64_t n_out,
+                                     const int32_t *n_out_dev, int64_t n_expected, int cin, int cout, int dtype, void *out_feats, const void *image,
+                                     size_t image_bytes, fd_stream_t stream) {
+    FD_REQUIRE(image && ((uintptr_t)image & 15) == 0, "fd_spconv_apply_image: the image must be a 16-byte aligned device buffer");
+    FD_REQUIRE(dtype == 0 && K == kMaxTaps && cin == cout && (cin == 32 || cin == 64 || cin == 128),
+               "fd_spconv_apply_image: no image kernel for %d -> %d, K = %d, dtype %d", cin, cout, K, dtype);
+    FD_REQUIRE(n_out >= 0 && n_out < (1ll << 31) && n_ranges >= 0, "fd_spconv_apply_image: bad sizes");
+    FD_REQUIRE(n_out == 0 || image_bytes >= fd::spconv_image_min_bytes(n_out, n_ranges), "fd_spconv_apply_image: image too small for %lld rows in %d ranges",
+               (long long)n_out, n_ranges);
+    return spconv_apply_impl(in_feats, n_in, wpacked, bias, residual, relu, nbr, nbr_stride, ranges, n_ranges, K, n_out, n_out_dev, n_expected, cin, cout,
+                             dtype, out_feats, image, stream);
+}
diff --git a/futuredet_amd/csrc/fd_spconv_c32.hip b/futuredet_amd/csrc/fd_spconv_c32.hip
--- a/futuredet_amd/csrc/fd_spconv_c32.hip
+++ b/futuredet_amd/csrc/fd_spconv_c32.hip
@@ -9,7 +9,7 @@
 constexpr sk::Layout L = sk::layout(TM, COUT, TS, 32);
 static_assert(((sk::kMaxTaps + TS - 1) / TS) * (TM / WR / 32) <= L.item_slot, "item list slot");
 
-template <int CIN, int DEPTH>
+template <int CIN, int DEPTH, bool IMAGE = false>
 __global__ void __launch_bounds__(256) spconv_f32_c32(const float *__restrict__ in, const float4 *__restrict__ wp, const float *__restrict__ bias,
                                                       const float *__restrict__ residual, int relu, const int *__restrict__ nbr, int64_t nbr_stride,
                                                       int K, int n_out, const int *__restrict__ n_out_dev, float *__restrict__ out, unsigned in_bytes,
@@ -29,7 +29,10 @@
     if (r_begin >= r_end) return;
     sk::cut_chunks<TM>(r_begin, r_end, n_chunks, chunk_rows);
     int pre[sk::kSliceRegs<TM>];
-    sk::fetch_slice<TM>(pre, nbr, nbr_stride, K, r_begin);
+    sk::image_vec rec[sk::kImageRegs<TM>];
+    const sk::image_vec *image = reinterpret_cast<const sk::image_vec *>(nbr);
+    if constexpr (IMAGE) sk::fetch_record<TM>(rec, sk::image_record<TM>(image, r_begin, 0));
+    else sk::fetch_slice<TM>(pre, nbr, nbr_stride, K, r_begin);
 
     const int ln = lane & 31, lh = lane >> 5;
     const int ts = wave, wr = 0;
@@ -40,11 +43,18 @@
     for (int chunk = 0; chunk < n_chunks; ++chunk) {
         int row0, n_rows;
         if (!sk::chunk_span(r_begin, r_end, chunk_rows, chunk, row0, n_rows)) break;
-        sk::stage_chunk<TM, COUT, TS, 32>(pre, s_list, s_pad, s_acc, bias, residual, K, row0, n_rows);
+        if constexpr (IMAGE) {
+            sk::stage_record<TM, COUT, TS, 32>(rec, s_list, s_cnt, s_pad, s_acc, bias, residual, row0, n_rows);
+        } else {
+            sk::stage_chunk<TM, COUT, TS, 32>(pre, s_list, s_pad, s_acc, bias, residual, K, row0, n_rows);
+            __syncthreads();
+            sk::compact_taps<TM, WR>(s_list, s_cnt, K);
+        }
         __syncthreads();
-        sk::compact_taps<TM, WR>(s_list, s_cnt, K);
-        __syncthreads();
-        if (chunk + 1 < n_chunks) sk::fetch_slice<TM>(pre, nbr, nbr_stride, K, row0 + chunk_rows);
+        if (chunk + 1 < n_chunks) {
+            if constexpr (IMAGE) sk::fetch_record<TM>(rec, sk::image_record<TM>(image, r_begin, chunk + 1));
+            else sk::fetch_slice<TM>(pre, nbr, nbr_stride, K, row0 + chunk_rows);
+        }
         const int n_items = sk::build_items<TS, 32>(s_cnt, items, K, ts, wr);
 
         int k_r[DEPTH], row_r[DEPTH];
@@ -123,14 +133,14 @@
     }
 }
 
-template <int CIN, int DEPTH>
+template <int CIN, int DEPTH, bool IMAGE = false>
 int launch_c32(const float *in, const void *wp, const float *bias, const float *residual, int relu, const int *nbr, int64_t nbr_stride, int K,
                int n_out, const int *n_out_dev, float *out, unsigned in_bytes, const int *ranges, int n_ranges, hipStream_t stream) {
     int rows_per = 0;
     if (!ranges) sk::equal_rows_split(n_out, TM, n_out_dev != nullptr, n_ranges, rows_per);
     static std::atomic<uint64_t> lds_set{0};
-    if (!fd::ensure_dynamic_lds(reinterpret_cast<const void *>(spconv_f32_c32<CIN, DEPTH>), (size_t)L.bytes, lds_set)) return 0;
-    hipLaunchKernelGGL((spconv_f32_c32<CIN, DEPTH>), dim3((unsigned)n_ranges), dim3(256), (size_t)L.bytes, stream, in, (const float4 *)wp, bias, residual, relu,
+    if (!fd::ensure_dynamic_lds(reinterpret_cast<const void *>(spconv_f32_c32<CIN, DEPTH, IMAGE>), (size_t)L.bytes, lds_set)) return 0;
+    hipLaunchKernelGGL((spconv_f32_c32<CIN, DEPTH, IMAGE>), dim3((unsigned)n_ranges), dim3(256), (size_t)L.bytes, stream, in, (const float4 *)wp, bias, residual, relu,
                        nbr, nbr_stride, K, n_out, n_out_dev, out, in_bytes, ranges, rows_per);
     return 1;
 }
@@ -140,11 +150,13 @@
 namespace fd {
 int spconv_f32_c32_dispatch(const float *in, const void *wp, const float *bias, const float *residual, int relu, const int *nbr, int64_t nbr_stride,
                             int K, int64_t n_in_bound, int n_out, const int *n_out_dev, int cin, int cout, float *out, const int *ranges,
-                            int n_ranges, hipStream_t stream) {
+                            int n_ranges, const void *image, hipStream_t stream) {
     if (cout != 32 || cin != 32) return 0;
     if (!sk::entries_fit(n_in_bound, cin)) return 0;
     const unsigned in_bytes = (unsigned)(n_in_bound * cin * 4);
     const int depth = fd::tuning(fd::kTuneV2Depth);
+    if (image && K == sk::kMaxTaps && (depth == 0 || depth == 3))
+        return launch_c32<32, 3, true>(in, wp, bias, residual, relu, (const int *)image, nbr_stride, K, n_out, n_out_dev, out, in_bytes, ranges, n_ranges, stream);
     if (depth == 2) return launch_c32<32, 2>(in, wp, bias, residual, relu, nbr, nbr_stride, K, n_out, n_out_dev, out, in_bytes, ranges, n_ranges, stream);
     if (depth == 4) return launch_c32<32, 4>(in, wp, bias, residual, relu, nbr, nbr_stride, K, n_out, n_out_dev, out, in_bytes, ranges, n_ranges, stream);
     return launch_c32<32, 3>(in, wp, bias, residual, relu, nbr, nbr_stride, K, n_out, n_out_dev, out, in_bytes, ranges, n_ranges, stream);
diff --git a/futuredet_amd/csrc/fd_spconv_chunk.h b/futuredet_amd/csrc/fd_spconv_chunk.h
--- a/futuredet_amd/csrc/fd_spconv_chunk.h
+++ b/futuredet_amd/csrc/fd_spconv_chunk.h
@@ -142,17 +142,23 @@
     }
 }
 
+template <int TM>
+__device__ __forceinline__ void stage_list(const int (&pre)[kSliceRegs<TM>], int *s_list, int K, int n_rows) {
+    const int tid = threadIdx.x;
+    static_assert(256 % TM == 0, "a thread stages the same local row in every pass");
+    const bool in_chunk = tid % TM < n_rows;
+#pragma unroll
+    for (int i = 0; i < kSliceRegs<TM>; ++i) {
+        const int t = tid + i * 256;
+        if (t < K * TM) s_list[t] = in_chunk ? pre[i] : -1;
+    }
+}
+
 template <int TM, int COUT, int TS, int ITEM>
 __device__ __forceinline__ void stage_chunk(const int (&pre)[kSliceRegs<TM>], int *s_list, int *s_pad, float *s_acc, const float *bias,
                                             const float *residual, int K, int row0, int n_rows) {
     const int tid = threadIdx.x;
-    static_assert(256 % TM == 0, "a thread stages the same local row in every pass");
-    const bool in_chunk = tid % TM < n_rows;
-#pragma unroll
-    for (int i = 0; i < kSliceRegs<TM>; ++i) {
-        const int t = tid + i * 256;
-        if (t < K * TM) s_list[t] = in_chunk ? pre[i] : -1;
-    }
+    stage_list<TM>(pre, s_list, K, n_rows);
     init_acc<TM, COUT, TS>(s_acc, bias, residual, row0, n_rows);
     if (tid < ITEM) s_pad[tid] = pad_entry(TM);
 }
@@ -188,6 +194,51 @@
             if (lane == 0) s_cnt[k * 4 + wr] = (unsigned char)count;
         }
     }
+}
+
+constexpr int kImageCntBytes = 128;
+typedef int image_vec __attribute__((ext_vector_type(4)));
+template <int TM>
+constexpr int kImageRecVecs = (kMaxTaps * TM * 4 + kImageCntBytes) / 16;
+template <int TM>
+constexpr int kImageListVecs = kMaxTaps * TM / 4;
+constexpr int kImageCntVecs = 112 / 16;
+template <int TM>
+constexpr int kImageRegs = (kImageRecVecs<TM> + 255) / 256;
+inline int64_t image_records(int64_t n_out, int tm, int64_t n_ranges) { return n_ranges + n_out / tm + 1; }
+inline size_t image_bytes(int64_t n_out, int tm, int64_t n_ranges) {
+    return (size_t)image_records(n_out, tm, n_ranges) * (size_t)(kMaxTaps * tm * 4 + kImageCntBytes);
+}
+template <int TM>
+__device__ __forceinline__ const image_vec *image_record(const image_vec *image, int r_begin, int chunk) {
+    return image + ((int64_t)blockIdx.x + r_begin / TM + chunk) * kImageRecVecs<TM>;
+}
+template <int TM>
+__device__ __forceinline__ void fetch_record(image_vec (&rec)[kImageRegs<TM>], const image_vec *record) {
+    const int tid = threadIdx.x;
+#pragma unroll
+    for (int i = 0; i < kImageRegs<TM>; ++i) {
+        const int t = tid + i * 256;
+        rec[i] = record[t < kImageRecVecs<TM> ? t : kImageRecVecs<TM> - 1];
+    }
+}
+template <int TM, int COUT, int TS, int ITEM>
+__device__ __forceinline__ void stage_record(const image_vec (&rec)[kImageRegs<TM>], int *s_list, unsigned char *s_cnt, int *s_pad, float *s_acc,
+                                             const float *bias, const float *residual, int row0, int n_rows) {
+    const int tid = threadIdx.x;
+#pragma unroll
+    for (int i = 0; i < kImageRegs<TM>; ++i) {
+        const int t = tid + i * 256;
+        if (t < kImageListVecs<TM>) reinterpret_cast<image_vec *>(s_list)[t] = rec[i];
+        else if (t < kImageListVecs<TM> + kImageCntVecs) reinterpret_cast<image_vec *>(s_cnt)[t - kImageListVecs<TM>] = rec[i];
+    }
+    init_acc<TM, COUT, TS>(s_acc, bias, residual, row0, n_rows);
+    if (tid < ITEM) s_pad[tid] = pad_entry(TM);
+}
+template <int TM>
+__device__ __forceinline__ void store_record(image_vec *record, const int *s_list, const unsigned char *s_cnt) {
+    for (int t = threadIdx.x; t < kImageRecVecs<TM>; t += 256)
+        record[t] = t < kImageListVecs<TM> ? reinterpret_cast<const image_vec *>(s_list)[t] : reinterpret_cast<const image_vec *>(s_cnt)[t - kImageListVecs<TM>];
 }
 
 template <int TS, int ITEM>
diff --git a/futuredet_amd/csrc/fd_spconv_v2.hip b/futuredet_amd/csrc/fd_spconv_v2.hip
--- a/futuredet_amd/csrc/fd_spconv_v2.hip
+++ b/futuredet_amd/csrc/fd_spconv_v2.hip
@@ -25,7 +25,7 @@
 
 constexpr int tap_splits(int cout) { return (cout == 32 || cout == 64) ? 2 : 1; }
 
-template <int CIN, int COUT, int TM, int DEPTH>
+template <int CIN, int COUT, int TM, int DEPTH, bool IMAGE = false>
 __global__ void __launch_bounds__(256) spconv_f32_compact(const float *__restrict__ in, const float4 *__restrict__ wp,
                                                           const float *__restrict__ bias, const float *__restrict__ residual, int relu,
                                                           const int *__restrict__ nbr, int64_t nbr_stride, int K, int n_out,
@@ -54,7 +54,10 @@
     FD_T(0);
     sk::cut_chunks<TM>(r_begin, r_end, n_chunks, chunk_rows);
     int pre[sk::kSliceRegs<TM>];
-    sk::fetch_slice<TM>(pre, nbr, nbr_stride, K, r_begin);
+    sk::image_vec rec[sk::kImageRegs<TM>];
+    const sk::image_vec *image = reinterpret_cast<const sk::image_vec *>(nbr);
+    if constexpr (IMAGE) sk::fetch_record<TM>(rec, sk::image_record<TM>(image, r_begin, 0));
+    else sk::fetch_slice<TM>(pre, nbr, nbr_stride, K, r_begin);
 
     const int lrow = lane & 15, lq = lane >> 4;
     const int wc = wave % WC, wr = TS == 1 ? wave / WC : 0, ts = TS == 1 ? 0 : wave / WC;
@@ -67,13 +70,20 @@
     for (int chunk = 0; chunk < n_chunks; ++chunk) {
     int row0, n_rows;
     if (!sk::chunk_span(r_begin, r_end, chunk_rows, chunk, row0, n_rows)) break;
-    sk::stage_chunk<TM, COUT, TS, 16>(pre, s_list, s_pad, s_acc, bias, residual, K, row0, n_rows);
-    __syncthreads();
-    if (chunk == 0) FD_T(1);
-    sk::compact_taps<TM, WR>(s_list, s_cnt, K);
+    if constexpr (IMAGE) {
+        sk::stage_record<TM, COUT, TS, 16>(rec, s_list, s_cnt, s_pad, s_acc, bias, residual, row0, n_rows);
+    } else {
+        sk::stage_chunk<TM, COUT, TS, 16>(pre, s_list, s_pad, s_acc, bias, residual, K, row0, n_rows);
+        __syncthreads();
+        if (chunk == 0) FD_T(1);
+        sk::compact_taps<TM, WR>(s_list, s_cnt, K);
+    }
     __syncthreads();
     if (chunk == 0) FD_T(2);
-    if (chunk + 1 < n_chunks) sk::fetch_slice<TM>(pre, nbr, nbr_stride, K, row0 + chunk_rows);
+    if (chunk + 1 < n_chunks) {
+        if constexpr (IMAGE) sk::fetch_record<TM>(rec, sk::image_record<TM>(image, r_begin, chunk + 1));
+        else sk::fetch_slice<TM>(pre, nbr, nbr_stride, K, row0 + chunk_rows);
+    }
     const int n_items = sk::build_items<TS, 16>(s_cnt, items, K, ts, wr);
 
     int k_r[DEPTH];
@@ -195,13 +205,13 @@
     return (cin == 64 && cout == 64 && tm == 128 && lds < 56 * 1024) ? (size_t)56 * 1024 : lds;
 }
 
-template <int CIN, int COUT, int TM, int DEPTH>
+template <int CIN, int COUT, int TM, int DEPTH, bool IMAGE = false>
 int launch_compact(const float *in, const void *wp, const float *bias, const float *residual, int relu, const int *nbr,
                    int64_t nbr_stride, int K, int n_out, const int *n_out_dev, float *out, unsigned in_bytes, const int *ranges, int n_ranges,
                    hipStream_t stream) {
     const size_t lds_req = lds_request(CIN, COUT, TM);
     static std::atomic<uint64_t> lds_set{0};
-    auto kern = spconv_f32_compact<CIN, COUT, TM, DEPTH>;
+    auto kern = spconv_f32_compact<CIN, COUT, TM, DEPTH, IMAGE>;
     if (fd::tuning(fd::kTuneV2LdsPad)) {
         if (hipFuncSetAttribute(reinterpret_cast<const void *>(kern), hipFuncAttributeMaxDynamicSharedMemorySize, (int)lds_req) != hipSuccess) {
             (void)hipGetLastError();
@@ -216,6 +226,40 @@
                        n_out, n_out_dev, out, in_bytes, ranges, rows_per);
     return 1;
 }
+
+template <int TM, int WR>
+__global__ void __launch_bounds__(256) chunk_image_kernel(const int *__restrict__ nbr, int64_t nbr_stride, int K, int n_out,
+                                                          const int *__restrict__ n_out_dev, const int *__restrict__ ranges, int rows_per_range,
+                                                          sk::image_vec *__restrict__ image) {
+    __shared__ __attribute__((aligned(16))) int s_list[sk::kMaxTaps * TM];
+    __shared__ __attribute__((aligned(16))) unsigned char s_cnt[sk::kImageCntBytes];
+    int r_begin, r_end, n_chunks, chunk_rows;
+    sk::resolve_range(n_out, n_out_dev, ranges, rows_per_range, r_begin, r_end);
+    if (r_begin >= r_end) return;
+    sk::cut_chunks<TM>(r_begin, r_end, n_chunks, chunk_rows);
+    int pre[sk::kSliceRegs<TM>];
+    sk::fetch_slice<TM>(pre, nbr, nbr_stride, K, r_begin);
+    if (threadIdx.x < sk::kImageCntBytes / 4) reinterpret_cast<int *>(s_cnt)[threadIdx.x] = 0;
+    for (int chunk = 0; chunk < n_chunks; ++chunk) {
+        int row0, n_rows;
+        if (!sk::chunk_span(r_begin, r_end, chunk_rows, chunk, row0, n_rows)) break;
+        sk::stage_list<TM>(pre, s_list, K, n_rows);
+        __syncthreads();
+        sk::compact_taps<TM, WR>(s_list, s_cnt, K);
+        __syncthreads();
+        if (chunk + 1 < n_chunks) sk::fetch_slice<TM>(pre, nbr, nbr_stride, K, row0 + chunk_rows);
+        sk::store_record<TM>(const_cast<sk::image_vec *>(sk::image_record<TM>(image, r_begin, chunk)), s_list, s_cnt);
+        __syncthreads();
+    }
+}
+
+constexpr int kImageTM = 128;
+inline int image_family(int cin, int cout, int dtype) {
+    if (dtype != 0 || cin != cout) return 0;
+    return cin == 32 ? 1 : cin == 64 ? 2 : cin == 128 ? 4 : 0;
+}
+constexpr int kImageDefault = 1 | 2 | 4;
+inline int64_t image_grid_bound(int64_t n_out, int n_ranges) { return n_ranges > 0 ? n_ranges : (n_out + kImageTM - 1) / kImageTM; }
 
 constexpr int kWorkRows = 8;
 constexpr int kRowCost = 24;
@@ -382,13 +426,46 @@
     return fd::check_launch("fd_spconv_ranges");
 }
 
+extern "C" size_t fd_spconv_image_bytes(int64_t n_out, int cin, int cout, int dtype, int n_ranges) {
+    const int fam = image_family(cin, cout, dtype);
+    if (!fam || n_out <= 0 || n_out >= (1ll << 31) || fd::tuning(fd::kTuneSpconvV1)) return 0;
+    const int sel = fd::tuning(fd::kTuneSpconvImage);
+    if (!((sel == 0 ? kImageDefault : sel < 0 ? 0 : sel) & fam)) return 0;
+    return sk::image_bytes(n_out, kImageTM, image_grid_bound(n_out, n_ranges));
+}
+
+extern "C" int fd_spconv_image_build(const int32_t *nbr, int64_t nbr_stride, int K, int64_t n_out, const int32_t *n_out_dev, const int32_t *ranges,
+                                     int n_ranges, int cin, int cout, void *image, size_t image_bytes, fd_stream_t stream_) {
+    FD_REQUIRE(nbr && image, "fd_spconv_image_build: null argument");
+    FD_REQUIRE(K == sk::kMaxTaps, "fd_spconv_image_build: the chunk image holds all 27 taps (K = %d)", K);
+    FD_REQUIRE(image_family(cin, cout, 0), "fd_spconv_image_build: no image kernel for %d -> %d", cin, cout);
+    FD_REQUIRE(n_out > 0 && n_out <= nbr_stride && n_out < (1ll << 31), "fd_spconv_image_build: bad sizes");
+    FD_REQUIRE(n_ranges >= 0 && (ranges == nullptr || n_ranges >= 1), "fd_spconv_image_build: ranges needs n_ranges >= 1");
+    FD_REQUIRE(((uintptr_t)image & 15) == 0, "fd_spconv_image_build: the image must be 16-byte aligned");
+    FD_REQUIRE(image_bytes >= sk::image_bytes(n_out, kImageTM, image_grid_bound(n_out, n_ranges)), "fd_spconv_image_build: image too small");
+    int rows_per = 0;
+    if (!ranges) sk::equal_rows_split((int)n_out, kImageTM, n_out_dev != nullptr, n_ranges, rows_per);
+    hipLaunchKernelGGL((chunk_image_kernel<kImageTM, 1>), dim3((unsigned)n_ranges), dim3(256), 0, fd::as_stream(stream_), nbr, nbr_stride, K, (int)n_out,
+                       n_out_dev, ranges, rows_per, (sk::image_vec *)image);
+    return fd::check_launch("fd_spconv_image_build");
+}
+
 namespace fd {
+size_t spconv_image_min_bytes(int64_t n_out, int n_ranges) { return sk::image_bytes(n_out, kImageTM, image_grid_bound(n_out, n_ranges)); }
+
 int spconv_f32_compact_dispatch(const float *in, const void *wp, const float *bias, const float *residual, int relu, const int *nbr,
                                 int64_t nbr_stride, int K, int64_t n_in_bound, int n_out, const int *n_out_dev, int cin, int cout, float *out,
-                                const int *ranges, int n_ranges, hipStream_t stream) {
+                                const int *ranges, int n_ranges, const void *image, hipStream_t stream) {
     if (!sk::entries_fit(n_in_bound, cin)) return 0;
     const unsigned in_bytes = (unsigned)(n_in_bound * cin * 4);
     const int dsel = fd::tuning(fd::kTuneV2Depth), tsel = fd::tuning(fd::kTuneV2TM);
+    if (image && K == sk::kMaxTaps && (tsel == 0 || tsel == 128)) {
+        const int *img = (const int *)image;
+        if (cin == 64 && cout == 64 && (dsel == 0 || dsel == 3))
+            return launch_compact<64, 64, 128, 3, true>(in, wp, bias, residual, relu, img, nbr_stride, K, n_out, n_out_dev, out, in_bytes, ranges, n_ranges, stream);
+        if (cin == 128 && cout == 128 && (dsel == 0 || dsel == 2))
+            return launch_compact<128, 128, 128, 2, true>(in, wp, bias, residual, relu, img, nbr_stride, K, n_out, n_out_dev, out, in_bytes, ranges, n_ranges, stream);
+    }
 #define FD_LAUNCH(CI, CO, T, D) \
     launch_compact<CI, CO, T, D>(in, wp, bias, residual, relu, nbr, nbr_stride, K, n_out, n_out_dev, out, in_bytes, ranges, n_ranges, stream)
 #define FD_CASE(CI, CO, DDEF, TDEF)                                  \
diff --git a/futuredet_amd/hip_ops.py b/futuredet_amd/hip_ops.py
--- a/futuredet_amd/hip_ops.py
+++ b/futuredet_amd/hip_ops.py
@@ -283,6 +283,40 @@
     return nbr.ranges
 
 
+def _split_for(nbr, cin, cout, balanced=None):
+    L = _lib.load()
+    K = nbr.shape[0]
+    n_out = getattr(nbr, "n_out", None) or 0
+    if balanced is None:
+        balanced = K == 27 and cin == cout and bool(L.fd_spconv_wants_balanced_ranges(cin, cout, 0))
+    if balanced == "tiles":
+        return None, 0
+    if balanced:
+        return ranges_for(nbr, cin, cout)
+    return None, int(L.fd_spconv_num_ranges(getattr(nbr, "n_expected", 0) or n_out, cin, cout, 0))
+
+
+def image_for(nbr, cin, cout, balanced=None):
+    cached = getattr(nbr, "image", None)
+    if cached is not None:
+        return cached or None
+    L = _lib.load()
+    n_out = getattr(nbr, "n_out", None)
+    K, nstride = nbr.shape
+    nbr.image = False
+    if not n_out or K != 27:
+        return None
+    ranges, n = _split_for(nbr, cin, cout, balanced)
+    nbytes = int(L.fd_spconv_image_bytes(n_out, cin, cout, 0, n))
+    if not nbytes:
+        return None
+    image = torch.empty((nbytes,), dtype=torch.uint8, device=nbr.device)
+    check(L.fd_spconv_image_build(_p(nbr), nstride, K, n_out, _p(getattr(nbr, "n_dev", None)), _p(ranges), n, cin, cout, _p(image), nbytes,
+                                  _stream()), "fd_spconv_image_build")
+    nbr.image = (image, cin, cout, ranges, n)
+    return nbr.image
+
+
 def rows_permute(src, row_of, c_dst, dtype=torch.float32, n_rows=None, n_dev=None):
     L = _lib.load()
     src = _dev(src, "src", torch.float32)
@@ -416,6 +450,12 @@
             ranges, n_ranges = ranges_for(nbr, cin, cout)
         else:
             n_ranges = int(L.fd_spconv_num_ranges(n_expected or n_out, cin, cout, 0))
+        img = getattr(nbr, "image", None)
+        if img and img[1:3] == (cin, cout) and img[3] is ranges and img[4] == n_ranges and getattr(nbr, "n_out", None) == n_out:
+            check(L.fd_spconv_apply_image(_p(feats), feats.shape[0], _p(_dev(wpacked, "wpacked")), _p(bias), _p(residual), int(bool(relu)),
+                                          _p(nbr), nstride, _p(ranges), n_ranges, K, n_out, _p(n_dev), int(n_expected or 0), cin, cout, dt,
+                                          _p(out), _p(img[0]), img[0].numel(), _stream()), "fd_spconv_apply_image")
+            return out
     check(L.fd_spconv_apply(_p(feats), feats.shape[0], _p(_dev(wpacked, "wpacked")), _p(bias), _p(residual), int(bool(relu)),
                             _p(_dev(nbr, "nbr", torch.int32)), nstride, _p(ranges), n_ranges, K, n_out, _p(n_dev), int(n_expected or 0),
                             cin, cout, dt, _p(out), _stream()),
diff --git a/futuredet_amd/lib.py b/futuredet_amd/lib.py
--- a/futuredet_amd/lib.py
+++ b/futuredet_amd/lib.py
@@ -69,6 +69,10 @@
     "fd_spconv_wants_balanced_ranges": (c_int, [c_int, c_int, c_int]),
     "fd_spconv_ranges_workspace_bytes": (c_size_t, [c_i64]),
     "fd_spconv_ranges": (c_int, [c_void_p, c_i64, c_int, c_i64, c_void_p, c_int, c_void_p, c_void_p, c_size_t, c_void_p]),
+    "fd_spconv_image_bytes": (c_size_t, [c_i64, c_int, c_int, c_int, c_int]),
+    "fd_spconv_image_build": (c_int, [c_void_p, c_i64, c_int, c_i64, c_void_p, c_void_p, c_int, c_int, c_int, c_void_p, c_size_t, c_void_p]),
+    "fd_spconv_apply_image": (c_int, [c_void_p, c_i64, c_void_p, c_void_p, c_void_p, c_int, c_void_p, c_i64, c_void_p, c_int, c_int, c_i64,
+                                      c_void_p, c_i64, c_int, c_int, c_int, c_void_p, c_void_p, c_size_t, c_void_p]),
     "fd_densify": (c_int, [c_void_p, c_int, c_int, c_void_p, c_void_p, c_int, c_int, c_int, c_int, c_void_p, c_int, c_i64,
                            c_i64, c_i64, c_i64, c_i64, c_void_p]),
     "fd_conv2d_packed_weight_bytes": (c_size_t, [c_int, c_int, c_int]),
diff --git a/include/futuredet_hip.h b/include/futuredet_hip.h
--- a/include/futuredet_hip.h
+++ b/include/futuredet_hip.h
@@ -57,6 +57,14 @@
 size_t fd_spconv_ranges_workspace_bytes(int64_t n_out);
 int fd_spconv_ranges(const int32_t *nbr, int64_t nbr_stride, int K, int64_t n_out, const int32_t *n_out_dev, int n_ranges,
                      int32_t *ranges , void *workspace, size_t workspace_bytes, fd_stream_t stream);
+size_t fd_spconv_image_bytes(int64_t n_out, int cin, int cout, int dtype, int n_ranges);
+int fd_spconv_image_build(const int32_t *nbr, int64_t nbr_stride, int K, int64_t n_out, const int32_t *n_out_dev,
+                          const int32_t *ranges , int n_ranges, int cin, int cout, void *image, size_t image_bytes,
+                          fd_stream_t stream);
+int fd_spconv_apply_image(const void *in_feats, int64_t n_in, const void *wpacked, const float *bias, const void *residual,
+                          int relu, const int32_t *nbr, int64_t nbr_stride, const int32_t *ranges, int n_ranges, int K, int64_t n_out,
+                          const int32_t *n_out_dev, int64_t n_expected, int cin, int cout, int dtype, void *out_feats,
+                          const void *image, size_t image_bytes, fd_stream_t stream);
 
 int fd_densify(const void *feats, int c, int dtype, const uint64_t *words, const int32_t *prefix, int B, int D,
                int H, int W, void *out, int out_dtype, int64_t stride_b, int64_t stride_c, int64_t stride_y,
```

Measured after the change: 284.5 (median of 6 runs). +1.2%, better.
